# trungnt13/odin-ai

Measured on AMD Instinct MI355X. Metric: VAE train images/sec, higher is better.
Workload: dtype f32; 1 GPU; dsprites_betavae_b256; global_batch=256, per_gpu_batch=256, parallelism=dp1, graph=True

## Files before the change

### include/odin_hip.h

```cpp
#ifndef ODIN_HIP_H
#define ODIN_HIP_H

#include <stddef.h>
#include <stdint.h>

#ifdef __cplusplus
extern "C" {
#endif

enum { ODIN_LINEAR = 0, ODIN_ELU = 1, ODIN_RELU = 2 };

typedef struct odin_conv_desc {
  int B, H, W, Cin;
  int OH, OW, Cout;
  int KH, KW, stride;
  int pad_t, pad_l;
  int act;
  int center;
  uint32_t* dy_amax;
  uint32_t* dx_amax;
  const uint32_t* x_amax;
  uint32_t* y_amax;
} odin_conv_desc;

int odin_version(void);
const char* odin_debug_last_path(void);
uint32_t odin_crc32c(uint32_t crc, const void* data, size_t n);
const char* odin_last_error(void);
int odin_max_slab_rows(void);
int odin_conv2d_dgrad_keeps_range(const odin_conv_desc* d, int aux_act);
int odin_deconv2d_dgrad_keeps_range(const odin_conv_desc* d, int aux_act);
int odin_bernoulli_tail_keeps_range(int is_deconv, const odin_conv_desc* d, int C1);
#define ODIN_RANGE_WORDS 2048
int odin_range_reset(uint32_t* words, int n, void* stream);
int odin_absmax(const float* t, size_t n, uint32_t* word, void* stream);
int odin_debug_stream_probe(const float* a, const float* b, float* out, size_t n, int variant, int blocks,
                            void* stream);
int odin_debug_absmax_fallbacks(void);

int odin_conv2d_fwd(const float* x, const float* w, const float* bias, float* y,
                    const odin_conv_desc* d, void* stream);
int odin_conv2d_dgrad(const float* dy, const float* w, const float* aux, int aux_act, float* dx,
                      float* colsum_slab, int* slab_rows_out, const odin_conv_desc* d,
                      void* stream);
int odin_conv2d_wgrad(const float* x, const float* dy, float* slab, int* slab_rows_out,
                      const odin_conv_desc* d, void* stream);

int odin_deconv2d_fwd(const float* x, const float* w, const float* bias, float* y,
                      const odin_conv_desc* d, void* stream);
int odin_deconv2d_dgrad(const float* dy, const float* w, const float* aux, int aux_act,
                        float* dx, float* colsum_slab, int* slab_rows_out,
                        const odin_conv_desc* d, void* stream);
int odin_deconv2d_wgrad(const float* x, const float* dy, float* slab, int* slab_rows_out,
                        const odin_conv_desc* d, void* stream);

int odin_conv2d_bwd(const float* x, const float* dy, const float* w, const float* aux, int aux_act, float* dx,
                    float* colsum_slab, int* colsum_rows_out, float* wslab, int* wslab_rows_out,
                    const odin_conv_desc* d, void* stream);
int odin_deconv2d_bwd(const float* x, const float* dy, const float* w, const float* aux, int aux_act, float* dx,
                      float* colsum_slab, int* colsum_rows_out, float* wslab, int* wslab_rows_out,
                      const odin_conv_desc* d, void* stream);
int odin_dense_bwd(const float* x, const float* dy, const float* w, const float* aux, int aux_act, float* dx,
                   float* colsum_slab, int* colsum_rows_out, float* wslab, int* wslab_rows_out, int B, int K,
                   int N, int want_wgrad, int want_dgrad, const uint32_t* dy_amax, uint32_t* dx_amax, void* stream);
int odin_conv2d_reads_x_range(const odin_conv_desc* d);
int odin_deconv2d_reads_x_range(const odin_conv_desc* d);
int odin_dense_reads_x_range(int B, int K, int N);
int odin_dense_fwd_ranged(const float* x, const float* w, const float* bias, float* y, int B, int K, int N, int act,
                          const uint32_t* x_amax, uint32_t* y_amax, void* stream);
int odin_dense_bwd_ranged(const float* x, const float* dy, const float* w, const float* aux, int aux_act, float* dx,
                          float* colsum_slab, int* colsum_rows_out, float* wslab, int* wslab_rows_out, int B, int K,
                          int N, int want_wgrad, int want_dgrad, const uint32_t* dy_amax, uint32_t* dx_amax,
                          const uint32_t* x_amax, void* stream);
int odin_dense_dgrad_keeps_range(int B, int K, int N);

int odin_bernoulli_tail_fwd_bwd(int is_deconv, const float* x, const float* w, const float* bias,
                                const float* w1, const float* b1, const float* target,
                                float* logits, float* g_out, float* llk_part, int* n_part_out,
                                float* tail_slab, int* slab_rows_out, const float* scale,
                                const odin_conv_desc* d, int C1, void* stream);

int odin_dense_fwd(const float* x, const float* w, const float* bias, float* y, int B, int K,
                   int N, int act, void* stream);
int odin_dense_dgrad(const float* dy, const float* w, const float* aux, int aux_act, float* dx,
                     float* colsum_slab, int* slab_rows_out, int B, int K, int N, void* stream);
int odin_dense_wgrad(const float* x, const float* dy, float* slab, int* slab_rows_out, int B,
                     int K, int N, void* stream);

typedef struct odin_reduce_job {
  const float* src;
  float* dst;
  int n;
  int rows;
  int stride;
  int pad_;
} odin_reduce_job;
int odin_slab_reduce(const odin_reduce_job* jobs, int n_jobs, void* stream);

int odin_latent_fwd(const float* p, const float* eps, float* z, float* kl, float* fbmask, int B,
                    int D, int analytic, float free_bits, const float* capacity, void* stream);
int odin_latent_bwd(const float* p, const float* eps, const float* z, const float* dz,
                    const float* dz_extra, const float* fbmask, const float* klw,
                    const float* dloc_x, const float* dscale_x, float* dp, int B, int D,
                    int analytic, void* stream);

int odin_latent_block_rows(int B, int P, int D, int N0);
int odin_latent_block_fwd(const float* h, const float* wl, const float* bl, const float* eps_in,
                          float* eps_out, uint64_t seed, const int32_t* step_dev, float* p, float* z,
                          float* kl, float* fbmask, const float* w0, const float* b0, float* y0, int B,
                          int P, int D, int N0, int act0, int analytic, float free_bits,
                          const float* capacity, void* stream);
int odin_latent_block_bwd(const float* g0, const float* w0, const float* z, const float* p,
                          const float* eps, const float* fbmask, const float* klw, const float* dz_extra,
                          const float* dloc_x, const float* dscale_x, const float* wl, const float* h,
                          int h_act, float* dz, float* dp, float* dh, float* slab0, float* slabl, int B,
                          int P, int D, int N0, int analytic, uint32_t* dh_amax, void* stream);

typedef struct odin_neck_args {
  int B, P, D, C0;
  int act2, act3, act4, act0, act1;
  int analytic;
  float free_bits;
  uint64_t seed;
  const int32_t* step_dev;
  const float* x;
  const uint32_t* x_amax;
  const float *w3, *b3;
  float* y3;
  const float *w4, *b4;
  float* y4;
  const float *wl, *bl;
  const float* eps_in;
  float* eps;
  float *p, *z, *kl, *fbmask;
  const float* capacity;
  const float *w0, *b0;
  float* y0;
  const float *w1, *b1;
  float* y1;
  uint32_t* y1_amax;
  const float* dy1;
  const float* klw;
  const float *dz_extra, *dloc_x, *dscale_x;
  float *dz, *dp;
  float* dh4;
  float* dy3;
  float* dx;
  uint32_t *dh4_amax, *dy3_amax, *dx_amax;
  float* slab1;
  float* slab0;
  float* slabl;
} odin_neck_args;
void odin_wgrad_pair_begin(void);
int odin_wgrad_pair_end(void);
int odin_neck_rows(int B, int P, int D, int C0);
int odin_neck_fwd(const odin_neck_args* a, void* stream);
int odin_neck_bwd(const odin_neck_args* a, void* stream);

int odin_disc_head_rows(int B, int K);
int odin_disc_head_fwd_bwd(const float* h, const float* w, const float* bias, float* logit, int mode,
                           const float* dlogit_in, float* dlogit_out, float* out, int aux_act, float* dh,
                           uint32_t* dh_amax, float* wslab, int* rows_out, void* workspace, int B, int K, void* stream);

int odin_elbo_bernoulli_fwd_bwd(const float* logits, const float* x, float* llk_part,
                                float* dlogits, const float* scale, int B, int n_per_sample,
                                int* n_part_out, void* stream);
int odin_elbo_bernoulli_fwd_bwd_ranged(const float* logits, const float* x, float* llk_part,
                                       float* dlogits, const float* scale, int B, int n_per_sample,
                                       int* n_part_out, uint32_t* dlogits_amax, void* stream);
int odin_elbo_gaussian_fwd_bwd(const float* h, const float* x, float* llk_part, float* dh,
                               const float* scale, int B, int n_pix, int C, int softplus1,
                               int* n_part_out, void* stream);
void odin_wgrad_planes_defer_begin(void);
int odin_wgrad_planes_defer_end(void* stream);
double odin_debug_igemm_h_min_flop(double flop);
double odin_debug_blk_min_flop(double flop);
int odin_debug_blk_planes(int enable);
int odin_debug_blk_first(int on);
int odin_debug_dense_hw_min_tiles(int tiles);

int odin_gaussian_tail_applicable(const odin_conv_desc* d, int C);
int odin_gaussian_tail_fwd_bwd(const float* x, const float* w, const float* bias, const float* w1, const float* b1,
                               const float* target, float* logits, float* g_out, float* llk_part, int* n_part_out,
                               float* tail_slab, int* slab_rows_out, const float* scale, const odin_conv_desc* d, int C,
                               int softplus1, void* stream);
int odin_gaussian_head_fwd_bwd(const float* h, const float* w1, const float* b1, const float* target,
                               float* logits, float* dlogits, float* dh, float* llk_part, int* n_part_out,
                               float* wslab, int* rows_out, float* colsum_slab, const float* scale, int B,
                               int n_pix, int Cin, int C, int softplus1, int h_act, uint32_t* dh_amax,
                               void* stream);
int odin_elbo_mixqlogistic_fwd_bwd(const float* h, const float* x, float* llk_part, float* dh,
                                   const float* scale, int B, int n_pix, int C, int K,
                                   int* n_part_out, void* stream);
int odin_elbo_finalize(const float* llk_part, int n_part, const float* kl, const float* hyper,
                       const float* tc, float* llk, float* out4, int B, void* stream);
int odin_mean(const float* x, int n, float* out, void* stream);

int odin_total_correlation_workspace(int B_local, int B_global, int D);
int odin_total_correlation_fwd_bwd(const float* z, const float* p, float* tc_out, float* dz,
                                   float* dloc, float* dscale, const float* coef, int B, int D,
                                   void* stream);
int odin_total_correlation_shard(const float* z_local, const float* p_global, float* tc_out,
                                 float* dz_local, float* dloc_part, float* dscale_part,
                                 const float* coef, int B_local, int B_global, int D, void* stream);
int odin_mmd_workspace(int B_local, int B_global, int M, int D);
int odin_mmd_fwd_bwd(const float* x, const float* y, float* ws, float* dz, const float* coef,
                     const float* coef_grad, int N, int M, int D, int kernel, uint64_t prior_seed,
                     const int32_t* step_dev, void* stream);
int odin_mmd_shard(const float* x_local, const float* x_all, const float* y, float* ws, float* dz_local,
                   const float* coef, const float* coef_grad, int B_local, int B_global, int M, int D,
                   int kernel, int include_yy, uint64_t prior_seed, const int32_t* step_dev, void* stream);
int odin_dip_workspace(int world, int D);
int odin_dip_fwd_bwd(const float* p, float* ws, float* dloc, float* dscale, const float* coef,
                     const float* coef_grad, int N, int D, int type2, float lambda_diag, float lambda_offdiag,
// ... 113 lines not shown
```

### odin_ai_amd/_lib.py

```python
from __future__ import annotations

import ctypes as C
import os
from typing import Optional

_HERE = os.path.dirname(os.path.abspath(__file__))
DEFAULT_LIB = os.path.join(_HERE, 'libodin_hip.so')

ACT = {'linear': 0, 'elu': 1, 'relu': 2, None: 0}


class ConvDesc(C.Structure):
  _fields_ = [(n, C.c_int) for n in ('B', 'H', 'W', 'Cin', 'OH', 'OW', 'Cout', 'KH', 'KW',
                                     'stride', 'pad_t', 'pad_l', 'act', 'center')] + \
             [('dy_amax', C.c_void_p), ('dx_amax', C.c_void_p),
              ('x_amax', C.c_void_p), ('y_amax', C.c_void_p)]


class ReduceJob(C.Structure):
  _fields_ = [('src', C.c_void_p), ('dst', C.c_void_p), ('n', C.c_int), ('rows', C.c_int),
              ('stride', C.c_int), ('pad_', C.c_int)]


class AdamFold(C.Structure):
  _fields_ = [('x', C.c_void_p), ('dy', C.c_void_p), ('B', C.c_int), ('K', C.c_int), ('N', C.c_int), ('w_off', C.c_size_t),
              ('slab', C.c_void_p), ('slab_rows', C.c_int), ('slab_stride', C.c_size_t), ('slab_n', C.c_size_t),
              ('slab_off', C.c_size_t), ('zero', C.c_void_p), ('zero_n', C.c_int)]


class NeckArgs(C.Structure):
  _fields_ = [(n, C.c_int) for n in ('B', 'P', 'D', 'C0', 'act2', 'act3', 'act4', 'act0', 'act1', 'analytic')] + \
             [('free_bits', C.c_float), ('seed', C.c_uint64)] + \
             [(n, C.c_void_p) for n in (
                 'step_dev', 'x', 'x_amax', 'w3', 'b3', 'y3', 'w4', 'b4', 'y4', 'wl', 'bl', 'eps_in', 'eps', 'p', 'z',
                 'kl', 'fbmask', 'capacity', 'w0', 'b0', 'y0', 'w1', 'b1', 'y1', 'y1_amax',
                 'dy1', 'klw', 'dz_extra', 'dloc_x', 'dscale_x', 'dz', 'dp', 'dh4', 'dy3', 'dx',
                 'dh4_amax', 'dy3_amax', 'dx_amax', 'slab1', 'slab0', 'slabl')]


P = C.c_void_p
I = C.c_int
F = C.c_float
IP = C.POINTER(C.c_int)
DP = C.POINTER(ConvDesc)

SIGNATURES = {
    'odin_version': [],
    'odin_debug_last_path': [],
    'odin_crc32c': [C.c_uint32, P, C.c_size_t],
    'odin_max_slab_rows': [],
    'odin_range_reset': [P, I, P],
    'odin_conv2d_dgrad_keeps_range': [DP, I],
    'odin_deconv2d_dgrad_keeps_range': [DP, I],
    'odin_bernoulli_tail_keeps_range': [I, DP, I],
    'odin_conv2d_bwd': [P, P, P, P, I, P, P, IP, P, IP, DP, P],
    'odin_deconv2d_bwd': [P, P, P, P, I, P, P, IP, P, IP, DP, P],
    'odin_dense_bwd': [P, P, P, P, I, P, P, IP, P, IP, I, I, I, I, I, P, P, P],
    'odin_dense_bwd_ranged': [P, P, P, P, I, P, P, IP, P, IP, I, I, I, I, I, P, P, P, P],
    'odin_dense_dgrad_keeps_range': [I, I, I],
    'odin_conv2d_reads_x_range': [DP],
    'odin_deconv2d_reads_x_range': [DP],
    'odin_dense_reads_x_range': [I, I, I],
    'odin_absmax': [P, C.c_size_t, P, P],
    'odin_debug_absmax_fallbacks': [],
    'odin_debug_stream_probe': [P, P, P, C.c_size_t, I, I, P],
    'odin_comm_unique_id': [P],
    'odin_comm_init': [C.POINTER(C.c_void_p), P, I, I],
    'odin_comm_destroy': [P],
    'odin_comm_library': [],
    'odin_allreduce_flat': [P, P, C.c_size_t, P],
    'odin_allgather_flat': [P, P, P, C.c_size_t, P],
    'odin_reduce_scatter_flat': [P, P, P, C.c_size_t, P],
    'odin_conv2d_fwd': [P, P, P, P, DP, P],
    'odin_conv2d_dgrad': [P, P, P, I, P, P, IP, DP, P],
    'odin_conv2d_wgrad': [P, P, P, IP, DP, P],
    'odin_deconv2d_fwd': [P, P, P, P, DP, P],
    'odin_deconv2d_dgrad': [P, P, P, I, P, P, IP, DP, P],
    'odin_deconv2d_wgrad': [P, P, P, IP, DP, P],
    'odin_bernoulli_tail_fwd_bwd': [I, P, P, P, P, P, P, P, P, P, IP, P, IP, P, DP, I, P],
    'odin_dense_fwd': [P, P, P, P, I, I, I, I, P],
    'odin_dense_fwd_ranged': [P, P, P, P, I, I, I, I, P, P, P],
    'odin_dense_dgrad': [P, P, P, I, P, P, IP, I, I, I, P],
    'odin_dense_wgrad': [P, P, P, IP, I, I, I, P],
    'odin_slab_reduce': [C.POINTER(ReduceJob), I, P],
    'odin_latent_fwd': [P, P, P, P, P, I, I, I, F, P, P],
    'odin_latent_bwd': [P, P, P, P, P, P, P, P, P, P, I, I, I, P],
    'odin_latent_block_rows': [I, I, I, I],
    'odin_latent_block_fwd': [P, P, P, P, P, C.c_uint64, P, P, P, P, P, P, P, P, I, I, I, I, I, I, F, P, P],
    'odin_latent_block_bwd': [P, P, P, P, P, P, P, P, P, P, P, P, I, P, P, P, P, P, I, I, I, I, I, P, P],
    'odin_wgrad_pair_begin': [],
    'odin_wgrad_pair_end': [],
    'odin_neck_rows': [I, I, I, I],
    'odin_neck_fwd': [C.POINTER(NeckArgs), P],
    'odin_neck_bwd': [C.POINTER(NeckArgs), P],
    'odin_elbo_bernoulli_fwd_bwd': [P, P, P, P, P, I, I, IP, P],
    'odin_elbo_bernoulli_fwd_bwd_ranged': [P, P, P, P, P, I, I, IP, P, P],
    'odin_elbo_gaussian_fwd_bwd': [P, P, P, P, P, I, I, I, I, IP, P],
    'odin_gaussian_tail_applicable': [DP, I],
    'odin_gaussian_tail_fwd_bwd': [P, P, P, P, P, P, P, P, P, IP, P, IP, P, DP, I, I, P],
    'odin_gaussian_head_fwd_bwd': [P, P, P, P, P, P, P, P, IP, P, IP, P, P, I, I, I, I, I, I, P, P],
    'odin_disc_head_rows': [I, I],
    'odin_disc_head_fwd_bwd': [P, P, P, P, I, P, P, P, I, P, P, P, IP, P, I, I, P],
    'odin_debug_igemm_h_min_flop': [C.c_double],
    'odin_debug_blk_min_flop': [C.c_double],
    'odin_debug_blk_planes': [C.c_int],
    'odin_debug_blk_first': [C.c_int],
    'odin_debug_dense_hw_min_tiles': [C.c_int],
    'odin_debug_mel_r16': [C.c_int],
    'odin_debug_smallc_planes': [C.c_int],
    'odin_wgrad_planes_defer_begin': [],
    'odin_wgrad_planes_defer_end': [P],
    'odin_elbo_mixqlogistic_fwd_bwd': [P, P, P, P, P, I, I, I, I, IP, P],
    'odin_elbo_finalize': [P, I, P, P, P, P, P, I, P],
    'odin_mean': [P, I, P, P],
    'odin_total_correlation_workspace': [I, I, I],
    'odin_total_correlation_fwd_bwd': [P, P, P, P, P, P, P, I, I, P],
    'odin_total_correlation_shard': [P, P, P, P, P, P, P, I, I, I, P],
    'odin_mmd_workspace': [I, I, I, I],
    'odin_mmd_fwd_bwd': [P, P, P, P, P, P, I, I, I, I, C.c_uint64, P, P],
    'odin_mmd_shard': [P, P, P, P, P, P, P, I, I, I, I, I, I, C.c_uint64, P, P],
    'odin_dip_workspace': [I, I],
    'odin_dip_fwd_bwd': [P, P, P, P, P, P, I, I, I, F, F, P],
    'odin_dip_moments': [P, P, I, I, P],
    'odin_dip_finish': [P, I, P, P, P, P, P, P, I, I, I, F, F, P],
    'odin_vamprior_workspace': [I, I, I],
    'odin_vamprior_fwd_bwd': [P, P, P, P, P, P, P, P, I, I, I, P],
    'odin_clip_range_fwd': [P, P, C.c_size_t, F, F, P],
    'odin_clip_range_bwd': [P, P, C.c_size_t, F, F, F, P],
    'odin_vq_workspace': [I],
    'odin_vq_assign': [P, P, P, P, P, P, P, P, I, I, I, P],
    'odin_vq_bwd': [P, P, P, P, P, P, P, P, P, F, C.c_double, C.c_double, I, P, I, I, I, P],
    'odin_permute_dims': [P, P, P, I, I, P],
    'odin_random_perm': [P, I, I, C.c_uint64, P, P],
    'odin_random_permute_dims': [P, P, P, I, I, C.c_uint64, P, P],
    'odin_dtc_loss_fwd_bwd': [P, P, P, P, P, I, P],
    'odin_adam_step_flat': [P, P, P, P, C.c_size_t, P, P, F, P, P],
    'odin_adam_step_fold': [P, P, P, P, C.c_size_t, P, C.POINTER(AdamFold), P],
    'odin_sumsq_flat': [P, C.c_size_t, P, P, P],
    'odin_latent_sample_logprob': [P, P, P, P, P, I, I, I, P],
    'odin_logmeanexp_rows': [P, P, I, I, P],
    'odin_sum_parts': [P, I, P, I, P],
    'odin_grad_skip_threshold': [P, C.c_size_t, F, P, P, P, P],
    'odin_clip_by_norm_segments': [P, P, I, F, P],
    'odin_clip_by_value': [P, C.c_size_t, F, P, F, P],
    'odin_sumsq_adam_flat': [P, P, P, P, C.c_size_t, P, P, P, F, P, P],
    'odin_sumsq_adam_finalize_flat': [P, P, P, P, C.c_size_t, P, P, P, F, P, P, I, P, P, P, P, P, I, P],
    'odin_sumsq_adam_ring': [P, P, P, P, C.c_size_t, P, P, P, F, P, P, I, P, P, P, P, P, I, P, P, P, I, I, I, P],
    'odin_slab_reduce_sumsq': [P, I, P, C.c_size_t, P, IP, P, P, I, P],
    'odin_adam_ring_parts': [P, P, P, P, C.c_size_t, P, I, I, P, I, P, F, P, P, I, P, P, P, P, I, P, P, I, I, I, P],
    'odin_rng_normal': [P, C.c_size_t, C.c_uint64, P, P],
    'odin_gather_normalize_u8': [P, P, P, I, I, F, I, P],
    'odin_gather_rows_f32': [P, P, P, I, I, P],
    'odin_stft_mel_db': [P, P, P, P, P, P, I, I, I, I, I, I, C.c_double, C.c_double, I, P],
    'odin_stft_mel_db_frames': [P, P, P, P, P, P, I, I, I, I, I, I, C.c_double, C.c_double, I, I, P, P],
    'odin_debug_set_stamps': [P],
    'odin_debug_set_wgrad_stamps': [P],
    'odin_debug_set_neck_stamps': [P],
    'odin_debug_elbo_shape': [I, I, I],
    'odin_debug_set_mel_stamps': [P],
    'odin_debug_igemm_h_ldsw_steps': [I],
    'odin_graph_begin': [P],
    'odin_graph_end': [P, C.POINTER(C.c_void_p)],
    'odin_graph_launch': [P, P],
    'odin_graph_destroy': [P],
}


VALUE_RETURNING = ('odin_version', 'odin_comm_library', 'odin_conv2d_dgrad_keeps_range',
                   'odin_deconv2d_dgrad_keeps_range', 'odin_bernoulli_tail_keeps_range', 'odin_dense_dgrad_keeps_range', 'odin_conv2d_reads_x_range',
                   'odin_deconv2d_reads_x_range', 'odin_dense_reads_x_range', 'odin_max_slab_rows', 'odin_debug_absmax_fallbacks', 'odin_crc32c', 'odin_debug_last_path',
                   'odin_latent_block_rows', 'odin_neck_rows', 'odin_debug_igemm_h_ldsw_steps', 'odin_total_correlation_workspace', 'odin_mmd_workspace', 'odin_dip_workspace', 'odin_vamprior_workspace', 'odin_vq_workspace', 'odin_debug_igemm_h_min_flop', 'odin_debug_blk_min_flop',
                   'odin_debug_blk_planes', 'odin_debug_blk_first', 'odin_debug_dense_hw_min_tiles', 'odin_gaussian_tail_applicable', 'odin_disc_head_rows', 'odin_debug_mel_r16', 'odin_debug_smallc_planes')
VOID_RETURNING = ('odin_wgrad_planes_defer_begin', 'odin_wgrad_pair_begin')


class OdinError(RuntimeError):
  pass


class Lib:

  def __init__(self, path: str):
    if not os.path.exists(path):
      raise OdinError(
          f"HIP extension not found: {path}. Build it with `python -c 'import "
          f"__graft_entry__ as g; g.build()'` (hipcc --offload-arch=gfx950). There is no "
          f"CPU fallback.")
    self.path = path
    self.c = C.CDLL(path)
    self.c.odin_last_error.restype = C.c_char_p
    self.c.odin_last_error.argtypes = []
    for name, args in SIGNATURES.items():
      fn = getattr(self.c, name)
      fn.argtypes = args
      fn.restype = (C.c_char_p if name in ('odin_debug_last_path', 'odin_comm_library') else
                    C.c_double if name in ('odin_debug_igemm_h_min_flop', 'odin_debug_blk_min_flop') else
                    None if name in VOID_RETURNING else
                    C.c_uint32 if name in VALUE_RETURNING else C.c_int)

  def check(self, rc: int, what: str = ''):
    if rc != 0:
      raise OdinError(f"{what} failed: {self.c.odin_last_error().decode()} (rc={rc})")

  def __getattr__(self, name):
    if name.startswith('odin_'):
      fn = getattr(self.c, name)

      trace = os.environ.get('ODIN_TRACE', '0') == '1'

# ... 45 lines not shown
```

### odin_ai_amd/csrc/dispatch.hip

```cpp
#include "odin_device.h"
#include "odin_internal.h"

namespace {

enum Family {
  GENERIC,
  SMALLC, PW1X1, SMALLDECONV, SMALLDECONV_GEN,
  FCONV_PLANES, FCONV_RING, FCONV_BLK, CONV5_BLK, TCONV_PLANES, TCONV_RING, TCONV_BLK, IGEMM_H, IGEMM,
  WGRAD_PLANES, WGRAD5_BLK, WGRAD_BLK, IGEMM_H_WGRAD, IGEMM_WGRAD,
  BWD_PLANES, BWD_BLK,
  BWD_PAIR,
  TINY_DENSE, THIN_DENSE, DENSE_H, DENSE_GEMM
};

enum { FOLDS_Y = 1, FOLDS_DX = 2, READS_X = 4 };
int traits(Family f) {
  switch (f) {
    case SMALLC: case SMALLDECONV_GEN: return FOLDS_Y;
    case SMALLDECONV: case IGEMM: case THIN_DENSE: return FOLDS_Y | FOLDS_DX;
    case FCONV_PLANES: case FCONV_BLK: case CONV5_BLK: case TCONV_PLANES: case TCONV_BLK: case IGEMM_H: case DENSE_H:
      return FOLDS_Y | FOLDS_DX | READS_X;
    case WGRAD_PLANES: case WGRAD5_BLK: case WGRAD_BLK: case IGEMM_H_WGRAD: return READS_X;
    case BWD_PLANES: case BWD_BLK: case DENSE_GEMM: return FOLDS_DX;
    default: return 0;
  }
}

int keep_range(int rc, Family f, int fold_bit, const float* t, size_t n, uint32_t* word, void* stream) {
  if (rc != 0 || t == nullptr || word == nullptr || (traits(f) & fold_bit)) return rc;
  return odin_absmax_fold(t, n, word, stream);
}

bool doubles(const odin_geom& g) { return g.OH == 2 * g.H && g.OW == 2 * g.W; }
bool same_size(const odin_geom& g) { return g.H == g.OH && g.W == g.OW; }
bool aligned16(const void* a, const void* b, const void* c, const void* d) {
  return ((((size_t)a | (size_t)b | (size_t)c | (size_t)d)) & 15) == 0;
}


Family select_conv2d_fwd(const odin_geom& g, bool bias, int act) {
  if (odin_smallc_applicable(g)) return SMALLC;
  if (odin_pw1x1_applicable(g)) return PW1X1;
  if (act == ODIN_ACT_ELU && bias && odin_fconv_planes_applicable(g)) return FCONV_PLANES;
  if (act == ODIN_ACT_ELU && bias && odin_fconv_ring_applicable(g)) return FCONV_RING;
  if (bias && same_size(g) && odin_conv5_blk_applicable(g)) return CONV5_BLK;
  if (bias && odin_fconv_blk_applicable(g)) return FCONV_BLK;
  if (odin_igemm_h_applicable(0, g)) return IGEMM_H;
  if (odin_igemm_applicable(0, g)) return IGEMM;
  return GENERIC;
}

bool igemm_dgrad(int tmode, const odin_geom& g, bool slab, bool dry) {
  return odin_igemm_applicable(tmode, g) && (odin_igemm_tiles(tmode, g) <= ODIN_MAX_COLSUM_BLOCKS || (!slab && !dry));
}

Family select_conv2d_dgrad(const odin_geom& l, const odin_geom& g, int aux_act, bool aux_ok, bool slab, bool dry) {
  if (odin_pw1x1_applicable(l)) return PW1X1;
  if (aux_act == ODIN_ACT_ELU && aux_ok && doubles(g) && odin_tconv_planes_applicable(g, 2, 1)) return TCONV_PLANES;
  if (aux_act == ODIN_ACT_ELU && aux_ok && doubles(g) && odin_tconv_ring_applicable(g)) return TCONV_RING;
  if (same_size(g) && odin_conv5_blk_applicable(g)) return CONV5_BLK;
  if (doubles(g) && odin_tconv_blk_applicable(g)) return TCONV_BLK;
  if (odin_igemm_h_applicable(1, g)) return IGEMM_H;
  if (igemm_dgrad(1, g, slab, dry)) return IGEMM;
  return GENERIC;
}

Family select_deconv2d_fwd(const odin_geom& g, bool bias, int act) {
  if (bias && odin_smalldeconv_applicable(g)) return SMALLDECONV;
  if (act == ODIN_ACT_ELU && bias && doubles(g) && odin_tconv_planes_applicable(g, 1, 1)) return TCONV_PLANES;
  if (act == ODIN_ACT_ELU && bias && doubles(g) && odin_tconv_ring_applicable(g)) return TCONV_RING;
  if (bias && (g.CI & 7) != 0 && odin_smalldeconv_gen_applicable(g)) return SMALLDECONV_GEN;
  if (bias && doubles(g) && odin_tconv_blk_applicable(g)) return TCONV_BLK;
  if (odin_igemm_h_applicable(1, g)) return IGEMM_H;
  if (odin_igemm_applicable(1, g)) return IGEMM;
  return GENERIC;
}

Family select_deconv2d_dgrad(const odin_geom& l, const odin_geom& g, int aux_act, bool aux_ok, bool slab, bool dry) {
  if (!slab && odin_smalldeconv_applicable(l)) return SMALLDECONV;
  if (aux_act == ODIN_ACT_ELU && aux_ok && odin_fconv_planes_applicable(g)) return FCONV_PLANES;
  if (odin_fconv_blk_applicable(g)) return FCONV_BLK;
  if (odin_igemm_h_applicable(0, g)) return IGEMM_H;
  const bool ring_two_pass_vs_igemm =
      g.CI == 64 && odin_igemm_applicable(0, g) && odin_igemm_tiles(0, g) <= ODIN_MAX_COLSUM_BLOCKS;
  if (!ring_two_pass_vs_igemm && aux_act == ODIN_ACT_ELU && aux_ok && odin_fconv_ring_applicable(g)) return FCONV_RING;
  if (igemm_dgrad(0, g, slab, dry)) return IGEMM;
  return GENERIC;
}

Family select_bernoulli_tail(int is_deconv, const odin_geom& g, int act, int C1) {
  if (is_deconv && act == ODIN_ACT_ELU && doubles(g) && odin_tconv_planes_applicable(g, 3, C1)) return TCONV_PLANES;
  if (is_deconv && act == ODIN_ACT_ELU && g.CO == 32 && (C1 == 1 || C1 == 3) && doubles(g) &&
      odin_tconv_ring_applicable(g))
    return TCONV_RING;
  return GENERIC;
}

Family select_wgrad_shared(const odin_geom& g, bool want_bias) {
  if (odin_wgrad_planes_applicable(g)) return WGRAD_PLANES;
  if (same_size(g) && want_bias && odin_wgrad5_blk_applicable(g)) return WGRAD5_BLK;
  if (odin_wgrad_blk_applicable(g)) return WGRAD_BLK;
  if (odin_igemm_h_wgrad_applicable(g)) return IGEMM_H_WGRAD;
  if (odin_igemm_wgrad_applicable(g)) return IGEMM_WGRAD;
  return GENERIC;
}
Family select_conv2d_wgrad(const odin_geom& g) {
  if (odin_smallc_applicable(g)) return SMALLC;
  if (odin_pw1x1_applicable(g)) return PW1X1;
  return select_wgrad_shared(g, true);
}
Family select_deconv2d_wgrad(const odin_geom& l, const odin_geom& g) {
  if (odin_smalldeconv_applicable(l)) return SMALLDECONV;
  return select_wgrad_shared(g, false);
}

Family select_deconv2d_bwd(const odin_geom& l, const odin_geom& g, int aux_act, bool aux, bool both, bool dry,
                           bool slab) {
  if (!slab && both && odin_smalldeconv_applicable(l)) return SMALLDECONV;
  const bool k4s2 = l.KH == 4 && l.KW == 4 && l.S == 2 && l.pt == 1 && l.pl == 1 && doubles(l);
  if (((both && aux) || dry) && aux_act == ODIN_ACT_ELU && k4s2 && odin_bwd_planes_applicable(l) &&
      odin_wgrad_planes_applicable(g) && odin_fconv_planes_applicable(g))
    return BWD_PLANES;
  if ((both || dry) && k4s2 && !l.center && odin_bwd_blk_applicable(l)) return BWD_BLK;
  return BWD_PAIR;
}

bool dense_via_igemm() { return ODIN_DIAG_ENV("ODIN_NODENSEIGEMM") == nullptr; }

Family select_dense_fwd(int B, int K, int N, bool aligned) {
  if (odin_tiny_dense_ok(B, K, N)) return TINY_DENSE;
  if (odin_thin_dense_kind(B, K, N) != 0 && aligned) return THIN_DENSE;
  if (odin_dense_h_ok(B, K, N)) return DENSE_H;
  if (dense_via_igemm() && odin_igemm_applicable(0, odin_geom_dense(B, K, N))) return IGEMM;
  if (odin_dense_gemm_ok(B, K, N)) return DENSE_GEMM;
  return GENERIC;
}
Family select_dense_dgrad(int B, int K, int N, bool slab, bool aligned) {
  if (odin_tiny_dense_ok(B, K, N)) return TINY_DENSE;
  if (slab) return GENERIC;
  if (odin_thin_dense_kind(B, K, N) != 0 && aligned) return THIN_DENSE;
  if (odin_dense_h_ok(B, K, N)) return DENSE_H;
  if (dense_via_igemm() && odin_igemm_applicable(1, odin_geom_dense(B, N, K))) return IGEMM;
  if (odin_dense_gemm_ok(B, K, N)) return DENSE_GEMM;
  return GENERIC;
}
Family select_dense_wgrad(int B, int K, int N, bool aligned) {
  if (odin_dense_h_ok(B, K, N)) return DENSE_H;
  if (odin_thin_dense_wgrad_rows(B, K, N) > 0 && aligned) return THIN_DENSE;
  if (dense_via_igemm() && !odin_tiny_dense_ok(B, K, N) && odin_igemm_wgrad_applicable(odin_geom_dense(B, K, N)))
    return IGEMM_WGRAD;
  if (odin_dense_gemm_ok(B, K, N) && !ODIN_DIAG_ENV("ODIN_NOTINYWGRADGEMM")) return DENSE_GEMM;
  return select_wgrad_shared(odin_geom_dense(B, K, N), true);
}
Family select_dense_bwd(int B, int K, int N, bool slab) {
  return odin_dense_h_ok(B, K, N) && !slab ? DENSE_H : BWD_PAIR;
}


int launch_gather(Family f, int tmode, int wmode, const odin_geom& g, const float* in, const float* w, const float* bias,
                  const float* aux, int aux_act, float* out, float* colsum, int* rows_out, int epi, int act,
                  const uint32_t* in_amax, uint32_t* out_amax, void* stream) {
  const float* blk_aux = aux_act != 0 ? aux : nullptr;
  const int blk_act = epi == 1 ? act : aux_act;
  switch (f) {
    case FCONV_PLANES:
      return odin_fconv_planes_launch(in, w, bias, aux, out, colsum, rows_out, g.B, g.OH, g.OW, g.CI, g.CO, epi, in_amax,
                                      out_amax, stream);
    case FCONV_RING:
      return odin_fconv_ring_launch(in, w, bias, aux, out, colsum, rows_out, g.B, g.H, g.W, g.CI, g.OH, g.OW, g.CO, epi,
                                    stream);
    case FCONV_BLK:
      return odin_fconv_blk_launch(in, w, bias, blk_aux, out, colsum, rows_out, g.B, g.OH, g.OW, g.CI, g.CO, epi, blk_act,
                                   in_amax, out_amax, stream);
    case CONV5_BLK:
      return odin_conv5_blk_launch(in, w, bias, blk_aux, out, colsum, rows_out, g.B, g.H, g.W, g.CI, g.CO, g.KH, epi,
                                   blk_act, in_amax, out_amax, stream);
    case TCONV_PLANES:
      return odin_tconv_planes_launch(in, w, bias, aux, out, colsum, rows_out, nullptr, nullptr, nullptr, nullptr, nullptr,
                                      nullptr, nullptr, nullptr, 1, g.B, g.H, g.W, g.CI, g.CO, epi, in_amax, out_amax, stream);
    case TCONV_RING:
      return odin_tconv_ring_launch(in, w, bias, aux, out, colsum, rows_out, nullptr, nullptr, nullptr, nullptr, nullptr,
                                    nullptr, nullptr, nullptr, 1, g.B, g.H, g.W, g.CO, epi, stream);
    case TCONV_BLK:
      return odin_tconv_blk_launch(in, w, bias, blk_aux, out, colsum, rows_out, g.B, g.H, g.W, g.CI, g.CO, epi, blk_act,
                                   in_amax, out_amax, stream);
    case IGEMM_H:
      return odin_igemm_h_launch(tmode, in, w, bias, aux, aux_act, out, colsum, g.B, g.H, g.W, g.CI, g.OH, g.OW, g.CO, g.KH,
                                 g.KW, g.S, g.pt, g.pl, act, in_amax, epi == 2, out_amax, stream);
    case IGEMM:
      return odin_igemm_launch(tmode, in, w, bias, aux, aux_act, out, colsum, g.B, g.H, g.W, g.CI, g.OH, g.OW, g.CO, g.KH,
                               g.KW, g.S, g.pt, g.pl, act, out_amax, stream);
    default:
      return odin_gather_generic(tmode, wmode, g, in, w, bias, act, aux, aux_act, out, colsum,
                                 colsum ? -ODIN_MAX_COLSUM_BLOCKS : odin_num_cus(), rows_out, nullptr, nullptr, stream);
  }
}

int dgrad_rows(Family f, int tmode, const odin_geom& g) {
  switch (f) {
    case SMALLDECONV: return 0;
    case IGEMM_H: return odin_igemm_h_rows(tmode, g);
    case IGEMM: return odin_igemm_tiles(tmode, g);
    default: return -1;
  }
}

int conv_dgrad(Family f, int tmode, int wmode, const odin_geom& g, const float* dy, const float* w, const float* aux,
               int aux_act, float* dx, float* colsum_slab, int* slab_rows_out, const odin_conv_desc* d, void* stream) {
  const int rows = dgrad_rows(f, tmode, g);
  if (rows >= 0) {
    if (slab_rows_out) *slab_rows_out = rows;
    if (dx == nullptr) return 0;
  }
  int rc;
  if (f == PW1X1) rc = odin_pw1x1_dgrad(dy, w, aux, aux_act, dx, colsum_slab, slab_rows_out, d, stream);
  else if (f == SMALLDECONV) rc = odin_smalldeconv_bwd(nullptr, dy, w, aux, aux_act, dx, nullptr, nullptr, d, stream);
  else
    rc = launch_gather(f, tmode, wmode, g, dy, w, nullptr, aux, aux_act, dx, colsum_slab, slab_rows_out, 2, 0, d->dy_amax,
                       d->dx_amax, stream);
  return keep_range(rc, f, FOLDS_DX, dx, (size_t)d->B * d->H * d->W * d->Cin, d->dx_amax, stream);
}

int conv_fwd(Family f, int tmode, int wmode, const odin_geom& g, const float* x, const float* w, const float* bias,
             float* y, const odin_conv_desc* d, void* stream) {
  int rc;
  switch (f) {
    case SMALLC: rc = odin_smallc_fwd(x, w, bias, y, d, stream); break;
    case PW1X1: rc = odin_pw1x1_fwd(x, w, bias, y, d, stream); break;
    case SMALLDECONV: rc = odin_smalldeconv_fwd(x, w, bias, y, d, stream); break;
    case SMALLDECONV_GEN: rc = odin_smalldeconv_gen_fwd(x, w, bias, y, d, stream); break;
    default:
      rc = launch_gather(f, tmode, wmode, g, x, w, bias, nullptr, 0, y, nullptr, nullptr, 1, d->act, d->x_amax, d->y_amax,
                         stream);
  }
  return keep_range(rc, f, FOLDS_Y, y, (size_t)d->B * d->OH * d->OW * d->Cout, d->y_amax, stream);
}

int launch_wgrad(Family f, const odin_geom& g, const float* in, const float* dy, float* slab, int want_bias,
                 const uint32_t* g_amax, const uint32_t* a_amax, int* rows_out, void* stream) {
  const int grad_u = want_bias ? 0 : 1;
  const int slab_stride = g.KH * g.KW * g.CI * g.CO + (want_bias ? g.CO : 0);
  if (f == IGEMM_H_WGRAD || f == IGEMM_WGRAD) {
    if (rows_out) *rows_out = f == IGEMM_H_WGRAD ? odin_igemm_h_wgrad_rows(g) : odin_igemm_wgrad_rows(g);
    if (slab == nullptr) return 0;
  }
  switch (f) {
    case WGRAD_PLANES:
      return odin_wgrad_planes_launch(in, dy, slab, rows_out, g.B, g.OH, g.OW, g.CI, g.CO, want_bias, grad_u, g_amax, a_amax,
                                      stream);
    case WGRAD5_BLK:
      return odin_wgrad5_blk_launch(in, dy, slab, rows_out, g.B, g.H, g.W, g.CI, g.CO, g.KH, want_bias, g_amax, a_amax,
                                    stream);
    case WGRAD_BLK:
      return odin_wgrad_blk_launch(in, dy, slab, rows_out, g.B, g.OH, g.OW, g.CI, g.CO, want_bias, grad_u, g_amax, a_amax,
                                   stream);
    case IGEMM_H_WGRAD:
      return odin_igemm_h_wgrad_launch(in, dy, slab, slab_stride, g.B, g.H, g.W, g.CI, g.OH, g.OW, g.CO, g.KH, g.KW, g.S,
                                       g.pt, g.pl, want_bias, grad_u, g_amax, a_amax, stream);
    case IGEMM_WGRAD:
      return odin_igemm_wgrad_launch(in, dy, slab, slab_stride, g.B, g.H, g.W, g.CI, g.OH, g.OW, g.CO, g.KH, g.KW, g.S, g.pt,
                                     g.pl, want_bias, stream);
    default:
      return odin_wgrad_generic(g, in, dy, slab, want_bias, rows_out, stream);
  }
}

int pair_end(int rc) {
  const int rc2 = odin_igemm_pair_end();
  return rc != 0 ? rc : rc2;
}

}

extern "C" int odin_conv2d_fwd(const float* x, const float* w, const float* bias, float* y, const odin_conv_desc* d,
                               void* stream) {
  const odin_geom g = odin_geom_fwd(d);
  return conv_fwd(select_conv2d_fwd(g, bias != nullptr, d->act), 0, 0, g, x, w, bias, y, d, stream);
}

extern "C" int odin_conv2d_dgrad(const float* dy, const float* w, const float* aux, int aux_act, float* dx,
                                 float* colsum_slab, int* slab_rows_out, const odin_conv_desc* d, void* stream) {
  const odin_geom g = odin_geom_dgrad(d);
  const Family f = select_conv2d_dgrad(odin_geom_fwd(d), g, aux_act, aux != nullptr || dx == nullptr,
                                       colsum_slab != nullptr, dx == nullptr);
  return conv_dgrad(f, 1, 1, g, dy, w, aux, aux_act, dx, colsum_slab, slab_rows_out, d, stream);
}

extern "C" int odin_conv2d_wgrad(const float* x, const float* dy, float* slab, int* slab_rows_out,
                                 const odin_conv_desc* d, void* stream) {
  const odin_geom g = odin_geom_fwd(d);
  const Family f = select_conv2d_wgrad(g);
  if (f == SMALLC) return odin_smallc_wgrad(x, dy, slab, slab_rows_out, d, stream);
  if (f == PW1X1) return odin_pw1x1_wgrad(x, dy, slab, slab_rows_out, d, stream);
  return launch_wgrad(f, g, x, dy, slab, 1, d->dy_amax, d->x_amax, slab_rows_out, stream);
}

extern "C" int odin_conv2d_bwd(const float* x, const float* dy, const float* w, const float* aux, int aux_act, float* dx,
                               float* colsum_slab, int* colsum_rows_out, float* wslab, int* wslab_rows_out,
                               const odin_conv_desc* d, void* stream) {
  odin_igemm_pair_begin();
  int rc = odin_conv2d_wgrad(x, dy, wslab, wslab_rows_out, d, stream);
  if (rc == 0) rc = odin_conv2d_dgrad(dy, w, aux, aux_act, dx, colsum_slab, colsum_rows_out, d, stream);
  return pair_end(rc);
}

extern "C" int odin_conv2d_dgrad_keeps_range(const odin_conv_desc* d, int aux_act) {
  const Family f = select_conv2d_dgrad(odin_geom_fwd(d), odin_geom_dgrad(d), aux_act, true, false, false);
  return (traits(f) & FOLDS_DX) ? 1 : 0;
}

extern "C" int odin_conv2d_reads_x_range(const odin_conv_desc* d) {
  const odin_geom g = odin_geom_fwd(d);
  return ((traits(select_conv2d_fwd(g, true, d->act)) | traits(select_conv2d_wgrad(g))) & READS_X) ? 1 : 0;
}

extern "C" int odin_deconv2d_fwd(const float* x, const float* w, const float* bias, float* y, const odin_conv_desc* d,
                                 void* stream) {
  const odin_geom g = odin_geom_fwd(d);
  return conv_fwd(select_deconv2d_fwd(g, bias != nullptr, d->act), 1, 1, g, x, w, bias, y, d, stream);
}

extern "C" int odin_deconv2d_dgrad(const float* dy, const float* w, const float* aux, int aux_act, float* dx,
                                   float* colsum_slab, int* slab_rows_out, const odin_conv_desc* d, void* stream) {
  const odin_geom g = odin_geom_dgrad(d);
  const Family f = select_deconv2d_dgrad(odin_geom_fwd(d), g, aux_act, aux != nullptr || dx == nullptr,
                                         colsum_slab != nullptr, dx == nullptr);
  return conv_dgrad(f, 0, 0, g, dy, w, aux, aux_act, dx, colsum_slab, slab_rows_out, d, stream);
}

extern "C" int odin_deconv2d_wgrad(const float* x, const float* dy, float* slab, int* slab_rows_out,
                                   const odin_conv_desc* d, void* stream) {
  const odin_geom g = odin_geom_dgrad(d);
  const Family f = select_deconv2d_wgrad(odin_geom_fwd(d), g);
  if (f == SMALLDECONV)
    return odin_smalldeconv_bwd(x, dy, nullptr, nullptr, 0, nullptr, slab, slab_rows_out, d, stream);
  return launch_wgrad(f, g, dy, x, slab, 0, d->dy_amax, d->x_amax, slab_rows_out, stream);
}

extern "C" int odin_deconv2d_bwd(const float* x, const float* dy, const float* w, const float* aux, int aux_act, float* dx,
                                 float* colsum_slab, int* colsum_rows_out, float* wslab, int* wslab_rows_out,
                                 const odin_conv_desc* d, void* stream) {
  const odin_geom l = odin_geom_fwd(d);
  const bool dry = dx == nullptr && wslab == nullptr;
  const Family f = select_deconv2d_bwd(l, odin_geom_dgrad(d), aux_act, aux != nullptr, dx != nullptr && wslab != nullptr,
                                       dry, colsum_slab != nullptr);
  if (f == SMALLDECONV) {
    if (colsum_rows_out) *colsum_rows_out = 0;
    return odin_smalldeconv_bwd(x, dy, w, aux, aux_act, dx, wslab, wslab_rows_out, d, stream);
  }
  if (f == BWD_PLANES || f == BWD_BLK) {
    const int rows = f == BWD_PLANES ? odin_bwd_planes_rows(l) : odin_bwd_blk_rows(l);
    if (colsum_rows_out) *colsum_rows_out = rows;
    if (wslab_rows_out) *wslab_rows_out = rows;
    if (dry) return 0;
    if (f == BWD_PLANES)
      return odin_bwd_planes_launch(x, dy, w, aux, dx, colsum_slab, wslab, d->B, d->H, d->W, d->Cin, d->Cout, d->dy_amax,
                                    d->x_amax, d->dx_amax, stream);
    return odin_bwd_blk_launch(x, dy, w, aux, aux_act, dx, colsum_slab, wslab, d->B, d->H, d->W, d->Cin, d->Cout,
                               d->dy_amax, d->x_amax, d->dx_amax, stream);
  }
  odin_igemm_pair_begin();
  int rc = odin_deconv2d_wgrad(x, dy, wslab, wslab_rows_out, d, stream);
  if (rc == 0) rc = odin_deconv2d_dgrad(dy, w, aux, aux_act, dx, colsum_slab, colsum_rows_out, d, stream);
  return pair_end(rc);
}

extern "C" int odin_deconv2d_dgrad_keeps_range(const odin_conv_desc* d, int aux_act) {
  const Family f = select_deconv2d_dgrad(odin_geom_fwd(d), odin_geom_dgrad(d), aux_act, true, false, false);
  return (traits(f) & FOLDS_DX) ? 1 : 0;
}
extern "C" int odin_deconv2d_reads_x_range(const odin_conv_desc* d) {
  const odin_geom l = odin_geom_fwd(d);
  return ((traits(select_deconv2d_fwd(l, true, d->act)) | traits(select_deconv2d_wgrad(l, odin_geom_dgrad(d)))) & READS_X)
             ? 1 : 0;
}

extern "C" int odin_bernoulli_tail_fwd_bwd(int is_deconv, const float* x, const float* w, const float* bias, const float* w1,
                                           const float* b1, const float* target, float* logits, float* g_out,
                                           float* llk_part, int* n_part_out, float* tail_slab, int* slab_rows_out,
                                           const float* scale, const odin_conv_desc* d, int C1, void* stream) {
  const odin_geom g = odin_geom_fwd(d);
  const Family f = select_bernoulli_tail(is_deconv, g, d->act, C1);
  const odin_tail_args tail = {w1, b1, target, scale, logits, llk_part, tail_slab, C1};
  int rc;
  if (f == TCONV_PLANES)
    rc = odin_tconv_planes_launch(x, w, bias, nullptr, g_out, nullptr, slab_rows_out, w1, b1, target, logits, llk_part,
                                  n_part_out, tail_slab, scale, C1, d->B, d->H, d->W, d->Cin, d->Cout, 3, d->x_amax,
                                  d->dy_amax, stream);
  else if (f == TCONV_RING)
    rc = odin_tconv_ring_launch(x, w, bias, nullptr, g_out, nullptr, slab_rows_out, w1, b1, target, logits, llk_part,
                                n_part_out, tail_slab, scale, C1, d->B, d->H, d->W, d->Cout, 3, stream);
  else
    rc = odin_gather_generic(is_deconv, is_deconv ? 1 : 0, g, x, w, bias, d->act, nullptr, 0, g_out, nullptr,
                             -ODIN_MAX_COLSUM_BLOCKS, slab_rows_out, &tail, n_part_out, stream);
  return keep_range(rc, f, FOLDS_Y, g_out, (size_t)d->B * d->OH * d->OW * d->Cout, d->dy_amax, stream);
}
extern "C" int odin_bernoulli_tail_keeps_range(int is_deconv, const odin_conv_desc* d, int C1) {
  return (traits(select_bernoulli_tail(is_deconv, odin_geom_fwd(d), d->act, C1)) & FOLDS_Y) ? 1 : 0;
}

extern "C" int odin_dense_fwd(const float* x, const float* w, const float* bias, float* y, int B, int K, int N, int act,
                              void* stream) {
  return odin_dense_fwd_ranged(x, w, bias, y, B, K, N, act, nullptr, nullptr, stream);
}

extern "C" int odin_dense_fwd_ranged(const float* x, const float* w, const float* bias, float* y, int B, int K, int N,
                                     int act, const uint32_t* x_amax, uint32_t* y_amax, void* stream) {
  const Family f = select_dense_fwd(B, K, N, aligned16(x, w, y, bias));
  int rc;
  switch (f) {
    case TINY_DENSE: rc = odin_tiny_dense_fwd(x, w, bias, y, B, K, N, act, stream); break;
    case THIN_DENSE: rc = odin_thin_dense_fwd(x, w, bias, y, B, K, N, act, y_amax, stream); break;
    case DENSE_H: rc = odin_dense_h_fwd(x, w, bias, y, B, K, N, act, x_amax, y_amax, stream); break;
    case DENSE_GEMM: rc = odin_dense_gemm_fwd(x, w, bias, y, B, K, N, act, stream); break;
    default:
      rc = launch_gather(f, 0, 0, odin_geom_dense(B, K, N), x, w, bias, nullptr, 0, y, nullptr, nullptr, 1, act, nullptr,
                         y_amax, stream);
  }
  return keep_range(rc, f, FOLDS_Y, y, (size_t)B * N, y_amax, stream);
}

static int dense_dgrad(const float* dy, const float* w, const float* aux, int aux_act, float* dx, float* colsum_slab,
                       int* slab_rows_out, int B, int K, int N, const uint32_t* dy_amax, uint32_t* dx_amax,
                       void* stream) {
  const Family f = select_dense_dgrad(B, K, N, colsum_slab != nullptr, aligned16(dy, w, dx, aux));
  if (f != TINY_DENSE && f != GENERIC) {
    if (slab_rows_out) *slab_rows_out = 0;
    if (dx == nullptr) return 0;
  }
  int rc;
  switch (f) {
    case TINY_DENSE:
      rc = odin_tiny_dense_dgrad(dy, w, aux, aux_act, dx, colsum_slab, slab_rows_out, B, K, N, stream);
      break;
    case THIN_DENSE: rc = odin_thin_dense_dgrad(dy, w, aux, aux_act, dx, B, K, N, dx_amax, stream); break;
    case DENSE_H: rc = odin_dense_h_dgrad(dy, w, aux, aux_act, dx, B, K, N, dy_amax, dx_amax, stream); break;
    case DENSE_GEMM: rc = odin_dense_gemm_dgrad(dy, w, aux, aux_act, dx, B, K, N, dx_amax, stream); break;
    default:
      rc = launch_gather(f, f == IGEMM, 1, odin_geom_dense(B, N, K), dy, w, nullptr, aux, aux_act, dx, colsum_slab,
                         slab_rows_out, 2, 0, nullptr, dx_amax, stream);
  }
  return keep_range(rc, f, FOLDS_DX, dx, (size_t)B * K, dx_amax, stream);
}

extern "C" int odin_dense_dgrad(const float* dy, const float* w, const float* aux, int aux_act, float* dx,
                                float* colsum_slab, int* slab_rows_out, int B, int K, int N, void* stream) {
  return dense_dgrad(dy, w, aux, aux_act, dx, colsum_slab, slab_rows_out, B, K, N, nullptr, nullptr, stream);
}

extern "C" int odin_dense_wgrad(const float* x, const float* dy, float* slab, int* slab_rows_out, int B, int K, int N,
                                void* stream) {
  const Family f = select_dense_wgrad(B, K, N, slab == nullptr || aligned16(x, dy, slab, nullptr));
  if (f == DENSE_H || f == THIN_DENSE || f == DENSE_GEMM) {
    if (slab_rows_out) *slab_rows_out = f == THIN_DENSE ? odin_thin_dense_wgrad_rows(B, K, N) : 1;
    if (slab == nullptr) return 0;
    if (f == DENSE_H) return odin_dense_h_wgrad(x, dy, slab, B, K, N, nullptr, nullptr, stream);
    if (f == THIN_DENSE) return odin_thin_dense_wgrad(x, dy, slab, B, K, N, stream);
    return odin_dense_gemm_wgrad(x, dy, slab, B, K, N, stream);
// ... 51 lines not shown
```

### odin_ai_amd/csrc/odin_internal.h

```cpp
#pragma once
#include <cstdio>
#include <cstring>
#include "../../include/odin_hip.h"

#define ODIN_MAX_SLAB_BLOCKS 256
#define ODIN_MAX_COLSUM_BLOCKS 512

#include <cstdlib>
#ifdef ODIN_DIAG
#define ODIN_DIAG_ENV(name) getenv(name)
#else
#define ODIN_DIAG_ENV(name) ((const char*)nullptr)
#endif
static inline bool odin_exact_fp32() { return getenv("ODIN_EXACT_FP32") != nullptr; }

struct odin_geom {
  int B, H, W, CI, OH, OW, CO, KH, KW, S, pt, pl, center;
};
static inline odin_geom odin_geom_fwd(const odin_conv_desc* d) {
  return {d->B, d->H, d->W, d->Cin, d->OH, d->OW, d->Cout, d->KH, d->KW, d->stride, d->pad_t, d->pad_l, d->center};
}
static inline odin_geom odin_geom_dgrad(const odin_conv_desc* d) {
  return {d->B, d->OH, d->OW, d->Cout, d->H, d->W, d->Cin, d->KH, d->KW, d->stride, d->pad_t, d->pad_l, 0};
}
static inline odin_geom odin_geom_dense(int B, int K, int N) { return {B, 1, 1, K, 1, 1, N, 1, 1, 1, 0, 0, 0}; }

int odin_fail(int code, const char* msg);
int odin_check_launch(const char* what);
int odin_wgrad_planes_flush(void* stream);
int odin_num_cus();
const uint32_t* odin_range_word_of(const float* t, size_t n, const uint32_t* given, void* stream);
int odin_absmax_fold(const float* t, size_t n, uint32_t* word, void* stream);

bool odin_smallc_applicable(const odin_geom& g);
int odin_smallc_fwd(const float* x, const float* w, const float* bias, float* y,
                    const odin_conv_desc* d, void* stream);
int odin_smallc_wgrad(const float* x, const float* dy, float* slab, int* rows_out,
                      const odin_conv_desc* d, void* stream);

bool odin_tiny_dense_ok(int B, int K, int N);
int odin_tiny_dense_fwd(const float* x, const float* w, const float* bias, float* y, int B, int K,
                        int N, int act, void* stream);
int odin_tiny_dense_dgrad(const float* dy, const float* w, const float* aux, int aux_act, float* dx,
                          float* colsum_slab, int* slab_rows_out, int B, int K, int N, void* stream);

bool odin_pw1x1_applicable(const odin_geom& g);
int odin_pw1x1_fwd(const float* x, const float* w, const float* bias, float* y,
                   const odin_conv_desc* d, void* stream);
int odin_pw1x1_dgrad(const float* dy, const float* w, const float* aux, int aux_act, float* dx,
                     float* colsum_slab, int* slab_rows_out, const odin_conv_desc* d, void* stream);
int odin_pw1x1_wgrad(const float* x, const float* dy, float* slab, int* slab_rows_out,
                     const odin_conv_desc* d, void* stream);

bool odin_dense_gemm_ok(int B, int K, int N);
int odin_dense_gemm_fwd(const float* x, const float* w, const float* bias, float* y, int B, int K,
                        int N, int act, void* stream);
int odin_dense_gemm_dgrad(const float* dy, const float* w, const float* aux, int aux_act, float* dx,
                          int B, int K, int N, uint32_t* dx_amax, void* stream);
int odin_zero_u32(uint32_t* p, size_t n, void* stream);
int odin_dense_gemm_wgrad(const float* x, const float* dy, float* slab, int B, int K, int N,
                          void* stream);

int odin_thin_dense_kind(int B, int K, int N);
int odin_thin_dense_wgrad_rows(int B, int K, int N);
int odin_thin_dense_fwd(const float* x, const float* w, const float* bias, float* y, int B, int K, int N, int act,
                        uint32_t* y_amax, void* stream);
int odin_thin_dense_dgrad(const float* dy, const float* w, const float* aux, int aux_act, float* dx, int B, int K, int N,
                          uint32_t* dx_amax, void* stream);
int odin_thin_dense_wgrad(const float* x, const float* dy, float* slab, int B, int K, int N, void* stream);

bool odin_dense_h_ok(int B, int K, int N);
int odin_dense_h_fwd(const float* x, const float* w, const float* bias, float* y, int B, int K, int N, int act,
                     const uint32_t* x_amax, uint32_t* y_amax, void* stream);
int odin_dense_h_dgrad(const float* dy, const float* w, const float* aux, int aux_act, float* dx, int B, int K, int N,
                       const uint32_t* dy_amax, uint32_t* dx_amax, void* stream);
int odin_dense_h_wgrad(const float* x, const float* dy, float* slab, int B, int K, int N, const uint32_t* dy_amax,
                       const uint32_t* x_amax, void* stream);
int odin_dense_h_bwd_pair(const float* x, const float* dy, const float* w, const float* aux, int aux_act, float* dx,
                          float* slab, int B, int K, int N, const uint32_t* dy_amax, uint32_t* dx_amax,
                          const uint32_t* x_amax, void* stream);

bool odin_bwd_planes_applicable(const odin_geom& g);
int odin_bwd_planes_rows(const odin_geom& g);
int odin_bwd_planes_launch(const float* x, const float* dy, const float* w, const float* aux, float* dx, float* colsum,
                           float* wslab, int B, int H, int W, int Cin, int Cout, const uint32_t* dy_amax,
                           const uint32_t* x_amax, uint32_t* dx_amax, void* stream);
bool odin_smalldeconv_applicable(const odin_geom& g);
bool odin_smalldeconv_gen_applicable(const odin_geom& g);
int odin_smalldeconv_gen_fwd(const float* x, const float* w, const float* bias, float* y, const odin_conv_desc* d,
                             void* stream);
int odin_smalldeconv_fwd(const float* x, const float* w, const float* bias, float* y, const odin_conv_desc* d,
                         void* stream);
int odin_smalldeconv_bwd(const float* x, const float* dy, const float* w, const float* aux, int aux_act, float* dx,
                         float* slab, int* rows_out, const odin_conv_desc* d, void* stream);

bool odin_fconv_ring_applicable(const odin_geom& g);
int odin_fconv_ring_launch(const float* in, const float* w, const float* bias, const float* aux,
                           float* out, float* colsum, int* rows_out, int B, int H, int W, int CI,
                           int OH, int OW, int CO, int epi, void* stream);
void odin_fconv_ring_set_stamps(void* buf);

void odin_tconv_ring_set_stamps(void* buf);
bool odin_tconv_ring_applicable(const odin_geom& g);
int odin_tconv_ring_launch(const float* in, const float* w, const float* bias, const float* aux,
                           float* out, float* colsum, int* rows_out, const float* w1, const float* b1,
                           const float* target, float* logits, float* llk_part, int* n_part_out,
                           float* slab, const float* scale, int C1, int B, int H, int W, int CO,
                           int epi, void* stream);

bool odin_tconv_blk_applicable(const odin_geom& g);
int odin_tconv_blk_launch(const float* in, const float* w, const float* bias, const float* aux, float* out,
                          float* colsum, int* rows_out, int B, int H, int W, int CI, int CO, int epi, int act,
                          const uint32_t* in_amax, uint32_t* out_amax, void* stream);
bool odin_fconv_blk_applicable(const odin_geom& g);
int odin_fconv_blk_launch(const float* in, const float* w, const float* bias, const float* aux, float* out,
                          float* colsum, int* rows_out, int B, int OH, int OW, int CI, int CO, int epi, int act,
                          const uint32_t* in_amax, uint32_t* out_amax, void* stream);
bool odin_wgrad_blk_applicable(const odin_geom& g);
int odin_wgrad_blk_launch(const float* U, const float* V, float* slab, int* rows_out, int B, int OH, int OW, int CI,
                          int CO, int want_bias, int grad_u, const uint32_t* g_amax, const uint32_t* a_amax,
                          void* stream);
bool odin_conv5_blk_applicable(const odin_geom& g);
int odin_conv5_blk_launch(const float* in, const float* w, const float* bias, const float* aux, float* out,
                          float* colsum, int* rows_out, int B, int H, int W, int CI, int CO, int K, int epi, int act,
                          const uint32_t* in_amax, uint32_t* out_amax, void* stream);
bool odin_wgrad5_blk_applicable(const odin_geom& g);
int odin_wgrad5_blk_launch(const float* x, const float* dy, float* slab, int* rows_out, int B, int H, int W, int CI,
                           int CO, int K, int want_bias, const uint32_t* g_amax, const uint32_t* a_amax, void* stream);
bool odin_blk_enabled(double flop);
bool odin_blk_first();
bool odin_bwd_blk_applicable(const odin_geom& g);
int odin_bwd_blk_rows(const odin_geom& g);
int odin_bwd_blk_launch(const float* x, const float* dy, const float* w, const float* aux, int aux_act, float* dx,
                        float* colsum, float* wslab, int B, int H, int W, int Cin, int Cout, const uint32_t* dy_amax,
                        const uint32_t* x_amax, uint32_t* dx_amax, void* stream);
void odin_tconv_planes_set_stamps(void* buf);
bool odin_tconv_planes_applicable(const odin_geom& g, int epi, int C1);
int odin_tconv_planes_launch(const float* in, const float* w, const float* bias, const float* aux,
                             float* out, float* colsum, int* rows_out, const float* w1, const float* b1,
                             const float* target, float* logits, float* llk_part, int* n_part_out,
                             float* slab, const float* scale, int C1, int B, int H, int W, int CI,
                             int CO, int epi, const uint32_t* in_amax, uint32_t* out_amax, void* stream);

bool odin_wgrad_planes_applicable(const odin_geom& g);
int odin_wgrad_planes_launch(const float* U, const float* V, float* slab, int* rows_out, int B, int OH,
                             int OW, int CI, int CO, int want_bias, int grad_u, const uint32_t* g_amax,
                             const uint32_t* a_amax, void* stream);

bool odin_fconv_planes_applicable(const odin_geom& g);
void odin_fconv_planes_set_stamps(void* buf);
int odin_fconv_planes_launch(const float* in, const float* w, const float* bias, const float* aux,
                             float* out, float* colsum, int* rows_out, int B, int OH, int OW, int CI, int CO,
                             int epi, const uint32_t* in_amax, uint32_t* out_amax, void* stream);

bool odin_igemm_applicable(int tmode, const odin_geom& g);
void odin_igemm_set_stamps(void* buf);
int odin_igemm_tiles(int tmode, const odin_geom& g);
int odin_igemm_launch(int tmode, const float* in, const float* w, const float* bias, const float* aux,
                      int aux_act, float* out, float* colsum, int B, int H, int W, int CI, int OH, int OW,
                      int CO, int KH, int KW, int S, int pt, int pl, int act, uint32_t* out_amax, void* stream);
void odin_igemm_pair_begin();
int odin_igemm_pair_end();
bool odin_igemm_h_applicable(int tmode, const odin_geom& g);
int odin_igemm_h_rows(int tmode, const odin_geom& g);
int odin_igemm_h_launch(int tmode, const float* in, const float* w, const float* bias, const float* aux, int aux_act,
                        float* out, float* colsum, int B, int H, int W, int CI, int OH, int OW, int CO, int KH, int KW,
                        int S, int pt, int pl, int act, const uint32_t* in_amax, int in_is_grad, uint32_t* out_amax,
                        void* stream);
bool odin_igemm_h_wgrad_applicable(const odin_geom& g);
int odin_igemm_h_wgrad_rows(const odin_geom& g);
int odin_igemm_h_wgrad_launch(const float* u, const float* v, float* slab, int slab_stride, int B, int FH, int FW,
                              int CU, int h, int w, int CV, int KH, int KW, int S, int pt, int pl, int want_bias,
                              int grad_u, const uint32_t* g_amax, const uint32_t* a_amax, void* stream);
bool odin_igemm_wgrad_applicable(const odin_geom& g);
int odin_igemm_wgrad_rows(const odin_geom& g);
int odin_igemm_wgrad_launch(const float* u, const float* v, float* slab, int slab_stride, int B, int FH,
                            int FW, int CU, int h, int w, int CV, int KH, int KW, int S, int pt, int pl,
                            int want_bias, void* stream);

struct odin_tail_args {
  const float *w1, *b1, *target, *scale;
  float *logits, *llk_part, *slab;
  int C1;
};
int odin_gather_generic(int mode_t, int wmode, const odin_geom& g, const float* in, const float* w, const float* bias,
                        int act, const float* aux, int aux_act, float* out, float* colsum_slab, int max_blocks,
                        int* rows_out, const odin_tail_args* tail, int* n_part_out, void* stream);
int odin_wgrad_generic(const odin_geom& g, const float* in, const float* dy, float* slab, int want_bias, int* rows_out,
                       void* stream);
```

### odin_ai_amd/csrc/tconv_planes.hip

```cpp
#include "odin_device.h"
#include "odin_internal.h"
#include <cstdlib>
#include <utility>

namespace {

struct TPParams {
  const float* in;
  const float* w;
  const float* bias;
  const float* aux;
  float* out;
  float* colsum;
  const float* w1;
  const float* b1;
  const float* target;
  float* logits;
  float* llk_part;
  float* slab;
  const float* scale;
  int B, H, CO;
  int CS, ci_off;
  int tiles_per_img, n_tiles, tiles_per_wg;
  const unsigned* in_amax;
  unsigned* out_amax;
  long long* stamps;
  int part_off;
};

#if defined(ODIN_SIM) || !defined(ODIN_DIAG)
#define TP_STAMP(k) ((void)0)
#else
#define TP_STAMP(k)                                                                               \
  do {                                                                                            \
    if (p.stamps != nullptr && blockIdx.x == 0 && blockIdx.y == 0 && lane == 0 && (wave & 3) == 0 && \
        stamp_i < 31)                                                                             \
      p.stamps[8 * wave + stamp_i++] = ((long long)(k) << 56) | (long long)(clock64() & 0xFFFFFFFFFFFFFFll); \
  } while (0)
#endif

__host__ __device__ constexpr int tp_late_index(int g0, int m) {
  return (m < g0 || m == 32 || m == 33 || m == 34 || m == 36 || m == 42)
             ? -1
             : (m - g0) - ((m > 32) + (m > 33) + (m > 34) + (m > 36) + (m > 42));
}
static_assert(tp_late_index(25, 47) >= 11, "three logit maps: 8 gradient + 4 store slots must fit");

template <int... Is, class F>
__device__ __forceinline__ void tp_static_for_impl(std::integer_sequence<int, Is...>, F&& f) {
  (f(std::integral_constant<int, Is>{}), ...);
}
template <int N, class F>
__device__ __forceinline__ void tp_static_for(F&& f) {
  tp_static_for_impl(std::make_integer_sequence<int, N>{}, static_cast<F&&>(f));
}

struct TpYes { static constexpr bool value = true; };
struct TpNo { static constexpr bool value = false; };

constexpr int TP_NPL = 2;
constexpr int TP_TAPB = TP_NPL * 4 * 512;
constexpr int TP_WBYTES = 16 * TP_TAPB;

__device__ __forceinline__ float tp_pairsum32(float x) {
#ifdef ODIN_SIM
  return x + __shfl_xor(x, 32);
#else
  const unsigned u = __float_as_uint(x);
  const auto r = __builtin_amdgcn_permlane32_swap(u, u, false, false);
  return __uint_as_float(r[0]) + __uint_as_float(r[1]);
#endif
}

struct alignas(8) TpEnt {
  int x, y;
};

struct TpItem {
  float4 v;
  int dst;
  int ok;
};

template <int EPI, int C1, int W, int DBG = 0, bool ACC = false, int SCM = 0, bool PL = false>
__device__ __forceinline__ void tp_body(const TPParams& p) {
  constexpr int NPL = TP_NPL;
  constexpr int RP = 64 / W;
  constexpr int NSLOT = 2 * RP + 3;
  constexpr int PB = (W + 2) * 64;
  constexpr int RB = NPL * PB;
  constexpr int CPR = W / 8;
  constexpr int CSHIFT = (W == 32) ? 2 : (W == 16) ? 1 : 0;
  ODIN_DYN_SMEM(char, smem);
  char* wl = smem;
  char* ring = smem + TP_WBYTES;
  constexpr int NRED = 32 * (1 + (EPI == 3 ? C1 : 0)) + 4;
  __shared__ float cred[8 * NRED];
  __shared__ float llk_red[2][8];
  const int tid = threadIdx.x, lane = tid & 63;
#ifdef ODIN_SIM
  const int wave = tid >> 6;
#else
  const int wave = __builtin_amdgcn_readfirstlane(tid >> 6);
#endif
  const int l31 = lane & 31, half = lane >> 5;
  int stamp_i = 0;
  (void)stamp_i;
  TP_STAMP(1);
#if defined(ODIN_DIAG) && !defined(ODIN_SIM)
  if (p.stamps != nullptr && blockIdx.x == 0 && blockIdx.y == 0 && tid == 0) {
    p.stamps[64] = clock64();
    p.stamps[65] = wall_clock64();
  }
#endif
  const int n0 = blockIdx.y * 32;
  const int HP = p.H + 1;
  const int OH = 2 * p.H, OW = 2 * W;
  const int T0 = blockIdx.x * p.tiles_per_wg;
  int T1 = T0 + p.tiles_per_wg;
  if (T1 > p.n_tiles) T1 = p.n_tiles;
  if (T0 >= T1) return;

  const OdinRangeReq in_rq = odin_range_issue(SCM != 0 ? p.in_amax : nullptr, lane);
  float4 wv[8];
#pragma unroll
  for (int j = 0; j < 8; ++j) {
    const int e = tid + 512 * j;
    const int ci4 = e & 7, co = (e >> 3) & 31, tap = e >> 8;
    wv[j] = *reinterpret_cast<const float4*>(p.w + ((size_t)(tap * p.CO + n0 + co) * p.CS + p.ci_off + 4 * ci4));
  }
  const OdinRun IN = odin_run(p.in, (unsigned)((size_t)p.B * p.H * W * p.CS * 4));
  float amx = 0.f;
  const int f_c = wave & (CPR - 1), f_r0 = wave >> CSHIFT;
  constexpr int F_RJ = 8 >> CSHIFT;
  const int f_px = 8 * f_c + (lane >> 3), f_ch4 = lane & 7, f_pc = f_px + 1;
  const int f_lds_lane = f_pc * 64 + ((((f_ch4 >> 1) ^ ((f_pc >> 2) & 3))) << 4) + (f_ch4 & 1) * 8;
  const unsigned f_g_lane = (unsigned)((f_px * p.CS + p.ci_off + 4 * f_ch4) * 4);
  const unsigned f_rowbytes = (unsigned)(W * p.CS * 4);
  TpItem itA[2], itB[2];
  {
    const int tpi = p.tiles_per_img;
    const int b0 = odin_div_small(T0, tpi), t0 = T0 - b0 * tpi;
    const int start = HP * b0 + RP * t0;
#pragma unroll
    for (int j = 0; j < 2; ++j) {
      const int r = f_r0 + F_RJ * j, G = start + r;
      const bool valid = r < RP + 2;
      const int b = b0 + (RP * t0 + r >= HP ? 1 : 0), gi = G - b * HP;
      const bool real = valid && gi != 0 && b < p.B;
      itA[j].dst = (G % NSLOT) * RB + f_lds_lane;
      itA[j].ok = valid;
      itA[j].v = odin_run_load4(IN, (real ? (unsigned)(G - b - 1) * f_rowbytes : 0xFFFF0000u) + f_g_lane);
    }
  }
  ODIN_SCHED_FENCE();
  bool scl = SCM == 1;
  float in_s = 1.f, in_s2k = ODIN_LO_SCALE, out_s = 1.f, out_sx = ODIN_LO_UNSCALE;

  for (int e = tid; e < NSLOT * 8 * NPL; e += 512) {
    const int sl = e / (8 * NPL), rem = e - sl * (8 * NPL);
    const int pl = rem >> 3, side = (rem >> 2) & 1, piece = rem & 3;
    *reinterpret_cast<float4*>(ring + sl * RB + pl * PB + (side ? (W + 1) * 64 : 0) + piece * 16) =
        make_float4(0.f, 0.f, 0.f, 0.f);
  }

  constexpr int RPF = 2 * F_RJ;
  const int NF = p.tiles_per_wg + 3;
  TpEnt* tr = reinterpret_cast<TpEnt*>(ring + NSLOT * RB);
  {
    const int tpi = p.tiles_per_img;
    for (int e = tid; e < NF * RPF; e += 512) {
      const int f = e / RPF, r = e - f * RPF;
      const int T = T0 + f, b1 = odin_div_small(T, tpi), t1 = T - b1 * tpi;
      const int end = HP * b1 + RP * t1 + RP + 2;
      int start = end - (RP + 2);
      if (f > 0) {
        const int b0 = t1 > 0 ? b1 : b1 - 1, t0 = t1 > 0 ? t1 - 1 : tpi - 1;
        start = HP * b0 + RP * t0 + RP + 2;
      }
      const int G = start + r;
      const bool valid = T < T1 && G < end;
      const int b = odin_div_small(G, HP), gi = G - b * HP;
      const bool real = valid && gi != 0 && b < p.B;
      tr[e] = TpEnt{valid ? (G % NSLOT) * RB : -1, real ? (int)((unsigned)(G - b - 1) * f_rowbytes) : (int)0xFFFF0000u};
    }
  }
  auto fill_entries = [&](TpEnt (&en)[2], int f) {
#pragma unroll
    for (int j = 0; j < 2; ++j) en[j] = tr[f * RPF + f_r0 + F_RJ * j];
  };
  auto fill_loads = [&](TpItem (&it)[2], const TpEnt (&en)[2]) {
#pragma unroll
    for (int j = 0; j < 2; ++j) {
      it[j].dst = en[j].x + f_lds_lane;
#ifdef ODIN_SIM
      it[j].ok = en[j].x >= 0;
#else
      it[j].ok = __builtin_amdgcn_readfirstlane(en[j].x) >= 0;
#endif
      it[j].v = odin_run_load4(IN, (unsigned)en[j].y + f_g_lane);
    }
  };
  auto store_fill1 = [&](const TpItem& it) {
    if (it.ok) {
      u32x2 h, l;
      if (SCM == 1 || (SCM == 2 && scl)) odin_split_h4<true>(it.v, in_s, in_s2k, h, l);
      else odin_split_h4<false>(it.v, 1.f, ODIN_LO_SCALE, h, l);
      char* d = ring + it.dst;
      *reinterpret_cast<u32x2*>(d) = h;
      *reinterpret_cast<u32x2*>(d + PB) = l;
    }
  };
  auto store_fill = [&](const TpItem (&it)[2]) {
    store_fill1(it[0]);
    store_fill1(it[1]);
  };

  const int role = wave & 3, grp = wave >> 2;
  const int cpw = role & 1, rpar = role >> 1;
  const int rp = (W == 32) ? grp : (W == 16) ? 2 * grp + (l31 >> 4) : 4 * grp + (l31 >> 3);
  const int i_in = (W == 32) ? l31 : (W == 16) ? (l31 & 15) : (l31 & 7);
  const int kw_a = cpw ? 0 : 1, kw_b = kw_a + 2;
  const int kh_a = rpar ? 0 : 1, kh_b = kh_a + 2;
  const int d_a = cpw ? 2 : 1;
  int offA[2], offB[2];
#pragma unroll
  for (int kk = 0; kk < 2; ++kk) {
    const int pa = i_in + d_a, pb = pa - 1;
    offA[kk] = pa * 64 + (((2 * kk + half) ^ ((pa >> 2) & 3)) << 4);
    offB[kk] = pb * 64 + (((2 * kk + half) ^ ((pb >> 2) & 3)) << 4);
  }
  const int roff_a = rp + (rpar ? 2 : 1);
  const char* wlane = wl + half * 512 + l31 * 16;
  const int tap_aa = (kh_a * 4 + kw_a) * TP_TAPB, tap_ab = (kh_a * 4 + kw_b) * TP_TAPB;
  const int tap_ba = (kh_b * 4 + kw_a) * TP_TAPB, tap_bb = (kh_b * 4 + kw_b) * TP_TAPB;

  auto ch_of = [&](int r) { return (r & 3) + 8 * (r >> 2) + 4 * half; };
  constexpr float LOG2E = 1.44269504088896341f;
  constexpr bool CL = (EPI == 3 && C1 > 1);
  __shared__ float cst[CL ? 32 * (1 + C1) : 4];
  if (CL) {
    for (int e = tid; e < 32 * (1 + C1); e += 512) {
      const int ch = e & 31, oc = (e >> 5) - 1;
      cst[e] = e < 32 ? p.bias[n0 + ch] : p.w1[(n0 + ch) * C1 + oc];
    }
  }
  const float* cl = cst + 4 * half;
  float bias_r[((EPI == 1 || EPI == 3) && !CL) ? 16 : 1];
  if ((EPI == 1 || EPI == 3) && !CL) {
#pragma unroll
    for (int r = 0; r < 16; ++r) bias_r[r] = p.bias[n0 + ch_of(r)];
  }
  float w1r[(EPI == 3 && !CL) ? 16 : 1][(EPI == 3 && !CL) ? C1 : 1];
  float dw1[(EPI == 3) ? 16 : 1][(EPI == 3) ? C1 : 1];
  float b1r[(EPI == 3) ? C1 : 1];
  float db1[(EPI == 3) ? C1 : 1];
  if (EPI == 3) {
#pragma unroll
    for (int r = 0; r < 16; ++r)
#pragma unroll
      for (int oc = 0; oc < C1; ++oc) {
        if (!CL) w1r[r][oc] = p.w1[(n0 + ch_of(r)) * C1 + oc];
        dw1[r][oc] = 0.f;
      }
#pragma unroll
    for (int oc = 0; oc < C1; ++oc) { b1r[oc] = p.b1[oc]; db1[oc] = 0.f; }
  }
  float csum[(EPI >= 2) ? 16 : 1];
#pragma unroll
  for (int r = 0; r < ((EPI >= 2) ? 16 : 1); ++r) csum[r] = 0.f;
  const float sc = (EPI == 3) ? p.scale[0] : 0.f;
  float llk_lane = 0.f;
  const unsigned out_bytes = (unsigned)((size_t)p.B * OH * OW * p.CO * 4);
  const OdinRun OUT = odin_run(p.out, out_bytes);
  const OdinRun AUX = odin_run(EPI == 2 ? p.aux : nullptr, EPI == 2 ? out_bytes : 0u);
  const unsigned tgt_bytes = (EPI == 3) ? (unsigned)((size_t)p.B * OH * OW * C1 * 4) : 0u;
  const OdinRun TG = odin_run(EPI == 3 ? p.target : nullptr, tgt_bytes);
  const OdinRun LG = odin_run(EPI == 3 ? p.logits : nullptr, (EPI == 3 && p.logits != nullptr) ? tgt_bytes : 0u);

  if (SCM != 0) {
    const unsigned in_mb = odin_range_finish(in_rq);
    scl = SCM == 1 || odin_act_needs_scale(in_mb);
    const int gk = scl ? odin_range_shift(in_mb) : 0;
    in_s = odin_pow2(gk); in_s2k = odin_pow2(gk + 11);
    out_s = odin_pow2(-gk); out_sx = odin_pow2(-gk - 11);
  }
  f32x16 biasv = f32x16_zero();
  if ((EPI == 1 || EPI == 3) && !CL) {
#pragma unroll
    for (int r = 0; r < 16; ++r) biasv[r] = bias_r[r] * in_s;
  }
  {
#pragma unroll
    for (int j = 0; j < 8; ++j) {
      const int e = tid + 512 * j;
      const int ci4 = e & 7, co = (e >> 3) & 31, tap = e >> 8;
      u32x2 h, l;
      odin_split_h4<false>(wv[j], 1.f, ODIN_LO_SCALE, h, l);
      char* d = wl + tap * TP_TAPB + (ci4 >> 1) * 512 + co * 16 + (ci4 & 1) * 8;
      *reinterpret_cast<u32x2*>(d) = h;
      *reinterpret_cast<u32x2*>(d + 2048) = l;
    }
  }
  store_fill(itA);
  TP_STAMP(2);
  __syncthreads();
  TP_STAMP(10);
  TpEnt en[2];
  fill_entries(en, 1);
  fill_loads(itA, en);

  int b_cur = T0 / p.tiles_per_img, t_cur = T0 - b_cur * p.tiles_per_img;
  int sl0 = (HP * b_cur + RP * t_cur) % NSLOT;
  const unsigned pix_lane = (unsigned)((2 * rp + rpar) * OW + 2 * i_in + cpw);
  const unsigned out_lane = (pix_lane * p.CO + n0 + 4 * half) * 4, tgt_lane = pix_lane * C1 * 4;
  const unsigned lg_lane = (half == 0) ? tgt_lane : ODIN_OOB_V;
  unsigned tileP_out = 0, tileP_tgt = 0;
  f32x16 pa = f32x16_zero();
  float4 axP[4], pvP[4];
  float tgtP[(EPI == 3) ? C1 : 1] = {};
#pragma unroll
  for (int q = 0; q < 4; ++q) axP[q] = pvP[q] = make_float4(0.f, 0.f, 0.f, 0.f);
  float dl[(EPI == 3) ? C1 : 1] = {};

  auto elu_b = [&](int r, float b) __attribute__((always_inline)) {
    const float t = pa[r] + b;
    const float em1 = odin_exp2(t * LOG2E) - 1.f;
    pa[r] = t > 0.f ? t : em1;
  };
  auto elu_r = [&](int r) { elu_b(r, 0.f); };
  char* plds = smem + p.part_off + tid * 16;
  int tileP_loc = 0;
  auto store_q = [&](int q) __attribute__((always_inline)) {
    if (DBG & 1) return;
    if (EPI >= 1) amx = odin_amax3(odin_amax3(amx, pa[4 * q], pa[4 * q + 1]), pa[4 * q + 2], pa[4 * q + 3]);
    if (PL && EPI == 0) {
      *reinterpret_cast<float4*>(plds + (tileP_loc * 4 + q) * 8192) =
          make_float4(pa[4 * q], pa[4 * q + 1], pa[4 * q + 2], pa[4 * q + 3]);
      return;
    }
    odin_run_store4s(OUT, out_lane + 32 * q, tileP_out,
                     make_float4(pa[4 * q], pa[4 * q + 1], pa[4 * q + 2], pa[4 * q + 3]));
  };
  float t_dot = 0.f, lgt = 0.f, eabs = 0.f;
  constexpr int N_EPI_OPS = (EPI == 3) ? 12 + 4 * C1 + 8 : 12;
  auto epi_op = [&](int k) {
    if (k < 8) {
      const int r0 = 2 * k, r1 = r0 + 1;
      if (ACC) {
        const int q = k >> 1;
        pa[r0] += (k & 1) ? pvP[q].z : pvP[q].x;
        pa[r1] += (k & 1) ? pvP[q].w : pvP[q].y;
      }
      if (EPI == 1 || EPI == 3) { elu_r(r0); elu_r(r1); }
      if (EPI == 2) {
        const int q = k >> 1;
        const float a0 = (k & 1) ? axP[q].z : axP[q].x, a1 = (k & 1) ? axP[q].w : axP[q].y;
        pa[r0] = fmaf(pa[r0], fminf(a0, 0.f), pa[r0]);
        pa[r1] = fmaf(pa[r1], fminf(a1, 0.f), pa[r1]);
        csum[r0] += pa[r0];
        csum[r1] += pa[r1];
      }
    }
    if (EPI <= 2) {
      if (k >= 8 && k < 12) store_q(k - 8);
    }
    if (EPI == 3) {
      if (k >= 8 && k < 8 + 4 * C1) {
        const int oc = (k - 8) >> 2, ph = (k - 8) & 3;
        if (ph == 0) {
          t_dot = pa[0] * w1r[0][oc];
#pragma unroll
          for (int r = 1; r < 16; ++r) t_dot = fmaf(pa[r], w1r[r][oc], t_dot);
        }
        if (ph == 1) {
          lgt = tp_pairsum32(t_dot) + b1r[oc];
          eabs = odin_exp2(-LOG2E * fabsf(lgt));
          odin_run_store1s(LG, lg_lane + 4 * oc, tileP_tgt, lgt);
        }
        if (ph == 2) {
          const float sp = fmaxf(lgt, 0.f) + 0.6931471805599453f * odin_log2(1.f + eabs);
          llk_lane += half == 0 ? tgtP[oc] * lgt - sp : 0.f;
        }
        if (ph == 3) {
          const float rr = odin_rcp(1.f + eabs);
          const float sg = lgt >= 0.f ? rr : eabs * rr;
          const float dsig = (sg - tgtP[oc]) * sc;
          db1[oc] += half == 0 ? dsig : 0.f;
          dl[oc] = dsig;
        }
      }
      constexpr int G0 = 8 + 4 * C1;
      if (k >= G0 && k < G0 + 8) {
#pragma unroll
        for (int r = 2 * (k - G0); r < 2 * (k - G0) + 2; ++r) {
          float gs = w1r[r][0] * dl[0];
          dw1[r][0] = fmaf(pa[r], dl[0], dw1[r][0]);
#pragma unroll
          for (int oc = 1; oc < C1; ++oc) {
            gs = fmaf(w1r[r][oc], dl[oc], gs);
            dw1[r][oc] = fmaf(pa[r], dl[oc], dw1[r][oc]);
          }
          pa[r] = fmaf(gs, fminf(pa[r], 0.f), gs);
          csum[r] += pa[r];
        }
      }
      if (k >= G0 + 8 && k < G0 + 12) store_q(k - G0 - 8);
    }
  };
  static_assert(CL || N_EPI_OPS + 8 <= 32, "epilogue micro-ops must fit before the row stores (steps 6, 7)");

  float4 cbq = make_float4(0.f, 0.f, 0.f, 0.f);
  float4 wqA[CL ? C1 : 1], wqB[CL ? C1 : 1];
  float t3[CL ? C1 : 1] = {}, lg3[CL ? C1 : 1] = {}, ea3[CL ? C1 : 1] = {};
  auto f4c = [](const float4& v, int j) { return j == 0 ? v.x : j == 1 ? v.y : j == 2 ? v.z : v.w; };
  auto ld_bias = [&](int q) { cbq = *reinterpret_cast<const float4*>(cl + 8 * q); };
  auto ld_w = [&](float4 (&wq)[CL ? C1 : 1], int q) __attribute__((always_inline)) {
#pragma unroll
    for (int oc = 0; oc < (CL ? C1 : 1); ++oc)
      wq[oc] = *reinterpret_cast<const float4*>(cl + 32 + 32 * oc + 8 * q);
  };
  auto cl_elu2 = [&](int k) __attribute__((always_inline)) {
    elu_b(2 * k, (k & 1) ? cbq.z : cbq.x);
    elu_b(2 * k + 1, (k & 1) ? cbq.w : cbq.y);
  };
  auto cl_dot = [&](int q, const float4 (&wq)[CL ? C1 : 1]) __attribute__((always_inline)) {
#pragma unroll
    for (int oc = 0; oc < (CL ? C1 : 1); ++oc) {
      float t = (q == 0) ? pa[0] * wq[oc].x : fmaf(pa[4 * q], wq[oc].x, t3[oc]);
      t = fmaf(pa[4 * q + 1], wq[oc].y, t);
      t = fmaf(pa[4 * q + 2], wq[oc].z, t);
      t3[oc] = fmaf(pa[4 * q + 3], wq[oc].w, t);
    }
  };
  auto cl_lg = [&](int ph, int oc) __attribute__((always_inline)) {
    if (ph == 0) {
      lg3[oc] = tp_pairsum32(t3[oc]) + b1r[oc];
      ea3[oc] = odin_exp2(-LOG2E * fabsf(lg3[oc]));
      odin_run_store1s(LG, lg_lane + 4 * oc, tileP_tgt, lg3[oc]);
    }
    if (ph == 1) {
      const float sp = fmaxf(lg3[oc], 0.f) + 0.6931471805599453f * odin_log2(1.f + ea3[oc]);
      llk_lane += half == 0 ? tgtP[oc] * lg3[oc] - sp : 0.f;
    }
    if (ph == 2) {
      const float rr = odin_rcp(1.f + ea3[oc]);
      const float sg = lg3[oc] >= 0.f ? rr : ea3[oc] * rr;
      const float dsig = (sg - tgtP[oc]) * sc;
      db1[oc] += half == 0 ? dsig : 0.f;
      dl[oc] = dsig;
    }
  };
  auto cl_grad2 = [&](int i, const float4 (&wq)[CL ? C1 : 1]) __attribute__((always_inline)) {
#pragma unroll
    for (int r = 2 * i; r < 2 * i + 2; ++r) {
      float gs = f4c(wq[0], r & 3) * dl[0];
      dw1[r][0] = fmaf(pa[r], dl[0], dw1[r][0]);
#pragma unroll
      for (int oc = 1; oc < (CL ? C1 : 1); ++oc) {
        gs = fmaf(f4c(wq[oc], r & 3), dl[oc], gs);
        dw1[r][oc] = fmaf(pa[r], dl[oc], dw1[r][oc]);
      }
      pa[r] = fmaf(gs, fminf(pa[r], 0.f), gs);
      csum[r] += pa[r];
    }
  };
  auto cl_top = [&]() __attribute__((always_inline)) {
    ld_bias(0);
    ld_w(wqA, 0);
  };
  auto cl_slot = [&](auto M) __attribute__((always_inline)) {
    constexpr int m = decltype(M)::value;
    if constexpr (m < 16) {
      if constexpr ((m & 1) == 0) {
        cl_elu2(m >> 1);
        if constexpr ((m & 3) == 2 && m < 14) ld_bias((m >> 2) + 1);
      } else if constexpr ((m & 3) == 3) {
        constexpr int q = m >> 2;
        if constexpr (q & 1) cl_dot(q, wqB); else cl_dot(q, wqA);
        if constexpr (q == 0) ld_w(wqA, 2);
        if constexpr (q == 1) ld_w(wqB, 3);
        if constexpr (q == 3) ld_w(wqA, 0);
      } else if constexpr (m == 1) {
        ld_w(wqB, 1);
      }
    } else if constexpr (m < 16 + 3 * C1) {
      cl_lg((m - 16) / C1, (m - 16) % C1);
      if constexpr (m == 16 + 3 * C1 - 1) ld_w(wqB, 1);
    } else {
      constexpr int n = tp_late_index(16 + 3 * C1, m);
      if constexpr (n >= 0 && n < 8) {
        if constexpr ((n >> 1) & 1) cl_grad2(n, wqB); else cl_grad2(n, wqA);
        if constexpr (n == 1) ld_w(wqA, 2);
        if constexpr (n == 3) ld_w(wqB, 3);
      }
      if constexpr (n >= 8 && n < 12) store_q(n - 8);
    }
  };

  auto flush_llk = [&](int T) {
    if (EPI == 3) {
#ifndef ODIN_SIM
      asm volatile("; llk flush" ::: "memory");
#endif
      const float tt = odin_wave_sum64_valu(llk_lane);
      llk_red[T & 1][wave] = tt;
      llk_lane = 0.f;
    }
  };

  auto run_tile = [&](auto with_epi, auto group_b, int T) {
    constexpr bool WE = decltype(with_epi)::value;
    constexpr bool GB = decltype(group_b)::value && !CL;
    constexpr int ESH = GB ? 16 : 0;
    constexpr int SF0 = GB ? 4 : 36, SF1 = GB ? 10 : 42, FL = GB ? 47 : 34;
    int sa = sl0 + roff_a, sb = sa - 1;
    if (sa >= NSLOT) sa -= NSLOT;
    if (sb >= NSLOT) sb -= NSLOT;
    const char* row_a = ring + sa * RB;
    const char* row_b = ring + sb * RB;
    f32x16 acc = ((EPI == 1 || EPI == 3) && !CL) ? biasv : f32x16_zero(), acx = f32x16_zero();
    u32x4 fa[2][NPL], fb[2][NPL];
    auto loads = [&](int s, u32x4 (&A)[NPL], u32x4 (&Bf)[NPL]) {
      const int tp = s >> 1, kk = s & 1;
      const bool ra = tp < 2, ca = (tp & 1) == 0;
      const char* bp = (ra ? row_a : row_b) + (ca ? offA[kk] : offB[kk]);
      const char* ap = wlane + (ra ? (ca ? tap_aa : tap_ab) : (ca ? tap_ba : tap_bb)) + kk * 1024;
#pragma unroll
      for (int pl = 0; pl < NPL; ++pl) {
        A[pl] = *reinterpret_cast<const u32x4*>(ap + pl * 2048);
        Bf[pl] = *reinterpret_cast<const u32x4*>(bp + pl * PB);
      }
    };
    loads(0, fa[0], fb[0]);
    if (WE && CL) cl_top();
    ODIN_SCHED_FENCE();
    const unsigned tile_pix = (unsigned)((b_cur * OH + 2 * RP * t_cur) * OW);
    const unsigned tile_out = tile_pix * (unsigned)p.CO * 4u, tile_tgt = tile_pix * (unsigned)C1 * 4u;
    float4 axN[4], pvN[4];
    float tgtN[(EPI == 3) ? C1 : 1] = {};
#pragma unroll
    for (int q = 0; q < 4; ++q) axN[q] = pvN[q] = make_float4(0.f, 0.f, 0.f, 0.f);
    ODIN_SCHED_FENCE();
    auto slot = [&](auto MS) __attribute__((always_inline)) {
      constexpr int m = decltype(MS)::value;
      constexpr int me = m - ESH;
      constexpr int k = me < 0 ? -1 : (me < 16 ? ((me & 1) ? -1 : me / 2) : me - 8);
      if constexpr (WE && !CL && k >= 0 && k < N_EPI_OPS && !(DBG & 4)) epi_op(k);
      if constexpr (WE && CL && !(DBG & 4)) cl_slot(MS);
      if (m == 20) fill_entries(en, T - T0 + 2);
      if (m == 32) fill_loads(itB, en);
      if (m == 33) {
        if (EPI == 2) {
#pragma unroll
          for (int q = 0; q < 4; ++q)
            axN[q] = odin_run_load4s(AUX, out_lane + 32 * q, tile_out);
        }
        if (EPI == 3) {
#pragma unroll
          for (int oc = 0; oc < C1; ++oc) tgtN[oc] = odin_run_load1s(TG, tgt_lane + 4 * oc, tile_tgt);
        }
        if (ACC && PL) {
#pragma unroll
          for (int q = 0; q < 4; ++q) pvN[q] = *reinterpret_cast<const float4*>(plds + ((T - T0) * 4 + q) * 8192);
        }
        if (ACC && !PL) {
#pragma unroll
          for (int q = 0; q < 4; ++q)
            pvN[q] = odin_run_load4s(OUT, out_lane + 32 * q, tile_out);
        }
      }
      if (WE && m == FL && t_cur == 0) flush_llk(T - 1);
      if (m == SF0) store_fill1(itA[0]);
      if (m == SF1) store_fill1(itA[1]);
    };
    tp_static_for<24>([&](auto MM) __attribute__((always_inline)) {
      constexpr int M = decltype(MM)::value;
      constexpr int s = M / 3, u = M % 3, cur = s & 1, nxt = cur ^ 1;
      if constexpr (u == 0) {
        if (s + 1 < 8 && !(DBG & 2)) loads(s + 1, fa[nxt], fb[nxt]);
        if (s + 1 < 8 && (DBG & 2)) {
#pragma unroll
          for (int pl = 0; pl < NPL; ++pl) { fa[nxt][pl] = fa[cur][pl]; fb[nxt][pl] = fb[cur][pl]; }
        }
      }
      if (u == 0) acx = mfma32_f16(fa[cur][0], fb[cur][1], acx);
      if (u == 1) acc = mfma32_f16(fa[cur][0], fb[cur][0], acc);
      if (u == 2) acx = mfma32_f16(fa[cur][1], fb[cur][0], acx);
      slot(std::integral_constant<int, 2 * M>{});
      slot(std::integral_constant<int, 2 * M + 1>{});
      ODIN_SCHED_FENCE();
#ifdef ODIN_DIAG
      if (M == 0 || M == 5 || M == 11 || M == 17 || M == 23) TP_STAMP(12 + (M + 1) / 6);
#endif
    });
    if (SCM == 1 || (SCM == 2 && scl)) {
#pragma unroll
      for (int r = 0; r < 16; ++r) pa[r] = fmaf(acx[r], out_sx, acc[r] * out_s);
    } else {
#pragma unroll
      for (int r = 0; r < 16; ++r) pa[r] = fmaf(acx[r], ODIN_LO_UNSCALE, acc[r]);
    }
    tileP_out = tile_out;
    tileP_tgt = tile_tgt;
    tileP_loc = T - T0;
#pragma unroll
    for (int q = 0; q < 4; ++q) { axP[q] = axN[q]; pvP[q] = pvN[q]; }
#pragma unroll
    for (int oc = 0; oc < ((EPI == 3) ? C1 : 1); ++oc) tgtP[oc] = tgtN[oc];
    itA[0] = itB[0];
    itA[1] = itB[1];
  };

  auto tile_loop = [&](auto group_b) __attribute__((always_inline)) {
    run_tile(TpNo{}, group_b, T0);
    TP_STAMP(11);
    __syncthreads();
    TP_STAMP(10);
#pragma unroll 1
    for (int T = T0 + 1; T < T1; ++T) {
      sl0 += RP;
      if (++t_cur == p.tiles_per_img) { t_cur = 0; ++b_cur; ++sl0; }
      if (sl0 >= NSLOT) sl0 -= NSLOT;
      run_tile(TpYes{}, group_b, T);
      TP_STAMP(11);
      __syncthreads();
      TP_STAMP(10);
      if (EPI == 3 && tid == 0) {
        const float* q = llk_red[(T - 1) & 1];
        p.llk_part[T - 1] =
            t_cur == 0 ? ((q[0] + q[1]) + (q[2] + q[3])) + ((q[4] + q[5]) + (q[6] + q[7])) : 0.f;
      }
    }
  };
  if (!CL && wave >= 4) tile_loop(TpYes{}); else tile_loop(TpNo{});
  if (CL) {
    cl_top();
    tp_static_for<48>([&](auto M) __attribute__((always_inline)) { cl_slot(M); });
  } else {
#pragma unroll
    for (int k = 0; k < N_EPI_OPS; ++k) epi_op(k);
  }
  flush_llk(T1 - 1);

#if defined(ODIN_DIAG) && !defined(ODIN_SIM)
  if (p.stamps != nullptr && blockIdx.x == 0 && blockIdx.y == 0 && tid == 0) {
    p.stamps[66] = clock64();
    p.stamps[67] = wall_clock64();
  }
#endif
  if (EPI >= 1) {
    __syncthreads();
    odin_amax_commit_wg(p.out_amax, amx, tid, 512, cred, blockIdx.x + gridDim.x * blockIdx.y);
    __syncthreads();
  }
  if (EPI >= 2) {
#pragma unroll
    for (int r = 0; r < 16; ++r) {
      const int ch = (r & 3) + 8 * (r >> 2) + 4 * half;
      float vv = csum[r];
#pragma unroll
      for (int m = 16; m >= 1; m >>= 1) vv += __shfl_xor(vv, m);
      if (l31 == 0) cred[wave * NRED + ch] = vv;
      if (EPI == 3) {
#pragma unroll
        for (int oc = 0; oc < C1; ++oc) {
          float ww = dw1[r][oc];
#pragma unroll
          for (int m = 16; m >= 1; m >>= 1) ww += __shfl_xor(ww, m);
          if (l31 == 0) cred[wave * NRED + 32 + ch * C1 + oc] = ww;
        }
      }
    }
  }
  if (EPI == 3) {
#pragma unroll
    for (int oc = 0; oc < C1; ++oc) {
      float vv = db1[oc];
#pragma unroll
      for (int m = 16; m >= 1; m >>= 1) vv += __shfl_xor(vv, m);
      if (lane == 0) cred[wave * NRED + 32 + 32 * C1 + oc] = vv;
    }
  }
  if (EPI == 2 && p.colsum != nullptr) {
    __syncthreads();
    if (tid < 32) {
      float tt = 0.f;
      for (int wv = 0; wv < 8; ++wv) tt += cred[wv * NRED + tid];
      p.colsum[(size_t)blockIdx.x * p.CO + n0 + tid] = tt;
    }
  }
  if (EPI == 3) {
    __syncthreads();
    if (tid == 0) {
      const float* q = llk_red[(T1 - 1) & 1];
      p.llk_part[T1 - 1] = ((q[0] + q[1]) + (q[2] + q[3])) + ((q[4] + q[5]) + (q[6] + q[7]));
    }
    float* row = p.slab + (size_t)blockIdx.x * (p.CO * C1 + C1 + p.CO);
    for (int e = tid; e < 32 + 32 * C1 + C1; e += 512) {
      float tt = 0.f;
      for (int wv = 0; wv < 8; ++wv) tt += cred[wv * NRED + e];
      if (e < 32) {
        row[p.CO * C1 + C1 + e] = tt;
      } else if (e < 32 + 32 * C1) {
        const int ch = (e - 32) / C1, oc = (e - 32) - ch * C1;
        row[ch * C1 + oc] = tt;
      } else {
        row[p.CO * C1 + (e - 32 - 32 * C1)] = tt;
      }
    }
  }
}

template <int EPI, int C1, int W, int DBG = 0, bool ACC = false, int SCM = 0>
__global__ __launch_bounds__(512) void tconv_planes_kernel(TPParams p) {
  tp_body<EPI, C1, W, DBG, ACC, SCM>(p);
}

template <int EPI, int W, int SCM, bool PL>
__global__ __launch_bounds__(512) void tconv_planes2_kernel(TPParams p) {
  {
    TPParams q = p;
    q.colsum = nullptr;
    q.out_amax = nullptr;
    q.ci_off = 0;
    tp_body<0, 1, W, 0, false, SCM, PL>(q);
  }
  odin_wait_vmem();
#ifndef ODIN_SIM
  __builtin_amdgcn_fence(__ATOMIC_SEQ_CST, "workgroup");
#endif
  __syncthreads();
  p.ci_off = 32;
  tp_body<EPI, 1, W, 0, true, SCM, PL>(p);
}

constexpr int TP_LDS_MAX = 152 * 1024;
int tp_ring_bytes(int W) { return TP_WBYTES + (2 * (64 / W) + 3) * TP_NPL * (W + 2) * 64; }
int tp_fill_bytes(int W) { return 8 * 2 * (W == 32 ? 2 : W == 16 ? 4 : 8); }
int tp_tiles_per_wg(int W, int n_tiles, int gy) {
  int cap = odin_num_cus() / gy;
  if (cap < 1) cap = 1;
  if (cap > ODIN_MAX_COLSUM_BLOCKS) cap = ODIN_MAX_COLSUM_BLOCKS;
  int tpw = (n_tiles + cap - 1) / cap;
  const int limit = (TP_LDS_MAX - tp_ring_bytes(W)) / tp_fill_bytes(W) - 3;
  if (tpw > limit) tpw = limit;
  if ((n_tiles + tpw - 1) / tpw > ODIN_MAX_COLSUM_BLOCKS) return -1;
  return tpw;
}

template <int EPI, int C1, bool ACC, int SC>
int tp_launch_w(const TPParams& p, int W, dim3 grid, void* stream) {
  const size_t lds = (size_t)tp_ring_bytes(W) + (size_t)(p.tiles_per_wg + 3) * tp_fill_bytes(W);
  constexpr int W3 = (EPI == 3 ? 16 : 8);
#ifndef ODIN_SIM
  static bool attr_done = false;
  if (!attr_done) {
    const void* fns[3] = {reinterpret_cast<const void*>(&tconv_planes_kernel<EPI, C1, 32, 0, ACC, SC>),
                          reinterpret_cast<const void*>(&tconv_planes_kernel<EPI, C1, 16, 0, ACC, SC>),
                          reinterpret_cast<const void*>(&tconv_planes_kernel<EPI, C1, W3, 0, ACC, SC>)};
    for (int i = 0; i < 3; ++i)
      if (hipFuncSetAttribute(fns[i], hipFuncAttributeMaxDynamicSharedMemorySize, TP_LDS_MAX) != hipSuccess)
        (void)hipGetLastError();
    attr_done = true;
  }
#ifdef ODIN_DIAG
  if (W == 32 && EPI == 3 && C1 == 1) {
    static const int dbg = [] { const char* e = ODIN_DIAG_ENV("ODIN_TP_DBG"); return e ? atoi(e) : 0; }();
    static bool dattr = false;
    if (!dattr) {
      const void* dfn[4] = {reinterpret_cast<const void*>(&tconv_planes_kernel<EPI, C1, 32, 1, ACC, SC>),
                            reinterpret_cast<const void*>(&tconv_planes_kernel<EPI, C1, 32, 2, ACC, SC>),
                            reinterpret_cast<const void*>(&tconv_planes_kernel<EPI, C1, 32, 4, ACC, SC>),
                            reinterpret_cast<const void*>(&tconv_planes_kernel<EPI, C1, 32, 7, ACC, SC>)};
      for (int i = 0; i < 4; ++i)
        if (hipFuncSetAttribute(dfn[i], hipFuncAttributeMaxDynamicSharedMemorySize, TP_LDS_MAX) != hipSuccess)
          (void)hipGetLastError();
      dattr = true;
    }
    if (dbg == 1) { ODIN_LAUNCH((tconv_planes_kernel<EPI, C1, 32, 1, ACC, SC>), grid, dim3(512), lds, stream, p); return odin_check_launch("tconv_planes(f16x2)"); }
    if (dbg == 2) { ODIN_LAUNCH((tconv_planes_kernel<EPI, C1, 32, 2, ACC, SC>), grid, dim3(512), lds, stream, p); return odin_check_launch("tconv_planes(f16x2)"); }
    if (dbg == 4) { ODIN_LAUNCH((tconv_planes_kernel<EPI, C1, 32, 4, ACC, SC>), grid, dim3(512), lds, stream, p); return odin_check_launch("tconv_planes(f16x2)"); }
    if (dbg == 7) { ODIN_LAUNCH((tconv_planes_kernel<EPI, C1, 32, 7, ACC, SC>), grid, dim3(512), lds, stream, p); return odin_check_launch("tconv_planes(f16x2)"); }
  }
#endif
#endif
  if (W == 32) ODIN_LAUNCH((tconv_planes_kernel<EPI, C1, 32, 0, ACC, SC>), grid, dim3(512), lds, stream, p);
  else if (W == 16) ODIN_LAUNCH((tconv_planes_kernel<EPI, C1, 16, 0, ACC, SC>), grid, dim3(512), lds, stream, p);
  else ODIN_LAUNCH((tconv_planes_kernel<EPI, C1, W3, 0, ACC, SC>), grid, dim3(512), lds, stream, p);
  return odin_check_launch("tconv_planes(f16x2)");
}

constexpr int TP2_LDS_MAX = 160000;
int tp_pl_tiles(int W) {
  const int free_b = TP2_LDS_MAX - tp_ring_bytes(W) - 8 * tp_fill_bytes(W);
  return free_b < 32768 ? 0 : free_b / 32768;
}

template <int EPI, int SC, bool PL>
int tp_launch2_w(const TPParams& p0, int W, dim3 grid, void* stream) {
  TPParams p = p0;
  size_t lds = (size_t)tp_ring_bytes(W) + (size_t)(p.tiles_per_wg + 3) * tp_fill_bytes(W);
  if (PL) {
    lds = (lds + 15) & ~(size_t)15;
    p.part_off = (int)lds;
    lds += (size_t)p.tiles_per_wg * 32768;
  }
#ifndef ODIN_SIM
  static bool attr_done = false;
  if (!attr_done) {
    const void* fns[3] = {reinterpret_cast<const void*>(&tconv_planes2_kernel<EPI, 32, SC, PL>),
                          reinterpret_cast<const void*>(&tconv_planes2_kernel<EPI, 16, SC, PL>),
                          reinterpret_cast<const void*>(&tconv_planes2_kernel<EPI, 8, SC, PL>)};
    for (int i = 0; i < 3; ++i)
      if (hipFuncSetAttribute(fns[i], hipFuncAttributeMaxDynamicSharedMemorySize, TP2_LDS_MAX) != hipSuccess)
        (void)hipGetLastError();
    attr_done = true;
  }
#endif
  if (W == 32) ODIN_LAUNCH((tconv_planes2_kernel<EPI, 32, SC, PL>), grid, dim3(512), lds, stream, p);
  else if (W == 16) ODIN_LAUNCH((tconv_planes2_kernel<EPI, 16, SC, PL>), grid, dim3(512), lds, stream, p);
  else ODIN_LAUNCH((tconv_planes2_kernel<EPI, 8, SC, PL>), grid, dim3(512), lds, stream, p);
  return odin_check_launch("tconv_planes(f16x2)");
}

}

static long long* g_tp_stamps = nullptr;
void odin_tconv_planes_set_stamps(void* buf) { g_tp_stamps = (long long*)buf; }

bool odin_tconv_planes_applicable(const odin_geom& g, int epi, int C1) {
  const int B = g.B, H = g.H, W = g.W, CI = g.CI, CO = g.CO, KH = g.KH, KW = g.KW, S = g.S, pt = g.pt, pl = g.pl;
  if (odin_blk_first()) return false;
  if (odin_exact_fp32() || ODIN_DIAG_ENV("ODIN_NOPLANES") || ODIN_DIAG_ENV("ODIN_SPLIT")) return false;
  if (epi == 3 && (CO != 32 || (C1 != 1 && C1 != 3) || CI != 32 || W == 8)) return false;
  return KH == 4 && KW == 4 && S == 2 && pt == 1 && pl == 1 && (CI == 32 || CI == 64) && (CO % 32) == 0 &&
         !g.center && (W == 8 || W == 16 || W == 32) && (H % (64 / W)) == 0 && (size_t)B * H * W * CI * 4 < (1ull << 31) &&
         (size_t)B * H * W * 4 * C1 * 4 < (1ull << 31) && tp_tiles_per_wg(W, B * (H / (64 / W)), CO / 32) > 0;
}

int odin_tconv_planes_launch(const float* in, const float* w, const float* bias, const float* aux,
                             float* out, float* colsum, int* rows_out, const float* w1, const float* b1,
                             const float* target, float* logits, float* llk_part, int* n_part_out,
                             float* slab, const float* scale, int C1, int B, int H, int W, int CI,
                             int CO, int epi, const uint32_t* in_amax, uint32_t* out_amax, void* stream) {
  TPParams p;
  memset(&p, 0, sizeof(p));
  p.in = in; p.w = w; p.bias = bias; p.aux = aux; p.out = out; p.colsum = colsum;
  p.w1 = w1; p.b1 = b1; p.target = target; p.logits = logits; p.llk_part = llk_part; p.slab = slab;
  p.scale = scale;
  p.B = B; p.H = H; p.CO = CO;
  p.CS = CI; p.ci_off = 0;
  p.stamps = g_tp_stamps;
  const int RP = 64 / W;
  p.tiles_per_img = H / RP;
  p.n_tiles = B * p.tiles_per_img;
  const int gy = CO / 32;
  p.tiles_per_wg = tp_tiles_per_wg(W, p.n_tiles, gy);
  if (p.tiles_per_wg <= 0) return odin_fail(-2, "tconv_planes: too many tiles for the fill table");
  bool pl = false;
  if (CI == 64 && !ODIN_DIAG_ENV("ODIN_TP_NOPL")) {
    const int cap = tp_pl_tiles(W);
    if (cap >= 1) {
      int tpw = p.tiles_per_wg < cap ? p.tiles_per_wg : cap;
      if ((p.n_tiles + tpw - 1) / tpw <= ODIN_MAX_COLSUM_BLOCKS) { p.tiles_per_wg = tpw; pl = true; }
    }
  }
  const int gx = (p.n_tiles + p.tiles_per_wg - 1) / p.tiles_per_wg;
  if (rows_out) *rows_out = gx;
  if (n_part_out) *n_part_out = p.tiles_per_img;
  if (out == nullptr) return 0;
  if (epi == 2) {
    p.in_amax = odin_range_word_of(in, (size_t)B * H * W * CI, in_amax, stream);
    if (p.in_amax == nullptr) return odin_fail(-3, "tconv_planes: no range word for the gradient input");
  }
  p.out_amax = out_amax;
  const bool aw = epi != 2 && in_amax != nullptr;
  if (aw) p.in_amax = in_amax;
  dim3 grid(gx, gy, 1);
  if (CI == 64) {
    if (epi == 3) return odin_fail(-2, "tconv_planes tail: 32 input channels only");
#ifdef ODIN_DIAG
    if (ODIN_DIAG_ENV("ODIN_TP_2LAUNCH")) {
      TPParams q = p;
      q.colsum = nullptr;
      q.out_amax = nullptr;
      const int rc = epi == 1 ? tp_launch_w<0, 1, false, 0>(q, W, grid, stream) : tp_launch_w<0, 1, false, 1>(q, W, grid, stream);
      if (rc != 0) return rc;
      p.ci_off = 32;
      return epi == 1 ? tp_launch_w<1, 1, true, 0>(p, W, grid, stream) : tp_launch_w<2, 1, true, 1>(p, W, grid, stream);
    }
#endif
    if (pl) {
      if (epi == 1) return aw ? tp_launch2_w<1, 2, true>(p, W, grid, stream) : tp_launch2_w<1, 0, true>(p, W, grid, stream);
      return tp_launch2_w<2, 1, true>(p, W, grid, stream);
    }
    if (epi == 1) return aw ? tp_launch2_w<1, 2, false>(p, W, grid, stream) : tp_launch2_w<1, 0, false>(p, W, grid, stream);
    return tp_launch2_w<2, 1, false>(p, W, grid, stream);
  }
  if (epi == 1) return aw ? tp_launch_w<1, 1, false, 2>(p, W, grid, stream) : tp_launch_w<1, 1, false, 0>(p, W, grid, stream);
  if (epi == 2) return tp_launch_w<2, 1, false, 1>(p, W, grid, stream);
  if (C1 == 1) return aw ? tp_launch_w<3, 1, false, 2>(p, W, grid, stream) : tp_launch_w<3, 1, false, 0>(p, W, grid, stream);
  if (C1 == 3) return aw ? tp_launch_w<3, 3, false, 2>(p, W, grid, stream) : tp_launch_w<3, 3, false, 0>(p, W, grid, stream);
  return odin_fail(-2, "tconv_planes tail: one or three logit maps only");
}
```

### odin_ai_amd/engine.py

```python
from __future__ import annotations

import ctypes as C
import math
from typing import Callable, Dict, List, NamedTuple, Optional, Sequence, Tuple

import numpy as np
import torch

from . import _lib
from ._lib import ACT, ConvDesc, ReduceJob


def same_pads(n: int, k: int, s: int) -> Tuple[int, int, int]:
  out = -(-n // s)
  total = max((out - 1) * s + k - n, 0)
  return out, total // 2, total - total // 2


class ParamLayout:

  def __init__(self):
    self.entries: List[Tuple[tuple, Tuple[int, ...], int]] = []
    self.size = 0

  def add(self, key, shape) -> int:
    off = self.size
    self.entries.append((key, tuple(shape), off))
    self.size += int(np.prod(shape))
    return off

  def pad_to(self, mult=4):
    self.size = (self.size + mult - 1) // mult * mult

  def views(self, flat: torch.Tensor) -> Dict[tuple, torch.Tensor]:
    return {k: flat[o:o + int(np.prod(s))].view(s) for k, s, o in self.entries}


class LayerRec:
  __slots__ = ('kind', 'act', 'key', 'w_off', 'b_off', 'w_n', 'b_n', 'in_shape', 'out_shape',
               'desc', 'K', 'N', 'center')


def build_layers(net: str, layers: Sequence[tuple], in_shape: Tuple[int, ...],
                 layout: ParamLayout) -> Tuple[List[LayerRec], Tuple[int, ...]]:
  recs: List[LayerRec] = []
  shp = tuple(in_shape)
  center = False
  for li, L in enumerate(layers):
    kind = L[0]
    if kind == 'center':
      center = True
      continue
    if kind == 'flatten':
      shp = (int(np.prod(shp)),)
      continue
    if kind == 'reshape':
      assert int(np.prod(L[1])) == int(np.prod(shp))
      shp = tuple(L[1])
      continue
    r = LayerRec()
    r.kind, r.key, r.center = kind, (net, li), center
    r.in_shape = shp
    r.desc = None
    r.K = r.N = 0
    if kind == 'conv':
      _, co, k, s, act = L
      H, W, Ci = shp
      OH, pt, _ = same_pads(H, k, s)
      OW, pl, _ = same_pads(W, k, s)
      r.act = act
      r.out_shape = (OH, OW, co)
      r.desc = dict(H=H, W=W, Cin=Ci, OH=OH, OW=OW, Cout=co, K=k, stride=s, pad_t=pt, pad_l=pl)
      wshape = (k, k, Ci, co)
    elif kind == 'deconv':
      _, co, k, s, act = L
      H, W, Ci = shp
      OH, OW = H * s, W * s
      _, pt, _ = same_pads(OH, k, s)
      _, pl, _ = same_pads(OW, k, s)
      r.act = act
      r.out_shape = (OH, OW, co)
      r.desc = dict(H=H, W=W, Cin=Ci, OH=OH, OW=OW, Cout=co, K=k, stride=s, pad_t=pt, pad_l=pl)
      wshape = (k, k, co, Ci)
      assert not center
    elif kind == 'dense':
      _, u, act = L
      assert len(shp) == 1, 'dense needs a flat input (add a flatten layer)'
      r.act, r.K, r.N = act, shp[0], u
      r.out_shape = (u,)
      wshape = (shp[0], u)
      assert not center
    else:
      raise ValueError(f'unknown layer kind {kind!r}')
    r.w_n = int(np.prod(wshape))
    r.b_n = wshape[-1] if kind != 'deconv' else wshape[2]
    r.w_off = layout.add((net, li, 'w'), wshape)
    r.b_off = layout.add((net, li, 'b'), (r.b_n,))
    center = False
    shp = r.out_shape
    recs.append(r)
  return recs, shp


RANGE_WORDS = 2048


class NetProgram:

  def __init__(self, lib, recs: List[LayerRec], B: int, device, params: torch.Tensor,
               grads: torch.Tensor, max_rows: int, range_words: Optional[torch.Tensor] = None,
               act_words: Optional[torch.Tensor] = None, use_act_words: bool = True, small_wgrad_gf: float = 0.8,
               direct_wgrad: bool = False):
    self.lib, self.recs, self.B, self.device = lib, recs, B, device
    self.params, self.grads = params, grads
    f32 = dict(dtype=torch.float32, device=device)
    self.act_words = (torch.zeros(len(recs) * RANGE_WORDS, dtype=torch.int32, device=device)
                      if act_words is None else act_words)
    assert self.act_words.numel() == len(recs) * RANGE_WORDS and self.act_words.is_contiguous()
    self.range_words = (torch.zeros(len(recs) * RANGE_WORDS, dtype=torch.int32, device=device)
                        if range_words is None else range_words)
    assert self.range_words.numel() == len(recs) * RANGE_WORDS and self.range_words.is_contiguous()
    self.outs = [torch.empty((B,) + r.out_shape, **f32) for r in recs]
    self.gouts = [torch.empty((B,) + r.out_shape, **f32) for r in recs]
    self.descs = []
    for r in recs:
      if r.desc is not None:
        d = r.desc
        cd = _lib.conv_desc(B, d['H'], d['W'], d['Cin'], d['OH'], d['OW'], d['Cout'],
                            d['K'], d['stride'], d['pad_t'], d['pad_l'], r.act, r.center)
        i = len(self.descs)
        cd.dx_amax = (self.range_words.data_ptr() + 4 * RANGE_WORDS * (i - 1)) if i > 0 else None
        self.descs.append(cd)
      else:
        self.descs.append(None)
    self.dy_word = [self.word(i) if i + 1 < len(recs) else None for i in range(len(recs))]
    self.dx_word = [self.word(i - 1) if i > 0 else None for i in range(len(recs))]
    for i, cd in enumerate(self.descs):
      if cd is not None:
        cd.dy_amax = self.dy_word[i]
    self.reads_x = [bool(use_act_words) and self._reads_x(i) for i in range(len(recs))]
    self.x_word: List[Optional[int]] = [None] * len(recs)
    self.y_word: List[Optional[int]] = [None] * len(recs)
    for i in range(1, len(recs)):
      if self.reads_x[i]:
        self.x_word[i] = self.y_word[i - 1] = self.aword(i - 1)
    for i, cd in enumerate(self.descs):
      if cd is not None:
        cd.x_amax, cd.y_amax = self.x_word[i], self.y_word[i]
    self.wslabs: List[Optional[torch.Tensor]] = [None] * len(recs)
    self.direct_wgrad = bool(direct_wgrad)
    self.wdirect = [False] * len(recs)
    self.wrows = [0] * len(recs)
    self.bslabs: List[Optional[torch.Tensor]] = [None] * len(recs)
    self.brows = [0] * len(recs)
    self.small_wgrad = []
    for r in recs:
      if r.desc is not None:
        d = r.desc
        mac = B * (d['OH'] * d['OW'] if r.kind == 'conv' else d['H'] * d['W']) * d['K'] ** 2 * \
            d['Cin'] * d['Cout']
      else:
        mac = B * r.K * r.N
      self.small_wgrad.append(2 * mac < float(small_wgrad_gf) * 1e9)
    self._plan_slabs()

  def word(self, i: int) -> int:
    return self.range_words.data_ptr() + 4 * RANGE_WORDS * i

  def aword(self, i: int) -> int:
    return self.act_words.data_ptr() + 4 * RANGE_WORDS * i

  def _reads_x(self, i: int) -> bool:
    r = self.recs[i]
    if self.descs[i] is None:
      return bool(self.lib.odin_dense_reads_x_range(self.B, r.K, r.N))
    fn = self.lib.odin_conv2d_reads_x_range if r.kind == 'conv' else self.lib.odin_deconv2d_reads_x_range
    return bool(fn(C.byref(self.descs[i])))

  def set_x_word(self, i: int, valid: bool) -> None:
    w = self.aword(i - 1) if (valid and self.reads_x[i]) else None
    self.x_word[i] = w
    if self.descs[i] is not None:
      self.descs[i].x_amax = w

  def set_top_word(self, kept: bool, n: Optional[int] = None) -> Optional[int]:
    n = len(self.recs) - 1 if n is None else n
    self.dy_word[n] = self.word(n) if kept else None
    if self.descs[n] is not None:
      self.descs[n].dy_amax = self.dy_word[n]
    return self.dy_word[n]

  def check_range_words(self, upto: Optional[int] = None, first: int = 0) -> None:
    n = len(self.recs) if upto is None else upto
    for i in range(first, n):
      if self.dy_word[i] is None or self.dy_word[i] != self.word(i):
        continue
      blk = self.range_words[RANGE_WORDS * i:RANGE_WORDS * (i + 1)]
      bound = float(blk.view(torch.float32).max().item())
      t = self.gouts[i]
      m = float(torch.nan_to_num(t, nan=0.0, posinf=0.0, neginf=0.0).abs().max().item())
      assert bound >= m, f'range word of gouts[{i}] ({self.recs[i].kind}): {bound} < max|t| = {m}'

  def dgrad_keeps_range(self, j: int) -> bool:
    if j <= 0 or j >= len(self.recs):
      return False
    if self.descs[j] is None:
      return self.bslabs_wanted(j - 1) is False and bool(
          self.lib.odin_dense_dgrad_keeps_range(self.B, self.recs[j].K, self.recs[j].N))
    fn = (self.lib.odin_conv2d_dgrad_keeps_range if self.recs[j].kind == 'conv'
          else self.lib.odin_deconv2d_dgrad_keeps_range)
    return bool(fn(C.byref(self.descs[j]), ACT[self.recs[j - 1].act]))

  def bslabs_wanted(self, i: int) -> bool:
    return self.recs[i].kind == 'deconv'

  def _plan_slabs(self):
    lib, B = self.lib, self.B
    f32 = dict(dtype=torch.float32, device=self.device)
    rows = C.c_int(0)
    for i, r in enumerate(self.recs):
      d = self.descs[i]
      if r.kind == 'conv':
        lib.odin_conv2d_wgrad(None, None, None, C.byref(rows), C.byref(d), None)
        n = r.w_n + r.b_n
      elif r.kind == 'deconv':
        lib.odin_deconv2d_wgrad(None, None, None, C.byref(rows), C.byref(d), None)
        r1, r2 = C.c_int(0), C.c_int(0)
        lib.odin_deconv2d_bwd(None, None, None, None, ACT[self.recs[i - 1].act] if i > 0 else 0, None, None, C.byref(r2),
                              None, C.byref(r1), C.byref(d), None)
        rows.value = max(rows.value, r1.value)
        n = r.w_n
      else:
        lib.odin_dense_wgrad(None, None, None, C.byref(rows), B, r.K, r.N, None)
        n = r.w_n + r.b_n
      self.wrows[i] = rows.value
      if (self.direct_wgrad and r.kind == 'dense' and rows.value == 1 and r.b_off == r.w_off + r.w_n and
          self.grads[r.w_off:].data_ptr() % 16 == 0):
        self.wslabs[i] = self.grads[r.w_off:r.w_off + n].view(1, n)
        self.wdirect[i] = True
        continue
      self.wslabs[i] = torch.empty((rows.value, n), **f32)
      if r.kind == 'deconv':
        assert i + 1 < len(self.recs), 'a network may not END with a Conv2DTranspose'
        self.bslabs[i] = torch.empty((lib.odin_max_slab_rows(), r.b_n), **f32)

  def w(self, i):
    r = self.recs[i]
    return self.params[r.w_off:r.w_off + r.w_n]

  def b(self, i):
    r = self.recs[i]
    return self.params[r.b_off:r.b_off + r.b_n]

  def forward(self, x: torch.Tensor, st, upto: Optional[int] = None, start: int = 0):
    lib, B = self.lib, self.B
    h = x
    for i in range(start, len(self.recs) if upto is None else upto):
      r = self.recs[i]
      y = self.outs[i]
      if r.kind == 'conv':
        lib.odin_conv2d_fwd(h.data_ptr(), self.w(i).data_ptr(), self.b(i).data_ptr(),
                            y.data_ptr(), C.byref(self.descs[i]), st)
      elif r.kind == 'deconv':
        lib.odin_deconv2d_fwd(h.data_ptr(), self.w(i).data_ptr(), self.b(i).data_ptr(),
                              y.data_ptr(), C.byref(self.descs[i]), st)
      else:
        lib.odin_dense_fwd_ranged(h.data_ptr(), self.w(i).data_ptr(), self.b(i).data_ptr(),
                                  y.data_ptr(), B, r.K, r.N, ACT[r.act], self.x_word[i], self.y_word[i], st)
      h = y
    return h

  def backward(self, x: torch.Tensor, gout_last: torch.Tensor, st,
               dx_out: Optional[torch.Tensor] = None, last: Optional[int] = None,
               skip_bias_of_last: bool = False, data_only: bool = False,
               fork=None, side_jobs: Optional[list] = None, first: int = 0) -> List[ReduceJob]:
    lib, B = self.lib, self.B
    n = len(self.recs) if last is None else last + 1
    jobs: List[ReduceJob] = []
    g = gout_last
    rows = C.c_int(0)
    for i in range(n - 1, first - 1, -1):
      r, d = self.recs[i], self.descs[i]
      xin = x if i == 0 else self.outs[i - 1]
      slab = self.wslabs[i]
      wst = st if (fork is None or not fork.wants(self.small_wgrad[i])) else fork(i)
      if i > 0:
        prev = self.recs[i - 1]
        dst, aux, aux_act = self.gouts[i - 1], self.outs[i - 1], ACT[prev.act]
        bslab = self.bslabs[i - 1]
      elif dx_out is not None:
        dst, aux, aux_act, bslab = dx_out, None, 0, None
      else:
        dst = None
      auxp = aux.data_ptr() if (dst is not None and aux is not None and aux_act != 0) else None
      bsp = bslab.data_ptr() if (dst is not None and bslab is not None) else None
      both = (not data_only) and dst is not None and wst is st
      wrows = C.c_int(0)
      if both:
        if r.kind == 'conv':
          lib.odin_conv2d_bwd(xin.data_ptr(), g.data_ptr(), self.w(i).data_ptr(), auxp, aux_act, dst.data_ptr(),
                              bsp, C.byref(rows), slab.data_ptr(), C.byref(wrows), C.byref(d), st)
        elif r.kind == 'deconv':
          lib.odin_deconv2d_bwd(xin.data_ptr(), g.data_ptr(), self.w(i).data_ptr(), auxp, aux_act, dst.data_ptr(),
                                bsp, C.byref(rows), slab.data_ptr(), C.byref(wrows), C.byref(d), st)
        else:
          lib.odin_dense_bwd_ranged(xin.data_ptr(), g.data_ptr(), self.w(i).data_ptr(), auxp, aux_act, dst.data_ptr(),
                                    bsp, C.byref(rows), slab.data_ptr(), C.byref(wrows), B, r.K, r.N, 1, 1,
                                    self.dy_word[i], self.dx_word[i], self.x_word[i], st)
      elif data_only:
        pass
      elif r.kind == 'conv':
        lib.odin_conv2d_wgrad(xin.data_ptr(), g.data_ptr(), slab.data_ptr(), C.byref(wrows),
                              C.byref(d), wst)
      elif r.kind == 'deconv':
        lib.odin_deconv2d_wgrad(xin.data_ptr(), g.data_ptr(), slab.data_ptr(), C.byref(wrows),
                                C.byref(d), wst)
      else:
        lib.odin_dense_bwd_ranged(xin.data_ptr(), g.data_ptr(), None, None, 0, None, None, None, slab.data_ptr(),
                                  C.byref(wrows), B, r.K, r.N, 1, 0, self.dy_word[i], None, self.x_word[i], wst)
      if not data_only:
        assert 0 < wrows.value <= self.wrows[i]
        n_red = slab.shape[1]
        if skip_bias_of_last and i == n - 1 and r.kind != 'deconv':
          n_red = r.w_n
        tgt = side_jobs if (side_jobs is not None and wst is not st) else jobs
        if self.wdirect[i]:
          assert wrows.value == 1
        else:
          tgt.append(ReduceJob(slab.data_ptr(), self.grads[r.w_off:].data_ptr(), n_red, wrows.value,
                               slab.shape[1], 0))
      if dst is None:
        break
      if not both:
        if r.kind == 'conv':
          lib.odin_conv2d_dgrad(g.data_ptr(), self.w(i).data_ptr(), auxp, aux_act, dst.data_ptr(),
                                bsp, C.byref(rows), C.byref(d), st)
        elif r.kind == 'deconv':
          lib.odin_deconv2d_dgrad(g.data_ptr(), self.w(i).data_ptr(), auxp, aux_act,
                                  dst.data_ptr(), bsp, C.byref(rows), C.byref(d), st)
        else:
          lib.odin_dense_bwd(None, g.data_ptr(), self.w(i).data_ptr(), auxp, aux_act, dst.data_ptr(), bsp,
                             C.byref(rows), None, None, B, r.K, r.N, 0, 1, self.dy_word[i], self.dx_word[i], st)
      if bslab is not None and not data_only:
        pr = self.recs[i - 1]
        jobs.append(ReduceJob(bslab.data_ptr(), self.grads[pr.b_off:].data_ptr(), pr.b_n,
                              rows.value, pr.b_n, 0))
      g = dst
    return jobs


OBS_MODE = {'gaussian': 0, 'gaussian_softplus1': 1, 'qlogistic': 2}
MIXQL_K = 10


def observation_maps(observation: str, C: int) -> int:
  if observation == 'bernoulli':
    return C
  if observation == 'mixqlogistic':
    return MIXQL_K * (2 * C + C * (C - 1) // 2 + 1)
  return 2 * C
H_ALPHA, H_B1, H_B2, H_EPS, H_GSCALE, H_INVB, H_KLW, H_BETA, H_TCCOEF, H_TCGRAD = range(10)
H_CAP = 15
N_HYPER = 16
MMD_KERNELS = {'gaussian': 0, 'linear': 1}
PRIOR_KEY_SALT = 0x6D6D6470 << 32


class LatentTerm(NamedTuple):
  value: Optional[torch.Tensor] = None
  dz: Optional[torch.Tensor] = None
  dloc: Optional[torch.Tensor] = None
  dscale: Optional[torch.Tensor] = None
  launch: Optional[Callable] = None

  def ptr(self) -> Optional[int]:
    return None if self.value is None else self.value.data_ptr()


class VAEEngine:

  def __init__(self, enc_layers, dec_layers, in_shape, zdim, batch_size, device,
               observation='bernoulli', analytic=False, free_bits=None, tc=None, lib=None,
               params: Optional[torch.Tensor] = None, world_size: int = 1, seed: int = 1,
               optim_state: Optional[Tuple[torch.Tensor, torch.Tensor]] = None,
               force_dp: bool = False, reverse: bool = True, capacity: bool = False,
               range_words: Optional[torch.Tensor] = None, *,
               act_words: bool = True, hyper_ring: bool = True, hyper_ring_rows: int = 128, fuse_norm: bool = True,
               overlap_wgrad: Optional[str] = None, early_reduce: bool = False, defer_wgrad: bool = False,
               side_streams: int = 2, small_wgrad_gf: float = 0.8, dp_buckets: Optional[int] = None,
               neck: bool = True, neck_bwd: Optional[bool] = None, static_top_word: bool = True,
               latent_reg: Optional[str] = None, reg_coef: float = 1.0, mmd_kernel: str = 'gaussian',
               mmd_prior_samples: int = 100, dip_lambda: Tuple[float, float] = (1.0, 2.0), prior_seed: int = 0,
               vamprior_components: Optional[int] = None, pseudoinputs_mean: float = -0.05,
               pseudoinputs_std: float = 0.01, pseudoinputs=None,
               vq_codes: Optional[int] = None, vq_code_size: Optional[int] = None, vq_commitment: float = 0.25,
               vq_ema: bool = False, vq_ema_decay: float = 0.99, vq_epsilon: float = 1e-5, vq_state=None):
    self.lib = lib if lib is not None else _lib.load()
    self.device = torch.device(device)
    self.B, self.D = int(batch_size), int(zdim)
    self.capacity_on = bool(capacity)
    self.in_shape = tuple(in_shape)
    self.observation = observation
    self.set_kl_form(analytic, reverse)
    self.free_bits = -1.0 if free_bits is None else float(free_bits)
    self.tc_mode, self.world_size, self.seed = tc, int(world_size), int(seed)
    self.is_dp = self.world_size > 1 or bool(force_dp)
    self.tc_sharded = tc == 'betatc' and self.is_dp
    if latent_reg not in (None, 'mmd', 'dip_i', 'dip_ii'):
      raise ValueError(f"latent_reg={latent_reg!r}: expected None, 'mmd', 'dip_i' or 'dip_ii'")
    if latent_reg is not None and tc is not None:
      raise ValueError(f'latent_reg={latent_reg!r} cannot be combined with tc={tc!r}')
    if latent_reg == 'mmd' and mmd_kernel not in MMD_KERNELS:
      raise NotImplementedError(f'mmd_kernel={mmd_kernel!r}: the HIP path offers {sorted(MMD_KERNELS)}')
    self.reg_mode, self.reg_coef = latent_reg, float(reg_coef)
    self.reg_sharded = latent_reg is not None and self.is_dp
    self.vamp_K = None if vamprior_components is None else int(vamprior_components)
    if self.vamp_K is not None:
      self._check_vamprior(analytic, reverse, free_bits, tc, latent_reg, capacity, range_words)
    self.vq_K = None if vq_codes is None else int(vq_codes)
    if self.vq_K is not None:
      self._check_vq(free_bits, tc, latent_reg, capacity, range_words, neck_bwd)
      self.vq_cw, self.vq_ema = float(vq_commitment), bool(vq_ema)
      self.vq_decay, self.vq_eps = float(vq_ema_decay), float(vq_epsilon)
    f32 = dict(dtype=torch.float32, device=self.device)
    self.layout = ParamLayout()
    self.enc_recs, eo = build_layers('enc', enc_layers, self.in_shape, self.layout)
    assert len(eo) == 1, 'encoder must end with a flat output'
    self.hdim = eo[0]
    if self.vq_K is None:
      self.lat_w_off = self.layout.add(('lat', 'w'), (self.hdim, 2 * self.D))
      self.lat_b_off = self.layout.add(('lat', 'b'), (2 * self.D,))
    else:
      self.lat_w_off = self.lat_b_off = 0
      self.D = self.hdim
      self._resolve_vq_code_size(vq_code_size)
    self.dec_recs, do = build_layers('dec', dec_layers, (self.D,), self.layout)
    if self.vq_K is not None and not self.vq_ema:
      self.vq_cb_off = self.layout.add(('vq', 'codebook'), (self.vq_K, self.vq_Cs))
    if self.vamp_K is not None:
      self.vamp_u_off = self.layout.add(('vamp', 'u'), (self.vamp_K, int(np.prod(self.in_shape))))
    self.layout.pad_to(4)
    self.out_shape = do
    C_in = self.in_shape[-1]
    assert tuple(do) == self.in_shape[:-1] + (observation_maps(observation, C_in),), (do, self.in_shape)
    n = self.layout.size
    own_params = params is None
    self.params = params if params is not None else torch.zeros(n, **f32)
    assert self.params.numel() == n
    if self.vamp_K is not None and (own_params or pseudoinputs is not None):
      self._init_pseudoinputs(pseudoinputs, pseudoinputs_mean, pseudoinputs_std)
    self.grads = torch.zeros(n, **f32)
    if optim_state is not None:
      self.m, self.v = optim_state
    else:
      self.m = torch.zeros(n, **f32)
      self.v = torch.zeros(n, **f32)
    self.n_params = sum(int(np.prod(s)) for _, s, _ in self.layout.entries)
    B, D = self.B, self.D
    mr = self.lib.odin_max_slab_rows()
    ne = len(self.enc_recs)
    nl = ne + len(self.dec_recs)
    self._shared_ranges = range_words is not None
    npw = 2 * ne if self.vamp_K is not None else 0
    if self.vq_K is not None:
      npw = 1
    self.range_words = (range_words if range_words is not None else
                        torch.zeros((2 * nl + npw) * RANGE_WORDS, dtype=torch.int32, device=self.device))
    assert self.range_words.numel() == (2 * nl + npw) * RANGE_WORDS
    gw, aw = self.range_words[:nl * RANGE_WORDS], self.range_words[nl * RANGE_WORDS:2 * nl * RANGE_WORDS]
    self.enc = NetProgram(self.lib, self.enc_recs, B, self.device, self.params, self.grads, mr,
                          range_words=gw[:ne * RANGE_WORDS], act_words=aw[:ne * RANGE_WORDS],
                          use_act_words=act_words, small_wgrad_gf=small_wgrad_gf)
    self.dec = NetProgram(self.lib, self.dec_recs, B, self.device, self.params, self.grads, mr,
                          range_words=gw[ne * RANGE_WORDS:], act_words=aw[ne * RANGE_WORDS:],
                          use_act_words=act_words, small_wgrad_gf=small_wgrad_gf)
    self._act_words_dirty = False
    self._bern_keeps_top = observation == 'bernoulli' and bool(static_top_word)
    if self._bern_keeps_top:
      self.dec.set_top_word(True)
    self.p = torch.empty(B, 2 * D, **f32)
    self.dp = torch.empty(B, 2 * D, **f32)
    self.eps = torch.zeros(B, D, **f32)
    self.z = torch.empty(B, D, **f32)
    self.dz = torch.empty(B, D, **f32)
    self.kl = torch.empty(B, **f32)
    self.fbmask = torch.empty(B, **f32)
    self.dh_e = torch.empty(B, self.hdim, **f32)
    n_per = int(np.prod(self.in_shape))
    self.n_per = n_per
    npart = self._observation_fwd_bwd(None, None, None, None, None, None)
    self.llk_part = torch.empty(B * max(npart, (n_per + 1023) // 1024), **f32)
    self.llk = torch.empty(B, **f32)
    self.out8 = torch.zeros(8, **f32)
    self.out4 = self.out8[:4]
    self.n_part = 0
    if self.vq_K is None:
      rows = C.c_int(0)
      self.lib.odin_dense_wgrad(None, None, None, C.byref(rows), B, self.hdim, 2 * D, None)
      self.lat_slab = torch.empty(rows.value, self.hdim * 2 * D + 2 * D, **f32)
      self.lat_rows = rows.value
    if tc == 'betatc':
      self.tc_ws = torch.zeros(self.lib.odin_total_correlation_workspace(
          B, B * self.world_size if self.tc_sharded else B, D), **f32)
      self.tc_dz = torch.empty(B, D, **f32)
      self.tc_dloc = torch.empty(B, D, **f32)
      self.tc_dscale = torch.empty(B, D, **f32)
      if self.tc_sharded:
        Bg = B * self.world_size
        self.tc_pz_local = torch.empty(B, 3 * D, **f32)
        self.tc_pz_all = torch.empty(Bg, 3 * D, **f32)
        self.tc_p_all = torch.empty(Bg, 2 * D, **f32)
        self.tc_part_all = torch.empty(2, Bg, D, **f32)
    if latent_reg is not None:
      self._plan_latent_reg(f32, mmd_kernel, mmd_prior_samples, dip_lambda, prior_seed)
    if self.vq_K is None:
      self._plan_fused_tail(f32)
      self._plan_gauss_head(f32)
      self._plan_latent_block(f32)
      self._neck_bwd_opt = neck_bwd
      self._plan_neck(f32, bool(neck))
    else:
      self._plan_vq(f32, own_params, vq_state)
    if self.vamp_K is not None:
      self._plan_vamprior(f32, mr, act_words, small_wgrad_gf)
    self._term = self._plan_term()
    self.ws = torch.empty(4096, **f32)
    self.gnorm2 = torch.zeros(1, **f32)
    self.flag = torch.zeros(1, dtype=torch.int32, device=self.device)
    self.skip_hit = torch.zeros(1, dtype=torch.int32, device=self.device)
    self.skipped_update = torch.zeros(1, dtype=torch.int32, device=self.device)
    offs = [o for _, _, o in self.layout.entries] + [self.n_params_end()]
    self.seg_offsets = torch.tensor(offs, dtype=torch.int64, device=self.device)
    self._ring = [torch.zeros(N_HYPER + 4, dtype=torch.float32) for _ in range(8)]
    self._ring_ev = [None] * 8
    if self.device.type == 'cuda':
      self._ring = [t.pin_memory() for t in self._ring]
    self._ring_i = 0
    self.hyper = torch.zeros(N_HYPER + 4, **f32)
    self.ring_rows = int(hyper_ring_rows)
    assert self.ring_rows >= 8 and self.ring_rows & (self.ring_rows - 1) == 0
    self.hyper_ring = torch.zeros(self.ring_rows, N_HYPER + 4, **f32)
    self.fuse_norm = bool(fuse_norm)
    self.hyper_staged = torch.zeros(32, **f32)
    self._ring_host = torch.zeros(self.ring_rows, N_HYPER + 4, dtype=torch.float32)
    if self.device.type == 'cuda':
      self._ring_host = self._ring_host.pin_memory()
    self._ring_filled_to = -1
    self._ring_last_t = None
    self._ring_live = False
    self._ring_args = None
    self._ring_copy_ev = [None, None]
    self.use_hyper_ring = bool(hyper_ring)
    self.step_count = 0
    self.side_stream = torch.cuda.Stream(self.device) if self.device.type == 'cuda' else None
    n_side = int(side_streams)
    self.side_streams = ([self.side_stream] + [torch.cuda.Stream(self.device) for _ in range(n_side - 1)]
                         if self.side_stream is not None else [])
    assert overlap_wgrad in (None, 'small'), overlap_wgrad
    self.overlap_wgrad = overlap_wgrad
    self.early_reduce = bool(early_reduce)
    self.defer_wgrad = bool(defer_wgrad)
    self.graph = None
    self.debug_check_ranges = False
    self._jobs_keepalive = None
    self._jobs_cover_ok: Dict[tuple, bool] = {}
    self.comm = None
    big = self.grads.numel() * 4 >= (8 << 20)
    self.dp_buckets = int(dp_buckets or 0) or (2 if (self.world_size >= 4 and big) else 1)
    self.dec_start = min(o for k, _, o in self.layout.entries if k[0] == 'dec')

  def _plan_latent_reg(self, f32, mmd_kernel, M, dip_lambda, prior_seed):
    B, D, W = self.B, self.D, self.world_size
    if self.reg_mode == 'mmd':
      self.mmd_kernel, self.mmd_M = MMD_KERNELS[mmd_kernel], int(M)
      self.prior_key = (int(prior_seed) ^ PRIOR_KEY_SALT) & 0xFFFFFFFFFFFFFFFF
      self.reg_ws = torch.zeros(self.lib.odin_mmd_workspace(B, B * W, self.mmd_M, D), **f32)
      self.reg_dz = torch.empty(B, D, **f32)
      self.reg_y = torch.zeros(self.mmd_M, D, **f32)
      if self.reg_sharded:
        self.reg_z_all = torch.empty(B * W, D, **f32)
    else:
      self.dip_type2 = int(self.reg_mode == 'dip_ii')
      self.dip_lambda = (float(dip_lambda[0]), float(dip_lambda[1]))
      self.reg_ws = torch.zeros(self.lib.odin_dip_workspace(W, D), **f32)
      self.reg_dloc = torch.empty(B, D, **f32)
      self.reg_dscale = torch.empty(B, D, **f32)
      bs = 1 + 2 * D + D * D
      self.dip_block_local = self.reg_ws[4:4 + bs]
      self.dip_blocks = self.reg_ws[4 + bs:4 + bs + W * bs]
    self._prior_explicit = False

  def _plan_term(self) -> LatentTerm:
    if self.tc_mode == 'betatc':
      return LatentTerm(self.tc_ws, self.tc_dz, self.tc_dloc, self.tc_dscale,
                        self._tc_global if self.tc_sharded else self._tc_local)
    if self.reg_mode == 'mmd':
      return LatentTerm(self.reg_ws, dz=self.reg_dz, launch=self._reg_global if self.reg_sharded else self._mmd_local)
    if self.reg_mode is not None:
      return LatentTerm(self.reg_ws, dloc=self.reg_dloc, dscale=self.reg_dscale if self.dip_type2 else None,
                        launch=self._reg_global if self.reg_sharded else self._dip_local)
    if self.vamp_K is not None:
      return LatentTerm(self.vamp_ws, dz=self.vamp_dz, launch=self._vamp_term)
    if self.vq_K is not None:
      return LatentTerm(self.out8[4:])
    return LatentTerm()

  def _tc_local(self, st):
    self.lib.odin_total_correlation_fwd_bwd(self.z.data_ptr(), self.p.data_ptr(), self.tc_ws.data_ptr(),
                                            self.tc_dz.data_ptr(), self.tc_dloc.data_ptr(), self.tc_dscale.data_ptr(),
                                            self.hp(H_TCGRAD), self.B, self.D, st)

  def _tc_global(self, st):
    self._tc_pack()
    self._tc_gather()
    self._tc_shard(st)
    self._tc_scatter()

  def _mmd_local(self, st):
    self.lib.odin_mmd_fwd_bwd(self.z.data_ptr(), self._prior_ptr(), self.reg_ws.data_ptr(), self.reg_dz.data_ptr(),
                              None, self.hp(H_TCGRAD), self.B, self.mmd_M, self.D, self.mmd_kernel, self.prior_key,
                              self.hp(N_HYPER), st)

  def _dip_local(self, st):
    self.lib.odin_dip_fwd_bwd(self.p.data_ptr(), self.reg_ws.data_ptr(), self.reg_dloc.data_ptr(),
                              self.reg_dscale.data_ptr() if self.dip_type2 else None, None, self.hp(H_TCGRAD), self.B,
# ... 752 lines not shown
    if finalize:
      lib.odin_elbo_finalize(llk_part.data_ptr(), self.n_part, self.kl.data_ptr(), self.hp(H_BETA),
                             self._term.ptr() if tc_ptr is None else tc_ptr, self.llk.data_ptr(), self.out4.data_ptr(),
                             B, st)
    return h_d

  def _tc_pack(self):
    D = self.D
    self.tc_pz_local[:, :2 * D].copy_(self.p)
    self.tc_pz_local[:, 2 * D:].copy_(self.z)

  def _tc_gather(self):
    self._comm().all_gather(self.tc_pz_all.view(-1), self.tc_pz_local.view(-1))

  def _tc_shard(self, st=None):
    lib, B, D, W = self.lib, self.B, self.D, self.world_size
    st = self.stream() if st is None else st
    self.tc_p_all.copy_(self.tc_pz_all[:, :2 * D])
    dl, ds = self.tc_part_all[0], self.tc_part_all[1]
    lib.odin_total_correlation_shard(self.z.data_ptr(), self.tc_p_all.data_ptr(),
                                     self.tc_ws.data_ptr(), self.tc_dz.data_ptr(), dl.data_ptr(),
                                     ds.data_ptr(), self.hp(H_TCGRAD), B, B * W, D, st)

  def _tc_scatter(self):
    c = self._comm()
    c.reduce_scatter(self.tc_dloc.view(-1), self.tc_part_all[0].view(-1))
    c.reduce_scatter(self.tc_dscale.view(-1), self.tc_part_all[1].view(-1))
    c.all_reduce(self.tc_ws[:1])

  def _prior_ptr(self):
    return self.reg_y.data_ptr() if self._prior_explicit else None

  def _dip_moments(self, st=None):
    st = self.stream() if st is None else st
    self.lib.odin_dip_moments(self.p.data_ptr(), self.dip_block_local.data_ptr(), self.B, self.D, st)

  def _reg_segments(self):
    lib, B, D, W = self.lib, self.B, self.D, self.world_size
    c = self._comm
    if self.reg_mode == 'mmd':
      def shard():
        rank = c().rank
        lib.odin_mmd_shard(self.z.data_ptr(), self.reg_z_all.data_ptr(), self._prior_ptr(), self.reg_ws.data_ptr(),
                           self.reg_dz.data_ptr(), None, self.hp(H_TCGRAD), B, B * W, self.mmd_M, D, self.mmd_kernel,
                           int(rank == 0), self.prior_key, self.hp(N_HYPER), self.stream())
      return [('c', lambda: c().all_gather(self.reg_z_all.view(-1), self.z.view(-1))),
              ('k', shard),
              ('c', lambda: c().all_reduce(self.reg_ws[:1]))]

    def finish():
      lib.odin_dip_finish(self.dip_blocks.data_ptr(), W, self.p.data_ptr(), self.reg_ws.data_ptr(),
                          self.reg_dloc.data_ptr(), self.reg_dscale.data_ptr() if self.dip_type2 else None, None,
                          self.hp(H_TCGRAD), B, D, self.dip_type2, self.dip_lambda[0], self.dip_lambda[1], self.stream())
    return [('c', lambda: c().all_gather(self.dip_blocks, self.dip_block_local)), ('k', finish)]

  def finalize(self, tc_ptr: Optional[int] = None, st=None):
    st = self.stream() if st is None else st
    self.lib.odin_elbo_finalize(self._llk_part_used.data_ptr(), self.n_part, self.kl.data_ptr(),
                                self.hp(H_BETA), tc_ptr, self.llk.data_ptr(),
                                self.out4.data_ptr(), self.B, st)

  def _fork(self):
    if self.side_stream is None or not (self.overlap_wgrad or self.early_reduce):
      return None, (lambda: None)
    cur = torch.cuda.current_stream(self.device)
    sides = self.side_streams
    nxt = [0]

    def fork(i):
      side = sides[nxt[0] % len(sides)]
      nxt[0] += 1
      ev = torch.cuda.Event()
      ev.record(cur)
      side.wait_event(ev)
      return side.cuda_stream

    small_on = self.overlap_wgrad == 'small'
    fork.wants = lambda small: small_on and bool(small)

    def join():
      for side in sides[:max(1, min(nxt[0], len(sides)))]:
        cur.wait_stream(side)

    return fork, join

  def backward(self, st=None, extra_dz: Optional[torch.Tensor] = None, phase: Optional[str] = None):
    lib = self.lib
    st = self.stream() if st is None else st
    if phase == 'dec':
      jobs, _, _ = self._backward_dec(st, None)
      arr = (ReduceJob * len(jobs))(*jobs)
      self._jobs_keepalive0 = arr
      lib.odin_slab_reduce(arr, len(jobs), st)
      return
    fork, join = self._fork() if phase is None else (None, (lambda: None))
    if phase is None and fork is None and self.defer_wgrad:
      lib.odin_wgrad_planes_defer_begin()
    try:
      jobs, late_jobs, early = ([], [], False) if phase == 'enc' else self._backward_dec(st, fork)
      self._backward_enc(st, extra_dz, fork, jobs, late_jobs)
      join()
    finally:
      lib.odin_wgrad_planes_defer_end(st)
    self._reduce_slabs(jobs, early, st)

  def _backward_dec(self, st, fork):
    lib, B, D = self.lib, self.B, self.D
    late_jobs: list = []
    early = fork is not None and self.early_reduce
    if self._used_fused:
      nd = len(self.dec_recs)
      a, b = self.dec_recs[-2], self.dec_recs[-1]
      co, c1 = a.desc['Cout'], b.desc['Cout']
      jobs = self.dec.backward(self.z, self.dec.gouts[-2], st, dx_out=self.dz, last=nd - 2,
                               skip_bias_of_last=True, fork=fork,
                               side_jobs=late_jobs if early else None, first=self._dec_first())
      ts = self.tail_slab
      jobs.append(self._slab_job(ts, b.w_off, self.tail_rows, n=co * c1 + c1))
      jobs.append(ReduceJob(ts[:, co * c1 + c1:].data_ptr(), self.grads[a.b_off:].data_ptr(), co,
                            self.tail_rows, ts.shape[1], 0))
    elif self._used_head:
      nd = len(self.dec_recs)
      a, b = self.dec_recs[-2], self.dec_recs[-1]
      jobs = self.dec.backward(self.z, self.dec.gouts[-2], st, dx_out=self.dz, last=nd - 2, fork=fork,
                               side_jobs=late_jobs if early else None, first=self._dec_first())
      jobs.append(self._slab_job(self.head_slab, b.w_off, self.head_rows))
      if self.head_colsum is not None:
        jobs.append(self._slab_job(self.head_colsum, a.b_off, self.head_rows, n=a.b_n))
    else:
      jobs = self.dec.backward(self.z, self.dec.gouts[-1], st, dx_out=self.dz, fork=fork,
                               side_jobs=late_jobs if early else None, first=self._dec_first())
    if early and jobs:
      arr0 = (ReduceJob * len(jobs))(*jobs)
      self._jobs_keepalive0 = arr0
      lib.odin_slab_reduce(arr0, len(jobs), fork(-3))
      jobs = []
    return jobs, late_jobs, early

  def _backward_enc(self, st, extra_dz, fork, jobs, late_jobs):
    lib, B, D = self.lib, self.B, self.D
    T = self._term
    assert extra_dz is None or (T.dz is None and self.vq_K is None)
    dzx, tl, ts = (None if t is None else t.data_ptr()
                   for t in (T.dz if extra_dz is None else extra_dz, T.dloc, T.dscale))
    h_e = self.enc.outs[-1]
    last = self.enc_recs[-1]
    aux_act = ACT[last.act]
    lw = self.params[self.lat_w_off:]
    if self.vq_K is not None:
      self._vq_bwd(st, jobs)
    elif self._bwd_neck():
      ne = len(self.enc_recs)
      self._neck_bwd(dzx, tl, ts, st, jobs)
      jobs += self.enc.backward(self.x, self.enc.gouts[ne - 3], st, fork=fork, last=ne - 3)
    elif self._bwd_block():
      r0 = self.dec_recs[0]
      lib.odin_latent_block_bwd(self.dec.gouts[0].data_ptr(), self.dec.w(0).data_ptr(), self.z.data_ptr(),
                                self.p.data_ptr(), self.eps.data_ptr(), self.fbmask.data_ptr(),
                                self.hp(H_KLW), dzx, tl, ts, lw.data_ptr(), h_e.data_ptr(), aux_act,
                                self.dz.data_ptr(), self.dp.data_ptr(), self.enc.gouts[-1].data_ptr(),
                                self.lb_slab0.data_ptr(), self.lb_slabl.data_ptr(), B, self.hdim, D, r0.N,
                                int(self.analytic), self.enc.set_top_word(True), st)
      jobs.append(self._slab_job(self.lb_slab0, r0.w_off, self.lb_rows))
      jobs.append(self._slab_job(self.lb_slabl, self.lat_w_off, self.lb_rows))
    else:
      lib.odin_latent_bwd(self.p.data_ptr(), self.eps.data_ptr(), self.z.data_ptr(),
                          self.dz.data_ptr(), dzx, self.fbmask.data_ptr(), self.hp(H_KLW), tl, ts,
                          self.dp.data_ptr(), B, D, int(self.analytic), st)
      rows = C.c_int(0)
      lib.odin_dense_wgrad(h_e.data_ptr(), self.dp.data_ptr(), self.lat_slab.data_ptr(),
                           C.byref(rows), B, self.hdim, 2 * D,
                           st if (fork is None or not fork.wants(True)) else fork(-1))
      jobs.append(self._slab_job(self.lat_slab, self.lat_w_off, rows.value))
      auxp = h_e.data_ptr() if aux_act != 0 else None
      bslab = self.enc.bslabs[-1]
      top = self.enc.set_top_word(True)
      lib.odin_dense_bwd(None, self.dp.data_ptr(), lw.data_ptr(), auxp, aux_act, self.enc.gouts[-1].data_ptr(),
                         bslab.data_ptr() if bslab is not None else None, C.byref(rows), None, None, B,
                         self.hdim, 2 * D, 0, 1, None, top, st)
      if bslab is not None:
        jobs.append(self._slab_job(bslab, last.b_off, rows.value))
    if not self._bwd_neck():
      jobs += self.enc.backward(self.x, self.enc.gouts[-1], st, fork=fork)
    if self.vamp_K is not None:
      self._backward_pseudo(st, jobs, late_jobs)
    jobs += late_jobs
    rw = self.range_words
    jobs.append(ReduceJob(rw.data_ptr(), rw.data_ptr(), rw.numel(), 0, rw.numel(), 0))
    self._act_words_dirty = False

  def _reduce_slabs(self, jobs, early, st):
    lib = self.lib
    arr = (ReduceJob * len(jobs))(*jobs)
    self._jobs_keepalive = arr
    if callable(self.debug_check_ranges):
      self.debug_check_ranges(self)
    elif self.debug_check_ranges:
      self.dec.check_range_words(upto=len(self.dec_recs) - 1 if (self._used_fused or self._used_head) else None,
                                 first=self._dec_first() - 1 if self._bwd_neck() else 0)
      self.enc.check_range_words()
    self._norm_parts = 0
    if getattr(self, '_fuse_norm_now', False) and not early:
      nparts = C.c_int(0)
      sig = tuple((jb.dst, jb.n) for jb in jobs)
      ok = self._jobs_cover_ok.get(sig)
      if ok is None:
        ok = self._jobs_cover(jobs)
        if ok:
          lib.odin_slab_reduce_sumsq(arr, len(jobs), self.grads.data_ptr(), self.grads.numel(), None, C.byref(nparts),
                                     None, None, 0, st)
          ok = 0 < nparts.value <= 2048
        self._jobs_cover_ok[sig] = ok
      if not ok:
        lib.odin_slab_reduce(arr, len(jobs), st)
        return
      lib.odin_slab_reduce_sumsq(arr, len(jobs), self.grads.data_ptr(), self.grads.numel(), self.ws.data_ptr(),
                                 C.byref(nparts), self.hyper.data_ptr(), self.hyper_staged.data_ptr(), N_HYPER + 4, st)
      assert 0 < nparts.value <= self.ws.numel(), (nparts.value, self.ws.numel())
      self._norm_parts = nparts.value
      return
    lib.odin_slab_reduce(arr, len(jobs), st)

  def _jobs_cover(self, jobs) -> bool:
    g0, n = self.grads.data_ptr(), self.grads.numel()
    cover = np.zeros(n, dtype=np.int32)
    for jb in jobs:
      off = (jb.dst - g0) // 4 if jb.dst is not None else -1
      if 0 <= off < n:
        if off + jb.n > n:
          return False
        cover[off:off + jb.n] += 1
    end = self.n_params_end()
    return bool(int(cover[:end].min()) == 1 and int(cover.max()) == 1 and int(cover[end:].sum()) == 0)

  def grad_policies(self, st=None, clipnorm: Optional[float] = None,
                    skip_update_threshold: Optional[float] = None):
    lib = self.lib
    st = self.stream() if st is None else st
    if skip_update_threshold is not None:
      lib.odin_grad_skip_threshold(self.grads.data_ptr(), self.grads.numel(),
                                   float(skip_update_threshold), self.hp(N_HYPER + 1),
                                   self.skip_hit.data_ptr(), self.skipped_update.data_ptr(), st)
    if clipnorm is not None:
      lib.odin_clip_by_norm_segments(self.grads.data_ptr(), self.seg_offsets.data_ptr(),
                                     self.seg_offsets.numel() - 1, float(clipnorm), st)

  def adam(self, st=None, global_clipnorm: Optional[float] = None, check_nan: bool = True,
           clipvalue: Optional[float] = None, ring: bool = False):
    lib = self.lib
    st = self.stream() if st is None else st
    fin, self._fin_pending = getattr(self, '_fin_pending', None), None
    if getattr(self, '_norm_parts', 0) > 0:
      assert clipvalue is None and (global_clipnorm is not None or check_nan)
      lib.odin_adam_ring_parts(self.params.data_ptr(), self.grads.data_ptr(), self.m.data_ptr(), self.v.data_ptr(),
                               self.params.numel(), self.hyper_staged.data_ptr(), H_ALPHA, H_BETA, self.ws.data_ptr(),
                               self._norm_parts, self.gnorm2.data_ptr(), float(global_clipnorm or 0.0),
                               self.flag.data_ptr() if check_nan else None,
                               fin[0] if fin is not None else None, fin[1] if fin is not None else 0,
                               self.kl.data_ptr(), fin[2] if fin is not None else None, self.llk.data_ptr(),
                               self.out4.data_ptr(), self.B, self.hyper_ring.data_ptr() if ring else None,
                               self.hyper.data_ptr(), self.ring_rows, N_HYPER + 4, N_HYPER, st)
      self._norm_parts = 0
      return
    if ring:
      assert clipvalue is None and (global_clipnorm is not None or check_nan)
      lib.odin_sumsq_adam_ring(self.params.data_ptr(), self.grads.data_ptr(), self.m.data_ptr(), self.v.data_ptr(),
                               self.params.numel(), self.hp(H_ALPHA), self.ws.data_ptr(), self.gnorm2.data_ptr(),
                               float(global_clipnorm or 0.0), self.flag.data_ptr() if check_nan else None,
                               fin[0] if fin is not None else None, fin[1] if fin is not None else 0,
                               self.kl.data_ptr(), self.hp(H_BETA), fin[2] if fin is not None else None,
                               self.llk.data_ptr(), self.out4.data_ptr(), self.B, self.hyper_ring.data_ptr(),
                               self.hyper.data_ptr(), self.hyper_staged.data_ptr(), self.ring_rows, N_HYPER + 4,
                               N_HYPER, st)
      return
    if fin is not None and (clipvalue is not None or not (global_clipnorm is not None or check_nan)):
      lib.odin_elbo_finalize(fin[0], fin[1], self.kl.data_ptr(), self.hp(H_BETA), fin[2], self.llk.data_ptr(),
                             self.out4.data_ptr(), self.B, st)
      fin = None
    if clipvalue is not None:
      lib.odin_sumsq_flat(self.grads.data_ptr(), self.grads.numel(), self.ws.data_ptr(),
                          self.gnorm2.data_ptr(), st)
      lib.odin_clip_by_value(self.grads.data_ptr(), self.grads.numel(), float(clipvalue),
                             self.gnorm2.data_ptr() if global_clipnorm else None,
                             float(global_clipnorm or 0.0), st)
      lib.odin_adam_step_flat(self.params.data_ptr(), self.grads.data_ptr(), self.m.data_ptr(),
                              self.v.data_ptr(), self.params.numel(), self.hp(H_ALPHA),
                              self.gnorm2.data_ptr() if check_nan else None, 0.0,
                              self.flag.data_ptr(), st)
      return
    if global_clipnorm is not None or check_nan:
      if fin is not None and clipvalue is None:
        lib.odin_sumsq_adam_finalize_flat(self.params.data_ptr(), self.grads.data_ptr(), self.m.data_ptr(),
                                          self.v.data_ptr(), self.params.numel(), self.hp(H_ALPHA),
                                          self.ws.data_ptr(), self.gnorm2.data_ptr(),
                                          float(global_clipnorm or 0.0),
                                          self.flag.data_ptr() if check_nan else None, fin[0], fin[1],
                                          self.kl.data_ptr(), self.hp(H_BETA), fin[2], self.llk.data_ptr(),
                                          self.out4.data_ptr(), self.B, st)
        return
      lib.odin_sumsq_adam_flat(self.params.data_ptr(), self.grads.data_ptr(), self.m.data_ptr(),
                               self.v.data_ptr(), self.params.numel(), self.hp(H_ALPHA),
                               self.ws.data_ptr(), self.gnorm2.data_ptr(),
                               float(global_clipnorm or 0.0), self.flag.data_ptr() if check_nan else None, st)
      return
    lib.odin_adam_step_flat(self.params.data_ptr(), self.grads.data_ptr(), self.m.data_ptr(),
                            self.v.data_ptr(), self.params.numel(), self.hp(H_ALPHA), None,
                            0.0, self.flag.data_ptr(), st)

  def allreduce(self, lo: int = 0, hi: Optional[int] = None):
    if self.is_dp:
      self._comm().all_reduce(self.grads[lo:hi])

  def step_program(self, x, eps, pol, prior=None):
    P = []
    tc_dp = self.tc_sharded
    if tc_dp:
      P.append(('k', lambda: self.forward(x, eps, tc_split=True)))
      P.append(('c', self._tc_gather))
      P.append(('k', self._tc_shard))
      P.append(('c', self._tc_scatter))
      P.append(('k', lambda: self.finalize(self._term.ptr())))
    elif self.reg_sharded:
      P.append(('k', lambda: self.forward(x, eps, tc_split=True, prior=prior)))
      P += self._reg_segments()
      P.append(('k', lambda: self.finalize(self._term.ptr())))
    else:
      def fwd():
        self.forward(x, eps, finalize=False, prior=prior)
        self._fin_pending = (self._llk_part_used.data_ptr(), self.n_part, self._term.ptr())
      P.append(('k', fwd))
    if self.is_dp and self.dp_buckets >= 2:
      cur = lambda: torch.cuda.current_stream(self.device)
      side = self.side_stream

      def reduce_dec_async():
        if side is None:
          return self.allreduce(self.dec_start, None)
        side.wait_stream(cur())
        with torch.cuda.stream(side):
          self.allreduce(self.dec_start, None)

      def reduce_enc_and_join():
# ... 104 lines not shown
```

Measured before the change: 535,600 images/sec.

## Fuse first-conv weight gradient into second conv's data-gradient kernel

```diff
diff --git a/include/odin_hip.h b/include/odin_hip.h
--- a/include/odin_hip.h
+++ b/include/odin_hip.h
@@ -60,6 +60,9 @@
 int odin_deconv2d_bwd(const float* x, const float* dy, const float* w, const float* aux, int aux_act, float* dx,
                       float* colsum_slab, int* colsum_rows_out, float* wslab, int* wslab_rows_out,
                       const odin_conv_desc* d, void* stream);
+int odin_conv2d_dgrad_first(const float* dy, const float* w, const float* aux, int aux_act, float* dx,
+                            float* colsum_slab, int* colsum_rows_out, const odin_conv_desc* d, const float* x0,
+                            float* wslab0, int* wslab0_rows_out, const odin_conv_desc* d0, void* stream);
 int odin_dense_bwd(const float* x, const float* dy, const float* w, const float* aux, int aux_act, float* dx,
                    float* colsum_slab, int* colsum_rows_out, float* wslab, int* wslab_rows_out, int B, int K,
                    int N, int want_wgrad, int want_dgrad, const uint32_t* dy_amax, uint32_t* dx_amax, void* stream);
diff --git a/odin_ai_amd/_lib.py b/odin_ai_amd/_lib.py
--- a/odin_ai_amd/_lib.py
+++ b/odin_ai_amd/_lib.py
@@ -55,6 +55,7 @@
     'odin_bernoulli_tail_keeps_range': [I, DP, I],
     'odin_conv2d_bwd': [P, P, P, P, I, P, P, IP, P, IP, DP, P],
     'odin_deconv2d_bwd': [P, P, P, P, I, P, P, IP, P, IP, DP, P],
+    'odin_conv2d_dgrad_first': [P, P, P, I, P, P, IP, DP, P, P, IP, DP, P],
     'odin_dense_bwd': [P, P, P, P, I, P, P, IP, P, IP, I, I, I, I, I, P, P, P],
     'odin_dense_bwd_ranged': [P, P, P, P, I, P, P, IP, P, IP, I, I, I, I, I, P, P, P, P],
     'odin_dense_dgrad_keeps_range': [I, I, I],
diff --git a/odin_ai_amd/csrc/dispatch.hip b/odin_ai_amd/csrc/dispatch.hip
--- a/odin_ai_amd/csrc/dispatch.hip
+++ b/odin_ai_amd/csrc/dispatch.hip
@@ -9,6 +9,8 @@
   FCONV_PLANES, FCONV_RING, FCONV_BLK, CONV5_BLK, TCONV_PLANES, TCONV_RING, TCONV_BLK, IGEMM_H, IGEMM,
   WGRAD_PLANES, WGRAD5_BLK, WGRAD_BLK, IGEMM_H_WGRAD, IGEMM_WGRAD,
   BWD_PLANES, BWD_BLK,
+  TCONV_PLANES_FIRST,
+  NOT_SERVED,
   BWD_PAIR,
   TINY_DENSE, THIN_DENSE, DENSE_H, DENSE_GEMM
 };
@@ -21,7 +23,7 @@
     case FCONV_PLANES: case FCONV_BLK: case CONV5_BLK: case TCONV_PLANES: case TCONV_BLK: case IGEMM_H: case DENSE_H:
       return FOLDS_Y | FOLDS_DX | READS_X;
     case WGRAD_PLANES: case WGRAD5_BLK: case WGRAD_BLK: case IGEMM_H_WGRAD: return READS_X;
-    case BWD_PLANES: case BWD_BLK: case DENSE_GEMM: return FOLDS_DX;
+    case BWD_PLANES: case BWD_BLK: case DENSE_GEMM: case TCONV_PLANES_FIRST: return FOLDS_DX;
     default: return 0;
   }
 }
@@ -63,6 +65,11 @@
   if (odin_igemm_h_applicable(1, g)) return IGEMM_H;
   if (igemm_dgrad(1, g, slab, dry)) return IGEMM;
   return GENERIC;
+}
+
+Family select_conv2d_dgrad_first(const odin_geom& l, const odin_geom& g, const odin_geom& l0, int aux_act, bool aux_ok) {
+  if (select_conv2d_dgrad(l, g, aux_act, aux_ok, false, false) != TCONV_PLANES) return NOT_SERVED;
+  return odin_tconv_planes_first_applicable(g, l0) ? TCONV_PLANES_FIRST : NOT_SERVED;
 }
 
 Family select_deconv2d_fwd(const odin_geom& g, bool bias, int act) {
@@ -304,6 +311,23 @@
   return pair_end(rc);
 }
 
+extern "C" int odin_conv2d_dgrad_first(const float* dy, const float* w, const float* aux, int aux_act, float* dx,
+                                       float* colsum_slab, int* colsum_rows_out, const odin_conv_desc* d, const float* x0,
+                                       float* wslab0, int* wslab0_rows_out, const odin_conv_desc* d0, void* stream) {
+  const bool dry = wslab0 == nullptr;
+  const Family f = select_conv2d_dgrad_first(odin_geom_fwd(d), odin_geom_dgrad(d), odin_geom_fwd(d0), aux_act,
+                                             aux != nullptr || dry);
+  if (f != TCONV_PLANES_FIRST) return odin_fail(-2, "conv2d_dgrad_first: shapes outside the kernel");
+  if (!dry && (dy == nullptr || w == nullptr || x0 == nullptr))
+    return odin_fail(-2, "conv2d_dgrad_first: null argument");
+  int rows = 0;
+  const int rc = odin_tconv_planes_first_launch(dy, w, aux, dx, colsum_slab, x0, d0->center, wslab0, &rows, d->B, d->dy_amax,
+                                                d->dx_amax, stream);
+  if (rc == 0 && wslab0_rows_out) *wslab0_rows_out = rows;
+  if (rc == 0 && colsum_rows_out) *colsum_rows_out = rows;
+  return keep_range(rc, f, FOLDS_DX, dx, (size_t)d->B * d->H * d->W * d->Cin, d->dx_amax, stream);
+}
+
 extern "C" int odin_conv2d_dgrad_keeps_range(const odin_conv_desc* d, int aux_act) {
   const Family f = select_conv2d_dgrad(odin_geom_fwd(d), odin_geom_dgrad(d), aux_act, true, false, false);
   return (traits(f) & FOLDS_DX) ? 1 : 0;
diff --git a/odin_ai_amd/csrc/odin_internal.h b/odin_ai_amd/csrc/odin_internal.h
--- a/odin_ai_amd/csrc/odin_internal.h
+++ b/odin_ai_amd/csrc/odin_internal.h
@@ -141,6 +141,10 @@
                              const float* target, float* logits, float* llk_part, int* n_part_out,
                              float* slab, const float* scale, int C1, int B, int H, int W, int CI,
                              int CO, int epi, const uint32_t* in_amax, uint32_t* out_amax, void* stream);
+bool odin_tconv_planes_first_applicable(const odin_geom& g, const odin_geom& l0);
+int odin_tconv_planes_first_launch(const float* in, const float* w, const float* aux, float* out, float* colsum, const float* img,
+                                   int center0, float* wslab0, int* rows_out, int B, const uint32_t* in_amax,
+                                   uint32_t* out_amax, void* stream);
 
 bool odin_wgrad_planes_applicable(const odin_geom& g);
 int odin_wgrad_planes_launch(const float* U, const float* V, float* slab, int* rows_out, int B, int OH,
diff --git a/odin_ai_amd/csrc/tconv_planes.hip b/odin_ai_amd/csrc/tconv_planes.hip
--- a/odin_ai_amd/csrc/tconv_planes.hip
+++ b/odin_ai_amd/csrc/tconv_planes.hip
@@ -26,6 +26,10 @@
   unsigned* out_amax;
   long long* stamps;
   int part_off;
+  const float* img;
+  float* wslab0;
+  int center0;
+  int fw_off;
 };
 
 #if defined(ODIN_SIM) || !defined(ODIN_DIAG)
@@ -76,14 +80,23 @@
   int x, y;
 };
 
+__host__ __device__ constexpr int tp_fw_addr(int lp, int n) {
+  return (lp >> 1) * 256 + (((((lp & 1) << 3) + (n >> 2)) ^ ((lp >> 1) & 7)) << 4) + (n & 3) * 4;
+}
+constexpr int TP_FW_IMG_STRIDE = 72;
+constexpr int TP_FW_IMG_FLOATS = 18 * TP_FW_IMG_STRIDE;
+constexpr int TP_FW_BYTES = 8 * 4096 + TP_FW_IMG_FLOATS * 4;
+static_assert(16 * 17 * 32 * 4 <= TP_FW_BYTES, "the partials of the 16 chains overlay the stage and the patch");
+
 struct TpItem {
   float4 v;
   int dst;
   int ok;
 };
 
-template <int EPI, int C1, int W, int DBG = 0, bool ACC = false, int SCM = 0, bool PL = false>
+template <int EPI, int C1, int W, int DBG = 0, bool ACC = false, int SCM = 0, bool PL = false, bool FW = false>
 __device__ __forceinline__ void tp_body(const TPParams& p) {
+  static_assert(!FW || (EPI == 2 && W == 16 && C1 == 1 && !ACC && !PL), "FW: the 32-channel data gradient, 16-pixel rows");
   constexpr int NPL = TP_NPL;
   constexpr int RP = 64 / W;
   constexpr int NSLOT = 2 * RP + 3;
@@ -164,6 +177,11 @@
         make_float4(0.f, 0.f, 0.f, 0.f);
   }
 
+  float* fw_img = reinterpret_cast<float*>(smem + p.fw_off + 8 * 4096);
+  if (FW) {
+    for (int e = tid; e < TP_FW_IMG_FLOATS; e += 512) fw_img[e] = 0.f;
+  }
+
   constexpr int RPF = 2 * F_RJ;
   const int NF = p.tiles_per_wg + 3;
   TpEnt* tr = reinterpret_cast<TpEnt*>(ring + NSLOT * RB);
@@ -329,6 +347,40 @@
     pa[r] = t > 0.f ? t : em1;
   };
   auto elu_r = [&](int r) { elu_b(r, 0.f); };
+  const OdinRun IMG = odin_run(FW ? p.img : nullptr, FW ? (unsigned)((size_t)p.B * 64 * 64 * 4) : 0u);
+  const int fw_rowl = tid >> 4, fw_c4 = tid & 15;
+  float4 imgP = make_float4(0.f, 0.f, 0.f, 0.f);
+  bool imgokP = false;
+  auto fw_load = [&](int b, int t, float4& v, bool& ok) {
+    const int row = 16 * t - 1 + fw_rowl;
+    ok = tid < 288 && row >= 0 && row < 64;
+    v = odin_run_load4(IMG, ok ? (unsigned)((((b * 64 + row) * 64) + 4 * fw_c4) * 4) : ODIN_OOB);
+  };
+  const int fw_k = lane >> 5, fw_j = lane & 31;
+  const bool fw_tap = fw_j < 16;
+  const float fw_aconst = fw_j == 16 ? 1.f : 0.f;
+  const int fw_a_lane = fw_tap ? (2 * wave + (fw_j >> 2)) * TP_FW_IMG_STRIDE + 2 * fw_k + (fw_j & 3) + 3 : 0;
+  f32x16 faccA = f32x16_zero(), faccB = f32x16_zero();
+  auto fw_chain = [&](f32x16 acc) __attribute__((always_inline)) {
+    const float* ib = fw_img + fw_a_lane;
+    const char* sb = smem + p.fw_off;
+#pragma unroll
+    for (int u0 = 0; u0 < 16; u0 += 4) {
+      float av[4], bv[4];
+#pragma unroll
+      for (int u = 0; u < 4; ++u) {
+        const float a = ib[4 * (u0 + u)];
+        av[u] = fw_tap ? a : fw_aconst;
+        bv[u] = *reinterpret_cast<const float*>(sb + tp_fw_addr(wave * 32 + 2 * (u0 + u) + fw_k, fw_j));
+      }
+#pragma unroll
+      for (int u = 0; u < 4; ++u) acc = mfma32(av[u], bv[u], acc);
+    }
+    return acc;
+  };
+  auto fw_phase = [&](int t) __attribute__((always_inline)) {
+    if (t & 1) faccB = fw_chain(faccB); else faccA = fw_chain(faccA);
+  };
   char* plds = smem + p.part_off + tid * 16;
   int tileP_loc = 0;
   auto store_q = [&](int q) __attribute__((always_inline)) {
@@ -338,6 +390,16 @@
       *reinterpret_cast<float4*>(plds + (tileP_loc * 4 + q) * 8192) =
           make_float4(pa[4 * q], pa[4 * q + 1], pa[4 * q + 2], pa[4 * q + 3]);
       return;
+    }
+    if (FW) {
+      *reinterpret_cast<float4*>(smem + p.fw_off + tp_fw_addr((int)pix_lane, 8 * q + 4 * half)) =
+          make_float4(pa[4 * q], pa[4 * q + 1], pa[4 * q + 2], pa[4 * q + 3]);
+      if (q == 0 && tid < 288) {
+        float4 v = imgP;
+        if (p.center0 && imgokP) { v.x = 2.f * v.x - 1.f; v.y = 2.f * v.y - 1.f; v.z = 2.f * v.z - 1.f; v.w = 2.f * v.w - 1.f; }
+        *reinterpret_cast<float4*>(fw_img + fw_rowl * TP_FW_IMG_STRIDE + 4 + 4 * fw_c4) = v;
+      }
+      if (p.out == nullptr) return;
     }
     odin_run_store4s(OUT, out_lane + 32 * q, tileP_out,
                      make_float4(pa[4 * q], pa[4 * q + 1], pa[4 * q + 2], pa[4 * q + 3]));
@@ -539,6 +601,8 @@
     const unsigned tile_out = tile_pix * (unsigned)p.CO * 4u, tile_tgt = tile_pix * (unsigned)C1 * 4u;
     float4 axN[4], pvN[4];
     float tgtN[(EPI == 3) ? C1 : 1] = {};
+    float4 imgN = make_float4(0.f, 0.f, 0.f, 0.f);
+    bool imgokN = false;
 #pragma unroll
     for (int q = 0; q < 4; ++q) axN[q] = pvN[q] = make_float4(0.f, 0.f, 0.f, 0.f);
     ODIN_SCHED_FENCE();
@@ -555,6 +619,7 @@
 #pragma unroll
           for (int q = 0; q < 4; ++q)
             axN[q] = odin_run_load4s(AUX, out_lane + 32 * q, tile_out);
+          if (FW) fw_load(b_cur, t_cur, imgN, imgokN);
         }
         if (EPI == 3) {
 #pragma unroll
@@ -606,6 +671,7 @@
     tileP_loc = T - T0;
 #pragma unroll
     for (int q = 0; q < 4; ++q) { axP[q] = axN[q]; pvP[q] = pvN[q]; }
+    if (FW) { imgP = imgN; imgokP = imgokN; }
 #pragma unroll
     for (int oc = 0; oc < ((EPI == 3) ? C1 : 1); ++oc) tgtP[oc] = tgtN[oc];
     itA[0] = itB[0];
@@ -620,12 +686,18 @@
 #pragma unroll 1
     for (int T = T0 + 1; T < T1; ++T) {
       sl0 += RP;
+      const int t_cons = t_cur;
+      (void)t_cons;
       if (++t_cur == p.tiles_per_img) { t_cur = 0; ++b_cur; ++sl0; }
       if (sl0 >= NSLOT) sl0 -= NSLOT;
       run_tile(TpYes{}, group_b, T);
       TP_STAMP(11);
       __syncthreads();
       TP_STAMP(10);
+      if (FW) {
+        fw_phase(t_cons);
+        __syncthreads();
+      }
       if (EPI == 3 && tid == 0) {
         const float* q = llk_red[(T - 1) & 1];
         p.llk_part[T - 1] =
@@ -642,6 +714,28 @@
     for (int k = 0; k < N_EPI_OPS; ++k) epi_op(k);
   }
   flush_llk(T1 - 1);
+  if (FW) {
+    __syncthreads();
+    fw_phase(t_cur);
+    __syncthreads();
+    float* part = reinterpret_cast<float*>(smem + p.fw_off);
+#pragma unroll
+    for (int r = 0; r < 16; ++r) {
+      const int row = (r & 3) + 8 * (r >> 2) + 4 * fw_k;
+      if (row <= 16) {
+        part[(wave * 17 + row) * 32 + fw_j] = faccA[r];
+        part[((wave + 8) * 17 + row) * 32 + fw_j] = faccB[r];
+      }
+    }
+    __syncthreads();
+    for (int e = tid; e < 17 * 32; e += 512) {
+      float tt = 0.f;
+#pragma unroll
+      for (int c = 0; c < 16; c += 4)
+        tt += (part[c * 544 + e] + part[(c + 1) * 544 + e]) + (part[(c + 2) * 544 + e] + part[(c + 3) * 544 + e]);
+      p.wslab0[(size_t)blockIdx.x * (17 * 32) + e] = tt;
+    }
+  }
 
 #if defined(ODIN_DIAG) && !defined(ODIN_SIM)
   if (p.stamps != nullptr && blockIdx.x == 0 && blockIdx.y == 0 && tid == 0) {
@@ -712,9 +806,9 @@
   }
 }
 
-template <int EPI, int C1, int W, int DBG = 0, bool ACC = false, int SCM = 0>
+template <int EPI, int C1, int W, int DBG = 0, bool ACC = false, int SCM = 0, bool FW = false>
 __global__ __launch_bounds__(512) void tconv_planes_kernel(TPParams p) {
-  tp_body<EPI, C1, W, DBG, ACC, SCM>(p);
+  tp_body<EPI, C1, W, DBG, ACC, SCM, false, FW>(p);
 }
 
 template <int EPI, int W, int SCM, bool PL>
@@ -738,12 +832,12 @@
 constexpr int TP_LDS_MAX = 152 * 1024;
 int tp_ring_bytes(int W) { return TP_WBYTES + (2 * (64 / W) + 3) * TP_NPL * (W + 2) * 64; }
 int tp_fill_bytes(int W) { return 8 * 2 * (W == 32 ? 2 : W == 16 ? 4 : 8); }
-int tp_tiles_per_wg(int W, int n_tiles, int gy) {
+int tp_tiles_per_wg(int W, int n_tiles, int gy, int extra_lds = 0) {
   int cap = odin_num_cus() / gy;
   if (cap < 1) cap = 1;
   if (cap > ODIN_MAX_COLSUM_BLOCKS) cap = ODIN_MAX_COLSUM_BLOCKS;
   int tpw = (n_tiles + cap - 1) / cap;
-  const int limit = (TP_LDS_MAX - tp_ring_bytes(W)) / tp_fill_bytes(W) - 3;
+  const int limit = (TP_LDS_MAX - extra_lds - tp_ring_bytes(W)) / tp_fill_bytes(W) - 3;
   if (tpw > limit) tpw = limit;
   if ((n_tiles + tpw - 1) / tpw > ODIN_MAX_COLSUM_BLOCKS) return -1;
   return tpw;
@@ -789,6 +883,26 @@
   else if (W == 16) ODIN_LAUNCH((tconv_planes_kernel<EPI, C1, 16, 0, ACC, SC>), grid, dim3(512), lds, stream, p);
   else ODIN_LAUNCH((tconv_planes_kernel<EPI, C1, W3, 0, ACC, SC>), grid, dim3(512), lds, stream, p);
   return odin_check_launch("tconv_planes(f16x2)");
+}
+
+int tp_launch_fw(const TPParams& p0, dim3 grid, void* stream) {
+  TPParams p = p0;
+  size_t lds = (size_t)tp_ring_bytes(16) + (size_t)(p.tiles_per_wg + 3) * tp_fill_bytes(16);
+  lds = (lds + 255) & ~(size_t)255;
+  p.fw_off = (int)lds;
+  lds += TP_FW_BYTES;
+#ifndef ODIN_SIM
+  static bool attr_done = false;
+  if (!attr_done) {
+    if (hipFuncSetAttribute(reinterpret_cast<const void*>(&tconv_planes_kernel<2, 1, 16, 0, false, 1, true>),
+                            hipFuncAttributeMaxDynamicSharedMemorySize, TP_LDS_MAX) != hipSuccess)
+      (void)hipGetLastError();
+    attr_done = true;
+  }
+#endif
+  if (lds > (size_t)TP_LDS_MAX) return odin_fail(-2, "tconv_planes(first): LDS");
+  ODIN_LAUNCH((tconv_planes_kernel<2, 1, 16, 0, false, 1, true>), grid, dim3(512), lds, stream, p);
+  return odin_check_launch("tconv_planes+wgrad0(f16x2)");
 }
 
 constexpr int TP2_LDS_MAX = 160000;
@@ -904,3 +1018,32 @@
   if (C1 == 3) return aw ? tp_launch_w<3, 3, false, 2>(p, W, grid, stream) : tp_launch_w<3, 3, false, 0>(p, W, grid, stream);
   return odin_fail(-2, "tconv_planes tail: one or three logit maps only");
 }
+
+bool odin_tconv_planes_first_applicable(const odin_geom& g, const odin_geom& l0) {
+  return odin_tconv_planes_applicable(g, 2, 1) && g.H == 16 && g.W == 16 && g.CI == 32 && g.CO == 32 && l0.B == g.B &&
+         l0.H == 64 && l0.W == 64 && l0.CI == 1 && l0.OH == 32 && l0.OW == 32 && l0.CO == 32 && l0.KH == 4 && l0.KW == 4 &&
+         l0.S == 2 && l0.pt == 1 && l0.pl == 1 && (size_t)g.B * 64 * 64 * 4 < (1ull << 31) &&
+         tp_tiles_per_wg(16, g.B * 4, 1, TP_FW_BYTES + 256) > 0;
+}
+
+int odin_tconv_planes_first_launch(const float* in, const float* w, const float* aux, float* out, float* colsum, const float* img,
+                                   int center0, float* wslab0, int* rows_out, int B, const uint32_t* in_amax,
+                                   uint32_t* out_amax, void* stream) {
+  TPParams p;
+  memset(&p, 0, sizeof(p));
+  p.in = in; p.w = w; p.aux = aux; p.out = out; p.colsum = colsum; p.img = img; p.wslab0 = wslab0; p.center0 = center0;
+  p.B = B; p.H = 16; p.CO = 32;
+  p.CS = 32; p.ci_off = 0;
+  p.stamps = g_tp_stamps;
+  p.tiles_per_img = 4;
+  p.n_tiles = B * 4;
+  p.tiles_per_wg = tp_tiles_per_wg(16, p.n_tiles, 1, TP_FW_BYTES + 256);
+  if (p.tiles_per_wg <= 0) return odin_fail(-2, "tconv_planes(first): too many tiles for the fill table");
+  const int gx = (p.n_tiles + p.tiles_per_wg - 1) / p.tiles_per_wg;
+  if (rows_out) *rows_out = gx;
+  if (wslab0 == nullptr) return 0;
+  p.in_amax = odin_range_word_of(in, (size_t)B * 16 * 16 * 32, in_amax, stream);
+  if (p.in_amax == nullptr) return odin_fail(-3, "tconv_planes(first): no range word for the gradient input");
+  p.out_amax = out != nullptr ? out_amax : nullptr;
+  return tp_launch_fw(p, dim3(gx, 1, 1), stream);
+}
diff --git a/odin_ai_amd/engine.py b/odin_ai_amd/engine.py
--- a/odin_ai_amd/engine.py
+++ b/odin_ai_amd/engine.py
@@ -110,8 +110,9 @@
   def __init__(self, lib, recs: List[LayerRec], B: int, device, params: torch.Tensor,
                grads: torch.Tensor, max_rows: int, range_words: Optional[torch.Tensor] = None,
                act_words: Optional[torch.Tensor] = None, use_act_words: bool = True, small_wgrad_gf: float = 0.8,
-               direct_wgrad: bool = False):
+               direct_wgrad: bool = False, fuse_first_wgrad: bool = False):
     self.lib, self.recs, self.B, self.device = lib, recs, B, device
+    self.fuse_first = bool(fuse_first_wgrad) and self._first_pair_qualifies()
     self.params, self.grads = params, grads
     f32 = dict(dtype=torch.float32, device=device)
     self.act_words = (torch.zeros(len(recs) * RANGE_WORDS, dtype=torch.int32, device=device)
@@ -211,6 +212,14 @@
           else self.lib.odin_deconv2d_dgrad_keeps_range)
     return bool(fn(C.byref(self.descs[j]), ACT[self.recs[j - 1].act]))
 
+  def _first_pair_qualifies(self) -> bool:
+    if len(self.recs) < 2 or any(r.kind != 'conv' for r in self.recs[:2]):
+      return False
+    r0, r1 = self.recs[0], self.recs[1]
+    k4s2 = dict(K=4, stride=2, pad_t=1, pad_l=1)
+    return (r0.act == 'elu' and r0.desc == dict(H=64, W=64, Cin=1, OH=32, OW=32, Cout=32, **k4s2) and
+            r1.desc == dict(H=32, W=32, Cin=32, OH=16, OW=16, Cout=32, **k4s2) and not r1.center)
+
   def bslabs_wanted(self, i: int) -> bool:
     return self.recs[i].kind == 'deconv'
 
@@ -223,6 +232,14 @@
       if r.kind == 'conv':
         lib.odin_conv2d_wgrad(None, None, None, C.byref(rows), C.byref(d), None)
         n = r.w_n + r.b_n
+        if i == 0 and self.fuse_first:
+          r1 = C.c_int(0)
+          try:
+            lib.odin_conv2d_dgrad_first(None, None, None, ACT[r.act], None, None, None, C.byref(self.descs[1]), None, None,
+                                        C.byref(r1), C.byref(d), None)
+            rows.value = max(rows.value, r1.value)
+          except _lib.OdinError:
+            self.fuse_first = False
       elif r.kind == 'deconv':
         lib.odin_deconv2d_wgrad(None, None, None, C.byref(rows), C.byref(d), None)
         r1, r2 = C.c_int(0), C.c_int(0)
@@ -273,7 +290,10 @@
   def backward(self, x: torch.Tensor, gout_last: torch.Tensor, st,
                dx_out: Optional[torch.Tensor] = None, last: Optional[int] = None,
                skip_bias_of_last: bool = False, data_only: bool = False,
-               fork=None, side_jobs: Optional[list] = None, first: int = 0) -> List[ReduceJob]:
+               fork=None, side_jobs: Optional[list] = None, first: int = 0,
+               fuse_first: bool = False) -> List[ReduceJob]:
+    fuse_first = (fuse_first and self.fuse_first and first == 0 and dx_out is None and not data_only and
+                  (fork is None or not (fork.wants(self.small_wgrad[0]) or fork.wants(self.small_wgrad[1]))))
     lib, B = self.lib, self.B
     n = len(self.recs) if last is None else last + 1
     jobs: List[ReduceJob] = []
@@ -296,6 +316,18 @@
       bsp = bslab.data_ptr() if (dst is not None and bslab is not None) else None
       both = (not data_only) and dst is not None and wst is st
       wrows = C.c_int(0)
+      if fuse_first and i == 1:
+        r0, slab0, rows0 = self.recs[0], self.wslabs[0], C.c_int(0)
+        lib.odin_conv2d_wgrad(xin.data_ptr(), g.data_ptr(), slab.data_ptr(), C.byref(wrows), C.byref(d), st)
+        lib.odin_conv2d_dgrad_first(g.data_ptr(), self.w(1).data_ptr(), auxp, aux_act, None, None, None, C.byref(d),
+                                    x.data_ptr(),
+                                    slab0.data_ptr(), C.byref(rows0), C.byref(self.descs[0]), st)
+        assert 0 < wrows.value <= self.wrows[1] and 0 < rows0.value <= self.wrows[0]
+        jobs.append(ReduceJob(slab.data_ptr(), self.grads[r.w_off:].data_ptr(), slab.shape[1], wrows.value,
+                              slab.shape[1], 0))
+        jobs.append(ReduceJob(slab0.data_ptr(), self.grads[r0.w_off:].data_ptr(), slab0.shape[1], rows0.value,
+                              slab0.shape[1], 0))
+        break
       if both:
         if r.kind == 'conv':
           lib.odin_conv2d_bwd(xin.data_ptr(), g.data_ptr(), self.w(i).data_ptr(), auxp, aux_act, dst.data_ptr(),
@@ -387,7 +419,7 @@
                range_words: Optional[torch.Tensor] = None, *,
                act_words: bool = True, hyper_ring: bool = True, hyper_ring_rows: int = 128, fuse_norm: bool = True,
                overlap_wgrad: Optional[str] = None, early_reduce: bool = False, defer_wgrad: bool = False,
-               side_streams: int = 2, small_wgrad_gf: float = 0.8, dp_buckets: Optional[int] = None,
+               fuse_first_wgrad: bool = True, side_streams: int = 2, small_wgrad_gf: float = 0.8, dp_buckets: Optional[int] = None,
                neck: bool = True, neck_bwd: Optional[bool] = None, static_top_word: bool = True,
                latent_reg: Optional[str] = None, reg_coef: float = 1.0, mmd_kernel: str = 'gaussian',
                mmd_prior_samples: int = 100, dip_lambda: Tuple[float, float] = (1.0, 2.0), prior_seed: int = 0,
@@ -470,7 +502,7 @@
     gw, aw = self.range_words[:nl * RANGE_WORDS], self.range_words[nl * RANGE_WORDS:2 * nl * RANGE_WORDS]
     self.enc = NetProgram(self.lib, self.enc_recs, B, self.device, self.params, self.grads, mr,
                           range_words=gw[:ne * RANGE_WORDS], act_words=aw[:ne * RANGE_WORDS],
-                          use_act_words=act_words, small_wgrad_gf=small_wgrad_gf)
+                          use_act_words=act_words, small_wgrad_gf=small_wgrad_gf, fuse_first_wgrad=fuse_first_wgrad)
     self.dec = NetProgram(self.lib, self.dec_recs, B, self.device, self.params, self.grads, mr,
                           range_words=gw[ne * RANGE_WORDS:], act_words=aw[ne * RANGE_WORDS:],
                           use_act_words=act_words, small_wgrad_gf=small_wgrad_gf)
@@ -1529,7 +1561,8 @@
     elif self._bwd_neck():
       ne = len(self.enc_recs)
       self._neck_bwd(dzx, tl, ts, st, jobs)
-      jobs += self.enc.backward(self.x, self.enc.gouts[ne - 3], st, fork=fork, last=ne - 3)
+      jobs += self.enc.backward(self.x, self.enc.gouts[ne - 3], st, fork=fork, last=ne - 3,
+                                fuse_first=self._fuse_first_now())
     elif self._bwd_block():
       r0 = self.dec_recs[0]
       lib.odin_latent_block_bwd(self.dec.gouts[0].data_ptr(), self.dec.w(0).data_ptr(), self.z.data_ptr(),
@@ -1558,13 +1591,16 @@
       if bslab is not None:
         jobs.append(self._slab_job(bslab, last.b_off, rows.value))
     if not self._bwd_neck():
-      jobs += self.enc.backward(self.x, self.enc.gouts[-1], st, fork=fork)
+      jobs += self.enc.backward(self.x, self.enc.gouts[-1], st, fork=fork, fuse_first=self._fuse_first_now())
     if self.vamp_K is not None:
       self._backward_pseudo(st, jobs, late_jobs)
     jobs += late_jobs
     rw = self.range_words
     jobs.append(ReduceJob(rw.data_ptr(), rw.data_ptr(), rw.numel(), 0, rw.numel(), 0))
     self._act_words_dirty = False
+
+  def _fuse_first_now(self) -> bool:
+    return not self.defer_wgrad and not self.debug_check_ranges
 
   def _reduce_slabs(self, jobs, early, st):
     lib = self.lib
```

New measurement: 547,100 images/sec (median of 6 runs). 2.2% higher.
